# dryman/HashMergeJoin

Measured on AMD Instinct MI355X. Metric: probe-side tuples/s + achieved HBM GB/s, |R|=|S|=2^28 u64 keys, higher is better.
Workload: dtype u64

## Files before the change

### hashmergejoin_amd/_lib.py

```python
import ctypes as C
import os

HMJ_MATERIALIZE = 0x01
HMJ_ORDERED = 0x02
HMJ_FIRST_WINS = 0x04
HMJ_CHECKSUM = 0x08
HMJ_SUM_PROBE = 0x10
HMJ_NULL_EQUAL = 0x20
HMJ_E_RCCL, HMJ_E_PEER, HMJ_E_TIMEOUT = -6, -7, -8
HMJ_PATH_SLAB, HMJ_PATH_EXACT, HMJ_PATH_UNIQ_WRITE, HMJ_PATH_SPLIT, HMJ_PATH_WINDOW = 0x1, 0x2, 0x4, 0x8, 0x10
HMJ_PATH_ORDER_DEFERRED, HMJ_PATH_ORDER_BY_KEY, HMJ_PATH_PREPARED, HMJ_PATH_CHUNKED_BUILD = 0x20, 0x40, 0x80, 0x100
HMJ_PATH_HOT_KEY_HINT = 0x200
HMJ_PATH_SLAB_PROBE = 0x400
HMJ_PATH_SORTED_WRITE = 0x800
HMJ_PATH_SORTED_FK = 0x1000
HMJ_PATH_DENSE_BUILD = 0x2000
HMJ_PATH_GLOBAL_TABLE = 0x100000
HMJ_PATH_ORDER_BY_RANK_SORT = 0x200000
HMJ_PATH_ORDERED_EXPANSION = 0x400000
HMJ_PATH_LDS_TABLE = 0x800000
HMJ_PATH_RANK_RUNS = 0x1000000
HMJ_PATH_RANK_LOOKUP_IN_PASS = 0x2000000
HMJ_PATH_SORT_MSD = 0x4000000
HMJ_PATH_KEY_RANGES = 0x8000000
# ... 284 lines not shown
def load_library():
    global _LIB
    if _LIB is not None:
        return _LIB
    path = lib_path()
    if not os.path.exists(path):
        raise HmjError(-100, "HIP extension not built: %s is missing (run `make` at the repo root)" % path)
    L = C.CDLL(path)
    u, i, vp, cp = C.c_uint64, C.c_int, C.c_void_p, C.c_char_p
    L.hmj_create.restype = i
    L.hmj_create.argtypes = [C.POINTER(vp), i]
    L.hmj_destroy.restype = None
    L.hmj_destroy.argtypes = [vp]
    L.hmj_set_stream.restype = i
    L.hmj_set_stream.argtypes = [vp, vp]
    L.hmj_reserve.restype = i
    L.hmj_reserve.argtypes = [vp, u, u, u, C.c_uint32]
    L.hmj_set_radix_bits.restype = i
    L.hmj_set_radix_bits.argtypes = [vp, i]
    L.hmj_autotune_radix_bits.restype = i
    L.hmj_autotune_radix_bits.argtypes = [vp, u, u, i, C.POINTER(C.c_int), C.POINTER(C.c_double)]
    L.hmj_set_key_prefix_bits.restype = i
    L.hmj_set_key_prefix_bits.argtypes = [vp, i]
    L.hmj_plan.restype = i
    L.hmj_plan.argtypes = [u, C.POINTER(i), C.POINTER(i), C.POINTER(i * 4)]
    L.hmj_set_profiling.restype = i
    L.hmj_set_profiling.argtypes = [vp, i]
    L.hmj_last_timing.restype = i
    L.hmj_last_timing.argtypes = [vp, C.POINTER(Timing)]
    L.hmj_last_plan.restype = i
    L.hmj_last_plan.argtypes = [vp, C.POINTER(PlanDesc)]
    L.hmj_forget_workloads.restype = i
    L.hmj_forget_workloads.argtypes = [vp]
    L.hmj_placement_info.restype = i
    L.hmj_placement_info.argtypes = [vp, C.POINTER(PlaceInfo), i]
    L.hmj_strerror.restype = cp
    L.hmj_strerror.argtypes = [i]
    L.hmj_last_error.restype = cp
    L.hmj_last_error.argtypes = [vp]
    L.hmj_version.restype = cp
    L.hmj_version.argtypes = []
    L.hmj_abi_version.restype = i
    L.hmj_abi_version.argtypes = []
    L.hmj_join_u64_device.restype = i
    L.hmj_join_u64_device.argtypes = [vp, vp, u, vp, u, C.c_uint32, C.POINTER(JoinResult)]
    L.hmj_join_kind_u64_device.restype = i
    L.hmj_join_kind_u64_device.argtypes = [vp, vp, u, vp, u, C.c_uint32, C.POINTER(JoinOpts), C.POINTER(JoinResult)]
    L.hmj_join_build_kind_u64_device.restype = i
    L.hmj_join_build_kind_u64_device.argtypes = [vp, vp, u, vp, u, C.c_uint32, C.POINTER(BuildJoinOpts), C.POINTER(JoinResult)]
    L.hmj_hash_str_device.restype = i
    L.hmj_hash_str_device.argtypes = [vp, vp, vp, u, C.c_uint32, vp]
    L.hmj_join_str_device.restype = i
    L.hmj_join_str_device.argtypes = [vp, C.POINTER(StrRel), C.POINTER(StrRel), C.c_uint32, C.POINTER(StrJoinOpts),
                                      C.POINTER(StrResult)]
    L.hmj_join_kind_str_device.restype = i
    L.hmj_join_kind_str_device.argtypes = [vp, C.POINTER(StrRel), C.POINTER(StrRel), C.c_uint32, C.POINTER(StrKindOpts),
                                           C.POINTER(StrResult)]
    L.hmj_join_cols_device.restype = i
    L.hmj_join_cols_device.argtypes = [vp, C.POINTER(ColsRel), C.POINTER(ColsRel), C.c_uint32, C.POINTER(ColsJoinOpts),
                                       C.POINTER(ColsResult)]
    L.hmj_join_kind_cols_device.restype = i
    L.hmj_join_kind_cols_device.argtypes = [vp, C.POINTER(ColsRel), C.POINTER(ColsRel), C.c_uint32, C.POINTER(ColsKindOpts),
                                            C.POINTER(ColsResult)]
    L.hmj_join_mixed_device.restype = i
    L.hmj_join_mixed_device.argtypes = [vp, C.POINTER(MixedRel), C.POINTER(MixedRel), C.c_uint32, C.POINTER(MixedOpts),
                                        C.POINTER(ColsResult)]
# ... 74 lines not shown
```

### hashmergejoin_amd/csrc/api.hip

```cpp
#include <hip/hip_runtime.h>
#include <sys/mman.h>

#include <algorithm>
#include <cstdio>
#include <cstdlib>
#include <chrono>
#include <cmath>
#include <cstring>
#include <mutex>
#include <string>
#include <thread>
#include <vector>

#include "hmj_ctx.h"

using hmj::u32;
using hmj::u64;
using namespace hmj_host;

namespace hmj_host {

constexpr int kMaxEvents = 1024;

int fail(hmj_ctx* c, int code, const char* what, hipError_t e) {
// ... 347 lines not shown
  for (int i = 0; i < 4; i++) pass_bits[i] = 0;
  for (int i = 0; i < np; i++) pass_bits[i] = B / np + (i < B % np ? 1 : 0);
  *total = B;
  *passes = np;
}

static inline bool slab_sizes_ok(const hmj_ctx* c, u64 nb, u64 np, bool small_side_ok = false) {
  const u64 big = nb > np ? nb : np, small = nb > np ? np : nb;
  const u64 floor_rows = small_side_ok ? (1u << 18) : (1u << 22);
  const u64 small_min = c->slab_min_rows < floor_rows ? c->slab_min_rows : floor_rows;
  return big >= c->slab_min_rows && small >= small_min;
}

int radix_pass(hmj_ctx* c, const void* src, void* dst, u32 n, int shift, int bits, int rel,
               u64* offsets_out, int pass_index) {
  u32 nblk, rpb;
  const int variant = c->scatter_variant;
  const int tile = hmj::radix_tile_rows(bits, variant);
  hmj::radix_pass_geometry(n, tile, &nblk, &rpb);
  RC_TRY(ensure_dev(c, c->hist, (size_t)(1u << bits) * nblk * sizeof(u32)));
  RC_TRY(ensure_dev(c, c->totals, (size_t)hmj::RP_MAXD * sizeof(u32)));
  int s = span_begin(c, K_HIST, rel);
  HIP_TRY(hmj::launch_radix_hist(src, n, tile, shift, bits, (u32*)c->hist.p, nblk, rpb, c->stream));
  span_end(c, s);
  s = span_begin(c, K_SCAN, rel);
  HIP_TRY(hmj::launch_radix_rowscan((u32*)c->hist.p, nblk, bits, (u32*)c->totals.p, c->stream));
  span_end(c, s);
  s = span_begin(c, K_SCATTER, rel, pass_index);
  HIP_TRY(hmj::launch_radix_scatter(src, dst, n, variant, shift, bits, (const u32*)c->hist.p,
                                    (const u32*)c->totals.p, nblk, rpb, offsets_out, c->stream));
  span_end(c, s);
  c->timing.bytes_hist += 16ull * n;
  c->timing.bytes_scatter += 32ull * n;
  return HMJ_OK;
}

int partition_relation(hmj_ctx* c, const void* in, u32 n, DevBuf buf[2], int top, int passes,
                       const int pass_bits[4], int rel, const void** result, bool try_in_place = false) {
  *result = in;
  if (passes == 0 || n == 0) return HMJ_OK;
  if (try_in_place) {
    int bits = 0;
    for (int i = 0; i < passes; i++) bits += pass_bits[i];
    RC_TRY(ensure_dev(c, c->offs64, 8 * sizeof(u64)));
    RC_TRY(ensure_host(c, c->h_accum, 8 * sizeof(u64)));
    u32* flag = (u32*)((u64*)c->offs64.p + 7);
    u32* hflag = (u32*)((u64*)c->h_accum.p + 7);
    HIP_TRY(hipMemsetAsync(flag, 0, 4, c->stream));
    const int sp = span_begin(c, K_HIST, rel);
    HIP_TRY(hmj::launch_check_partitioned(in, n, top, bits, flag, c->num_cus, c->stream));
    span_end(c, sp);
    HIP_TRY(hipMemcpyAsync(hflag, flag, 4, hipMemcpyDeviceToHost, c->stream));
    HIP_TRY(hipStreamSynchronize(c->stream));
    if (*hflag == 0) {
      c->timing.path |= HMJ_PATH_PRESORTED;
      return HMJ_OK;
    }
  }
  RC_TRY(ensure_dev(c, buf[0], (size_t)n * 16));
  if (passes > 1) RC_TRY(ensure_dev(c, buf[1], (size_t)n * 16));
  const void* src = in;
  int shift = top;
  for (int i = 0; i < passes; i++) {
    void* dst = buf[i & 1].p;
    RC_TRY(radix_pass(c, src, dst, n, shift, pass_bits[i], rel, nullptr, i));
    shift += pass_bits[i];
// ... 113 lines not shown
  a.r_off = (const u32*)c->r_off.p;
  a.S = Sp;
  a.s_off = (const u32*)c->s_off.p;
  a.P = P;
  a.Q = Q;
  a.accum = (u64*)c->accum.p;
  return a;
}
static hmj::ProbeArgs slab_probe_args(hmj_ctx* c, const hmj::SlabGeom* build_slabs, const void* Rp, const DevBuf& s_slab,
                                      const DevBuf& s_cnt, u32 s_cap, u32 P, u32 Q) {
  hmj::ProbeArgs a;
  std::memset(&a, 0, sizeof(a));
  if (build_slabs) {
    a.R = c->slab_br.p;
    a.r_cnt = (const u32*)c->cnt_br.p;
    a.r_cap = build_slabs->CB;
    a.r_cnt_n = c->cnt_br.cap / 4;
    a.r_rows = c->slab_br.cap / 16;
  } else {
    a.R = Rp;
    a.r_off = (const u32*)c->r_off.p;
  }
  a.S = s_slab.p;
  a.s_cnt = (const u32*)s_cnt.p;
  a.s_cap = s_cap;
  a.s_cnt_n = s_cnt.cap / 4;
  a.s_rows = s_slab.cap / 16;
  a.P = P;
  a.Q = Q;
  a.accum = (u64*)c->accum.p;
  return a;
}

static int slab_pass_a(hmj_ctx* c, const void* in, u32 n, int rel, int low, int bits, const hmj::SlabGeom& g, bool arriving) {
  u64* acc = (u64*)c->accum.p;
  const u64 a_rows = c->slab_a.cap / 16, a_cnt = c->cnt_a.cap / 4;
  const int sp = span_begin(c, K_SCATTER, rel, 0);
  if (arriving) {
    u32 w_done = 0;
    for (size_t i = 0; i < c->arrive_ev.size(); i++) {
      RC_TRY(wait_arrival(c, c->arrive_ev[i]));
      const bool last = i + 1 == c->arrive_ev.size();
      const u32 w_end = last ? g.WA : (u32)std::min<u64>(g.WA, c->arrive_rows[i] / g.rpw);
      if (w_end > w_done) {
        HIP_TRY(hmj::launch_slab_a(in, n, low, bits, g, c->slab_a.p, a_rows, (u32*)c->cnt_a.p, a_cnt, acc, c->stream, w_done, w_end));
        w_done = w_end;
      }
    }
  } else {
    HIP_TRY(hmj::launch_slab_a(in, n, low, bits, g, c->slab_a.p, a_rows, (u32*)c->cnt_a.p, a_cnt, acc, c->stream));
  }
  span_end(c, sp);
  c->timing.bytes_scatter += 32ull * n;
  return HMJ_OK;
}
static int slab_passes(hmj_ctx* c, const void* in, u32 n, int rel, int low, int ba, int bb, const hmj::SlabGeom& g, DevBuf& sb,
                       DevBuf& cb, bool arriving) {
  RC_TRY(slab_pass_a(c, in, n, rel, low, ba, g, arriving));
  const int sp = span_begin(c, K_SCATTER, rel, 1);
  HIP_TRY(hmj::launch_slab_b(c->slab_a.p, (const u32*)c->cnt_a.p, ba, low + ba, bb, g, sb.p, sb.cap / 16, (u32*)cb.p, cb.cap / 4,
                             (u64*)c->accum.p, c->stream));
  span_end(c, sp);
  c->timing.bytes_scatter += 32ull * n;
  return HMJ_OK;
}

static int clear_matched(hmj_ctx* c, size_t slots, u32** matched) {
  const size_t bytes = (slots / 32 + 1) * 4;
  RC_TRY(ensure_dev(c, c->matched, bytes));
  *matched = (u32*)c->matched.p;
  HIP_TRY(hipMemsetAsync(c->matched.p, 0, bytes, c->stream));
  return HMJ_OK;
}

int order_rows(hmj_ctx* c, const u32* vstart, const u32* in_base32, const u64* in_base64, u32 P, u32 Q, int low,
               u64 n, bool by_key_only, bool many_per_key, const u64** rk, const u64** rr, const u64** rs, int* retry_code) {
  const size_t bytes = (size_t)n * 8;
  RC_TRY(ensure_dev(c, c->ord_key, bytes));
  RC_TRY(ensure_dev(c, c->ord_rval, bytes));
  RC_TRY(ensure_dev(c, c->ord_sval, bytes));
  const bool can_sort = n <= 0xFFFFFFFFull;
  if (by_key_only && !can_sort) {
    *retry_code = kRetryNoWinOrdered;
    return HMJ_OK;
  }
  int sp = span_begin(c, K_ORDER, -1);
  HIP_TRY(hmj::launch_order((const u64*)c->part_out_off.p, vstart, in_base32, in_base64, P, Q, low,
                            (const u64*)c->out_key.p, (const u64*)c->out_rval.p, (const u64*)c->out_sval.p,
                            (u64*)c->ord_key.p, (u64*)c->ord_rval.p, (u64*)c->ord_sval.p, (u64*)c->accum.p,
                            can_sort ? 65536u : 0u, many_per_key, c->num_cus * 4, c->stream));
  span_end(c, sp);
  u64* h = (u64*)c->h_accum.p;
  HIP_TRY(hipMemcpyAsync(&h[hmj::ACC_ERR], (u64*)c->accum.p + hmj::ACC_ERR, 8, hipMemcpyDeviceToHost, c->stream));
  HIP_TRY(hipStreamSynchronize(c->stream));
  if (h[hmj::ACC_ERR] & hmj::ERR_ORDER_FAIL)
    return fail(c, HMJ_E_UNSUPPORTED, "HMJ_ORDERED: one partition's result exceeds 2^31-1 rows and the whole result 2^32-1 rows");
// ... 520 lines not shown

static int run_slab_join(hmj_ctx* c, const JoinCall& j, const JoinPlan& p) {
  const bool materialize = j.materialize(), first = j.first(), extra = j.extra();
  const u32 nb = j.nb, np = j.np, np_plan = p.np_plan, P = p.P;
  const int* pass_bits = p.pass_bits;
  hmj::SlabGeom gr, gs;
  if (p.allow_slab && c->slab_mode && c->wm->slab_cooldown == 0 && !c->prepare_only && !(c->timing.path & HMJ_PATH_SLAB) &&
      !((!materialize || p.fast_write) && p.Q == 1 && p.probe_fits && p.passes == 2 && pass_bits[0] <= hmj::SLAB_MAX_BITS &&
        pass_bits[1] <= hmj::SLAB_MAX_BITS && p.dense_scale <= 2.5))
    c->plan.refused |= HMJ_REFUSED_SLAB_SHAPE;
  if (!(p.allow_slab && c->slab_mode && c->wm->slab_cooldown == 0 && (!materialize || p.fast_write) && p.Q == 1 &&
        p.probe_fits &&
        p.passes == 2 && pass_bits[0] <= hmj::SLAB_MAX_BITS && pass_bits[1] <= hmj::SLAB_MAX_BITS &&
        slab_sizes_ok(c, nb, np_plan, materialize || np_plan < nb) &&
        p.dense_scale <= 2.5 &&
        hmj::slab_geometry(nb, pass_bits[0], pass_bits[1], &gr, 0, 1.0, p.dense_scale) &&
        hmj::slab_geometry(np_plan, pass_bits[0], pass_bits[1], &gs, 0,
                           (nb && np_plan > nb) ? (double)np_plan / (double)nb : 1.0, p.dense_scale)))
    return kPlanNotTaken;
  const bool reuse = c->prep.valid && c->prep.slab && c->prep.ptr == j.R && c->prep.n == nb &&
                     c->prep.low == p.low && c->prep.B == p.B;
  c->prep.valid = false;
  c->timing.path |= HMJ_PATH_SLAB | (reuse ? HMJ_PATH_PREPARED : 0u);
  c->timing.n_probe_items = P;
  const int ba = pass_bits[0], bb = pass_bits[1];
  const u64 rows_a = gr.rows_a > gs.rows_a ? gr.rows_a : gs.rows_a;
  const u32 wa = gr.WA > gs.WA ? gr.WA : gs.WA;
  RC_TRY(ensure_dev(c, c->slab_a, rows_a * 16));
  RC_TRY(ensure_dev(c, c->cnt_a, ((size_t)wa << ba) * 4));
  RC_TRY(ensure_dev(c, c->slab_br, gr.rows_b * 16));
  RC_TRY(ensure_dev(c, c->slab_bs, gs.rows_b * 16));
  RC_TRY(ensure_dev(c, c->cnt_br, (size_t)P * gr.KB * 4));
  RC_TRY(ensure_dev(c, c->cnt_bs, (size_t)P * gs.KB * 4));
  if (!reuse) RC_TRY(slab_passes(c, j.R, nb, 0, p.low, ba, bb, gr, c->slab_br, c->cnt_br, false));
  if (!c->prepare_only) RC_TRY(slab_passes(c, j.S, np, 1, p.low, ba, bb, gs, c->slab_bs, c->cnt_bs, !c->arrive_ev.empty()));
  u64* hh;
  if (c->prepare_only) {
    RC_TRY(read_accum(c, &hh));
    if (hh[hmj::ACC_ERR] & hmj::ERR_SLAB) {
      c->wm->slab_cooldown = 8;
      return kRetryNoSlab;
    }
    c->prep.valid = true;
    c->prep.slab = true;
    c->prep.ptr = j.R;
    c->prep.n = nb;
    c->prep.low = p.low;
    c->prep.B = p.B;
    return HMJ_OK;
  }
  hmj::ProbeArgs sa = slab_probe_args(c, &gr, nullptr, c->slab_bs, c->cnt_bs, gs.CB, P, 1);
  if (p.fast_write)
    return unique_key_write(c, sa, true, nb, np, p.low, extra, p.verify_pfx ? p.prefix : 0, p.pfx_ref, j.ordered(), j.to_host,
                            p.fk_wide_plan, p.dense_scale, j.out);
#ifdef HMJ_DEV
  sa.debug = c->dev_ablate;
#endif
  int sp = span_begin(c, K_PROBE_COUNT, -1);
  if (first || extra) {
    sa.extra = (extra ? 1u : 0u) | (first ? 2u : 0u);
    HIP_TRY(hmj::launch_probe_count_ext(sa, nullptr, nullptr, true, c->num_cus, c->stream));
  } else {
    HIP_TRY(hmj::launch_probe_count_slab(sa, c->num_cus, c->stream));
  }
  span_end(c, sp);
  c->timing.bytes_probe_count = 16ull * ((u64)nb + np);
  RC_TRY(read_accum(c, &hh));
  if (hh[hmj::ACC_ERR] & hmj::ERR_SLAB) {
    c->wm->slab_cooldown = 8;
    return kRetryNoSlab;
  }
  result_sums(j.out, hh);
  return HMJ_OK;
}

static int partition_build_exact(hmj_ctx* c, const JoinCall& j, const JoinPlan& p, const void** Rp) {
  const bool reuse_exact = c->prep.valid && !c->prep.slab && c->prep.ptr == j.R && c->prep.n == j.nb &&
                           c->prep.low == p.low && c->prep.B == p.B;
  c->prep.valid = false;
  c->timing.path |= HMJ_PATH_EXACT | (reuse_exact ? HMJ_PATH_PREPARED : 0u);
  if (reuse_exact) {
    *Rp = c->prep.Rp;
  } else {
    RC_TRY(partition_relation(c, j.R, j.nb, c->rbuf, p.low, p.passes, p.pass_bits, 0, Rp, p.asc_r));
    const int s = span_begin(c, K_OFFSETS, -1);
    HIP_TRY(hmj::launch_part_offsets(*Rp, j.nb, p.low, p.B, (u32*)c->r_off.p, c->stream));
    span_end(c, s);
  }
  if (c->prepare_only) {
    HIP_TRY(hipStreamSynchronize(c->stream));
    c->prep.valid = true;
    c->prep.slab = false;
    c->prep.ptr = j.R;
    c->prep.Rp = *Rp;
    c->prep.n = j.nb;
    c->prep.low = p.low;
    c->prep.B = p.B;
  }
  return HMJ_OK;
}

static int run_probe_slab_join(hmj_ctx* c, const JoinCall& j, const JoinPlan& p, const void* Rp) {
  const bool materialize = j.materialize(), first = j.first(), extra = j.extra();
// ... 1089 lines not shown
      HIP_TRY(hipMemcpyAsync((u64*)c->cat_key.p + rows_done, sub.key, bytes, hipMemcpyDeviceToDevice, c->stream));
      HIP_TRY(hipMemcpyAsync((u64*)c->cat_rval.p + rows_done, sub.rval, bytes, hipMemcpyDeviceToDevice, c->stream));
      HIP_TRY(hipMemcpyAsync((u64*)c->cat_sval.p + rows_done, sub.sval, bytes, hipMemcpyDeviceToDevice, c->stream));
      rows_done += sub.n_matches;
    }
    tot.n_matches += sub.n_matches;
    tot.sum_r += sub.sum_r;
    tot.sum_s += sub.sum_s;
    tot.xor_fold ^= sub.xor_fold;
    tot.mix_sum += sub.mix_sum;
    tot.sum_probe_all += sub.sum_probe_all;
  }
  HIP_TRY(hipStreamSynchronize(c->stream));
  *out = tot;
  out->key = rows_done ? (const uint64_t*)c->cat_key.p : nullptr;
  out->rval = rows_done ? (const uint64_t*)c->cat_rval.p : nullptr;
  out->sval = rows_done ? (const uint64_t*)c->cat_sval.p : nullptr;
  c->timing = tsum;
  c->timing.path |= HMJ_PATH_KEY_RANGES;
  *done = true;
  return HMJ_OK;
}

int join_device(hmj_ctx* c, const void* R, uint64_t n_build, const void* S, uint64_t n_probe,
                uint32_t flags, hmj_result* out, bool to_host) {
  if ((flags & HMJ_MATERIALIZE) && !(flags & HMJ_ORDERED) && !c->prepare_only && !c->join_kind && c->promote_to_ordered && n_build > 0 &&
      n_probe <= 0xFFFFFFFFull && n_probe >= c->big_join_rows && (double)n_probe >= 2.5 * (double)n_build && c->force_bits < 0) {
    const double P18 = (double)(1u << (2 * hmj::SLAB_MAX_BITS));
    const double hi = fk_probe_rows_hi((double)n_probe / P18, (double)n_probe / (double)n_build, P18);
    if (hi > 5120.0 && hi <= 6144.0) flags |= HMJ_ORDERED;
  }
  memo_for(c, workload_signature(n_build, c->prepare_only ? c->probe_hint : n_probe, flags, c->join_kind ? 2 + (int)c->join_kind : c->memo_kind));
  std::memset(&c->plan, 0, sizeof(c->plan));
  int rc = HMJ_OK, kr_h = 0;
  bool kr_done = false;
  if (!c->join_kind && key_ranges_wanted(c, n_build, n_probe, flags, to_host, &kr_h)) {
    rc = join_by_key_ranges(c, R, n_build, S, n_probe, flags, out, kr_h, &kr_done);
  } else if (c->cat_key.p) {
    free_dev(c->cat_key);
    free_dev(c->cat_rval);
    free_dev(c->cat_sval);
  }
  if (rc == HMJ_OK && !kr_done) rc = join_device_planned(c, R, n_build, S, n_probe, flags, out, to_host);
  hmj_plan_desc& p = c->plan;
  p.struct_size = sizeof(p);
  p.path = c->timing.path;
  p.radix_bits = c->timing.radix_bits;
  p.radix_passes = c->timing.radix_passes;
  p.key_prefix_bits = c->timing.key_prefix_bits;
  p.key_window_low = c->timing.key_window_low;
  p.n_partitions = (c->timing.path & (HMJ_PATH_GLOBAL_TABLE | HMJ_PATH_LDS_TABLE)) ? 0u : (p.radix_bits < 32 ? 1u << p.radix_bits : 0u);
  p.probe_items = c->timing.n_probe_items;
  p.cooling = c->wm->cooling();
  p.workload = c->wm_sig;
  return rc;
}
static int join_device_planned(hmj_ctx* c, const void* R, uint64_t n_build, const void* S, uint64_t n_probe, uint32_t flags,
                               hmj_result* out, bool to_host) {
  const bool kinds = c->join_kind != 0;
  if (!kinds) {
    bool done = false;
    int rc = try_global_table(c, R, n_build, S, n_probe, flags, out, to_host, &done);
    if (rc != HMJ_OK || done) return rc;
    rc = try_small_build_ordered(c, R, n_build, S, n_probe, flags, out, to_host, &done);
    if (rc != HMJ_OK || done) return rc;
  }
// ... 6 lines not shown
  struct Unforce {
    hmj_ctx* c;
    bool* on;
    ~Unforce() {
      if (*on) c->force_bits = -1;
      c->expand_allow_rebits = true;
    }
  } unforce{c, &forced_here};
  for (int attempt = 0; attempt < 8; attempt++) {
    c->plan.attempts = (uint32_t)attempt + 1;
    int rc = join_device_impl(c, R, n_build, S, n_probe, flags, out, to_host, auto_prefix, slab, fast_write,
                              win_ordered, prefix_unsafe, slab_probe);
    c->plan.refused |= rc == kRetryNoSlab ? HMJ_REFUSED_SLAB_OVERFLOW : rc == kRetryNoPrefix ? HMJ_REFUSED_PREFIX_VIOLATED
                       : rc == kRetryNoFastWrite ? HMJ_REFUSED_FAST_WRITE_GAVE_UP : rc == kRetryNoSlabProbe ? HMJ_REFUSED_SLAB_PROBE_OVERFLOW
                       : rc == kRetryMoreBits ? HMJ_REFUSED_EXPANSION_GAVE_UP : 0u;
    if (c->trace)
      std::fprintf(stderr, "[hmj] join nb=%llu np=%llu flags=%#x attempt %d: rc=%d bits=%d passes=%d path=%#x prefix=%d low=%d items=%u%s\n",
                   (unsigned long long)n_build, (unsigned long long)n_probe, flags, attempt, rc, c->timing.radix_bits,
                   c->timing.radix_passes, c->timing.path, c->timing.key_prefix_bits, c->timing.key_window_low,
                   c->timing.n_probe_items,
                   rc == kRetryNoSlab ? " -> retry without the slab path (a slab overflowed)"
                   : rc == kRetryNoPrefix ? " -> retry: a row outside the sampled key prefix"
                   : rc == kRetryNoFastWrite ? " -> retry without the unique-key write mode"
                   : rc == kRetryNoWinOrdered ? " -> retry without the key window"
                   : rc == kRetryNoSlabProbe ? " -> retry without probe-side slabs (one overflowed)"
                   : rc == kRetryMoreBits ? " -> retry with one more radix bit (a partition did not fit the ordered expansion)" : "");
    if (rc == kRetryNoSlab || rc == kRetryNoPrefix || rc == kRetryNoFastWrite || rc == kRetryNoWinOrdered || rc == kRetryNoSlabProbe ||
        rc == kRetryMoreBits) {
      std::vector<Span> keep;
      for (const Span& sp : c->spans)
        if (sp.kind == K_TOTAL || sp.kind == K_H2D) keep.push_back(sp);
      c->spans.swap(keep);
      std::memset(&c->timing, 0, sizeof(c->timing));
      if (rc == kRetryNoSlab) slab = false;
      else if (rc == kRetryMoreBits) {
        c->force_bits = c->expand_rebits;
        c->expand_allow_rebits = false;
        forced_here = true;
      }
      else if (rc == kRetryNoSlabProbe) slab_probe = false;
      else if (rc == kRetryNoFastWrite) fast_write = false;
      else if (rc == kRetryNoWinOrdered) win_ordered = false;
      else if (!prefix_unsafe && win_ordered) {
        prefix_unsafe = true;
        c->wm->exact_prefix_joins = 32;
      }
      else auto_prefix = false;
      continue;
    }
    return rc;
  }
  return fail(c, HMJ_E_HIP, "join could not be planned");
}

int prepare_build(hmj_ctx* c, const void* R, uint64_t n_build, uint64_t n_probe_hint) {
  hmj_result dummy;
  c->prepare_only = true;
  c->probe_hint = n_probe_hint;
  c->prep.valid = false;
  const int rc = join_device(c, R, n_build, nullptr, 0, 0, &dummy, false);
  c->prepare_only = false;
  return rc;
}

int join_device_kind(hmj_ctx* c, const JoinKind& k, const void* R, uint64_t n_build, const void* S, uint64_t n_probe,
                     uint32_t flags, hmj_result* out, hmj_kind_counts* counts) {
// ... 17 lines not shown
    const u64 unmatched = k.kind == HMJ_JOIN_SEMI ? n_probe - out->n_matches : filled;
    counts->n_probe_matched = n_probe - unmatched;
    counts->n_probe_unmatched = unmatched;
  } else {
    const u64 b_unmatched = k.kind == HMJ_BUILD_SEMI ? n_build - swept : swept;
    counts->n_build_matched = n_build - b_unmatched;
    counts->n_build_unmatched = b_unmatched;
    if (k.kind == HMJ_FULL_OUTER) {
      counts->n_probe_matched = n_probe - filled;
      counts->n_probe_unmatched = filled;
    }
  }
  return HMJ_OK;
}

}

extern "C" {

int hmj_create(hmj_ctx** out, int device_id) {
  if (!out) return HMJ_E_ARG;
  *out = nullptr;
  int ndev = 0;
  if (hipGetDeviceCount(&ndev) != hipSuccess || ndev <= 0) {
    (void)hipGetLastError();
    return HMJ_E_NODEV;
  }
  if (device_id < 0 && hipGetDevice(&device_id) != hipSuccess) return HMJ_E_NODEV;
  if (device_id >= ndev) return HMJ_E_ARG;
  if (hipSetDevice(device_id) != hipSuccess) return HMJ_E_NODEV;
  hmj_ctx* c = new hmj_ctx();
  c->device = device_id;
  if (const char* e = getenv("HMJ_SLAB")) c->slab_mode = atoi(e);
  if (const char* e = getenv("HMJ_ONE_PASS_SLAB")) c->one_pass_slab = atoi(e) != 0;
  if (const char* e = getenv("HMJ_GTABLE")) c->gtable_mode = atoi(e) != 0;
  if (const char* e = getenv("HMJ_RANK_RUNS")) c->rank_runs_mode = atoi(e) != 0;
  if (const char* e = getenv("HMJ_RANK_RUNS_MAX_CUT")) c->rank_runs_max_cut = atoi(e) < 0 ? 0 : atoi(e) > 16 ? 16 : atoi(e);
  if (const char* e = getenv("HMJ_RANK_RUNS_MAX_GROUP")) c->rank_runs_max_group = atoi(e) < 0 ? 0 : atoi(e) > 4 ? 4 : atoi(e);
  if (const char* e = getenv("HMJ_PROMOTE_TO_ORDERED")) c->promote_to_ordered = atoi(e) != 0;
  if (const char* e = getenv("HMJ_KEY_RANGES")) c->key_ranges = atoi(e) != 0;
  if (const char* e = getenv("HMJ_KEY_RANGES_FORCE")) c->key_ranges_force = atoi(e) < 0 ? 0 : atoi(e) > 4 ? 4 : atoi(e);
  if (const char* e = getenv("HMJ_RANK_RUNS_WAVE")) c->rank_runs_wave = atoi(e) != 0;
  if (const char* e = getenv("HMJ_RANK_RUNS_MAX_LEVEL")) c->rank_runs_max_level = atoi(e) < 0 ? 0 : atoi(e) > 2 ? 2 : atoi(e);
  if (const char* e = getenv("HMJ_GTABLE_SORT")) c->gtable_sort_mode = atoi(e) != 0;
  if (const char* e = getenv("HMJ_EXPAND_FK_FANOUT")) c->expand_fk_fanout = atoi(e) > 0 ? (u32)atoi(e) : 0u;
  if (const char* e = getenv("HMJ_SORT_MSD")) c->sort_msd = atoi(e) != 0;
  if (const char* e = getenv("HMJ_SORT_MSD_MEAN")) c->sort_msd_mean = atof(e) >= 64.0 ? atof(e) : c->sort_msd_mean;
  if (const char* e = getenv("HMJ_SORT_MSD_MAX_BITS")) c->sort_msd_max_bits = atoi(e) < 2 ? 2 : atoi(e) > 18 ? 18 : atoi(e);
  if (const char* e = getenv("HMJ_SORT_MSD_MIN_LOG2")) {
    const int l = atoi(e);
    if (l >= 16 && l <= 32) c->sort_msd_min = 1ull << l;
  }
  if (const char* e = getenv("HMJ_SORT_SLAB_MIN_LOG2")) {
    const int l = atoi(e);
    if (l >= 12 && l <= 32) c->sort_slab_min = 1ull << l;
  }
  if (const char* e = getenv("HMJ_GTABLE_SORT_SLAB_MIN_LOG2")) {
    const int l = atoi(e);
    if (l >= 12 && l <= 32) c->gtable_sort_slab_min = 1ull << l;
  }
  if (const char* e = getenv("HMJ_GTABLE_SORT_FANOUT")) c->gtable_sort_fanout = atoi(e) > 0 ? (u32)atoi(e) : 1u;
  if (const char* e = getenv("HMJ_PLACE")) {
    c->place_tune = atoi(e) != 0;
    if (atoi(e) > 0) {
      c->place_tries = atoi(e);
      c->place_search_always = true;
// ... 208 lines not shown
  return HMJ_OK;
}

int hmj_set_profiling(hmj_ctx* c, int enabled) {
  if (!c) return HMJ_E_ARG;
  c->profiling = enabled != 0;
  return HMJ_OK;
}

int hmj_placement_info(hmj_ctx* c, hmj_place_info* out, int max_entries) {
  if (!c || !out || max_entries <= 0) return 0;
  int n = 0;
  for (const hmj_place_info& e : c->place_log)
    if (n < max_entries) out[n++] = e;
  return n;
}

int hmj_last_plan(hmj_ctx* c, hmj_plan_desc* out) {
  if (!c || !out || out->struct_size < 8) return HMJ_E_ARG;
  const uint32_t room = out->struct_size < sizeof(hmj_plan_desc) ? out->struct_size : (uint32_t)sizeof(hmj_plan_desc);
  hmj_plan_desc p = c->plan;
  p.struct_size = room;
  std::memcpy(out, &p, room);
  return HMJ_OK;
}

int hmj_forget_workloads(hmj_ctx* c) {
  if (!c) return HMJ_E_ARG;
  c->memos.clear();
  c->wm = &c->memo_init;
  c->wm_sig = 0;
  return HMJ_OK;
}

int hmj_last_timing(hmj_ctx* c, hmj_timing* out) {
  if (!c || !out) return HMJ_E_ARG;
  *out = c->timing;
  return HMJ_OK;
}

const char* hmj_strerror(int code) {
  switch (code) {
    case HMJ_OK: return "ok";
    case HMJ_E_ARG: return "invalid argument";
    case HMJ_E_NODEV: return "no usable HIP device";
    case HMJ_E_OOM: return "out of device or pinned host memory";
    case HMJ_E_HIP: return "HIP runtime error";
    case HMJ_E_UNSUPPORTED: return "unsupported flag combination for this input";
    case HMJ_E_RCCL: return "RCCL / transport error";
    case HMJ_E_PEER: return "another rank of the collective failed";
    case HMJ_E_TIMEOUT: return "the exchange step timed out (a peer never took part); the communicator was aborted";
    default: return "unknown error";
  }
}

const char* hmj_last_error(hmj_ctx* c) { return c ? c->last_error.c_str() : ""; }
const char* hmj_version(void) { return "hashmergejoin_amd 0.5 (gfx950)"; }
int hmj_abi_version(void) { return HMJ_ABI_VERSION; }

int hmj_reserve(hmj_ctx* c, uint64_t n_build, uint64_t n_probe, uint64_t max_matches,
                uint32_t flags) {
  if (!c) return HMJ_E_ARG;
  if (n_build > 0xFFFFFFFFull || n_probe > 0xFFFFFFFFull) return fail(c, HMJ_E_ARG, "too many rows");
  HIP_TRY(hipSetDevice(c->device));
  c->prep.valid = false;
  struct InReserve {
// ... 588 lines not shown
```

### hashmergejoin_amd/csrc/hmj_ctx.h

```cpp
#pragma once
#include <hip/hip_runtime.h>

#include <string>
#include <unordered_map>
#include <vector>

#include "../../include/hmj.h"
#include "hmj_dev.h"
#include "hmj_launch.h"

struct hmj_comm;

namespace hmj_host {

struct DevBuf {
  void* p = nullptr;
  size_t cap = 0;
};
struct HostBuf {
  void* p = nullptr;
  size_t cap = 0;
  bool pinned = true;
};

// ... 33 lines not shown
    for (DevBuf* b : {&rows, &sorted, &flags, &blk, &blk_off, &list, &runs, &acc, &start}) f(*b);
    each_result_buf(f);
  }
};

enum Kind {
  K_TOTAL = 0, K_H2D, K_D2H, K_HIST, K_SCAN, K_SCATTER, K_OFFSETS, K_PROBE_COUNT, K_OUT_SCAN,
  K_PROBE_WRITE, K_ORDER, K_NKINDS
};
struct Span {
  int kind, rel, e0, e1;
  int pass;
};

struct WorkloadMemo {
  int uniq_cooldown = 0;
  int sorted_cooldown = 0;
  bool sorted_chained = false;
  bool sorted_wide = true;
  bool sorted_fk = false;
  int sorted_fk_age = 0;
  int gtable_cooldown = 0;
  int gtable_write_cooldown = 0;
  int gtable_sort_cooldown = 0;
  int gtable_sort_slab_cooldown = 0;
  int rank_runs_cooldown = 0;
  int rank_lookup_cooldown = 0;
  int expand_cooldown = 0;
  int sort_slab_cooldown = 0;
  int sort_msd_cooldown = 0;
  int slab_cooldown = 0;
  int slab_probe_cooldown = 0;
  int one_pass_write_cooldown = 0;
  int exact_prefix_joins = 0;
  uint32_t cooling() const;
};

}

namespace hmj_host {
struct OrderedCostModel {
  double part_fixed_ms = 0.15;
  double part_ns = 0.030, part_ns_per_f = 0.00023;
  double part_bucket_ns = 0.043, part_bucket_ns_per_f = 0.0001;
  double part_epilogue_ns = 0.25;
  double comp_fixed_ms = 0.65;
  double comp_ns_chain = 0.060, comp_ns_exact = 0.072;
  double comp_ns_wide = 0.145;
  double comp_ns_beyond_l2 = 0.02;
  double runs_fixed_ms = 0.25, runs_ns = 0.0215, runs_ns_per_run = 7.5;
  double runs_ns_per_log2_build = 0.0023;
  double runs_wave_ns_per_run = 1.2, runs_wave_ns = 0.007;
  double runs_range_ns = 0.0;
};
}

struct hmj_ctx {
  using DevBuf = hmj_host::DevBuf;
  using HostBuf = hmj_host::HostBuf;
  using Span = hmj_host::Span;
  using WorkloadMemo = hmj_host::WorkloadMemo;
  using u32 = hmj::u32;
  using u64 = hmj::u64;
  int device = 0, num_cus = 256;
  hipStream_t own_stream = nullptr, stream = nullptr;
  DevBuf rbuf[2], sbuf[2], in_r, in_s, hist, totals, r_off, s_off, part_count, part_out_off, accum,
// ... 55 lines not shown
  uint64_t gtable_max_rows = 1ull << 17;
  u32 gtable_min_fanout = 0;
  uint64_t gtable_min_probe = 1;
  int gtable_wg_per_cu = 8;
  u32 gtable_slots_per_row = 16;
  int gtable_max_log_cap = 18;
  bool ltable_mode = true;
  bool gtable_sort_mode = true;
  u32 gtable_sort_fanout = 128;
  bool rank_runs_mode = true;
  int rank_runs_max_cut = 10;
  int rank_runs_max_group = 3;
  int rank_runs_max_level = 2;
  uint64_t big_join_rows = 1ull << 29;
  bool promote_to_ordered = true;
  bool key_ranges = true;
  int key_ranges_force = 0;
  bool rank_runs_wave = true;
  bool build_sort_msd = true;
  bool gtable_sort_slab = true;
  u64 gtable_sort_slab_min = 1ull << 25;
  bool expand_mode = true;
  u32 fk_payload_buckets = 24;
  u32 expand_fk_fanout = 0;
  bool expand_allow_rebits = true;
  int expand_rebits = 0;
  bool sort_msd = true;
  double sort_msd_mean = 1200.0;
  int sort_msd_max_bits = 18;
  u64 sort_msd_min = 1ull << 22;
  bool sort_slab = true;
  u64 sort_slab_min = 1ull << 25;
  int slab_mode = 1;
  bool staged_upload = false;
  bool host_pipeline = true;
  hipStream_t copy_stream = nullptr;
  std::vector<hipEvent_t> copy_ev;
  bool split_mode = true;
  bool window_mode = true;
  u32 slab_min_rows = 1u << 21;
  u32 slab_probe_kb = 0;
  bool one_pass_slab = true;
  int scatter_variant = 1;
  bool profiling = false;
  bool trace = false;
#ifdef HMJ_DEV
  u32 dev_ablate = 0;
#endif
  std::vector<hipEvent_t> events;
  std::vector<Span> spans;
  int ev_used = 0;
  hmj_timing timing;
  std::string last_error;
  hmj_comm* comm = nullptr;
  std::vector<u64> arrive_rows;
  std::vector<hipEvent_t> arrive_ev;
  bool sample_build_only = false;
  int (*arrive_wait)(hmj_ctx*, hipEvent_t) = nullptr;
};


namespace hmj_host {
int fail(hmj_ctx* c, int code, const char* what, hipError_t e = hipSuccess);
#define HIP_TRY(expr)                                                        \
  do {                                                                       \
    hipError_t _e = (expr);                                                  \
// ... 38 lines not shown
```

### hashmergejoin_amd/csrc/hmj_dev.h

```cpp
#pragma once
#include <hip/hip_runtime.h>
#include <stdint.h>

namespace hmj {

typedef unsigned long long u64;
typedef unsigned int u32;
typedef unsigned short u16;

struct __attribute__((aligned(16))) Tup {
  u64 key;
  u64 val;
};

constexpr int kWave = 64;
#ifndef HMJ_SCAN_DPP
#define HMJ_SCAN_DPP 1
#endif

#ifndef HMJ_STREAM_POLICY
#define HMJ_STREAM_POLICY 2
#endif
typedef u64 u64x2_t __attribute__((ext_vector_type(2)));
__device__ __forceinline__ void store_stream(Tup* p, const Tup& v) {
#if HMJ_STREAM_POLICY >= 1
  u64x2_t x = {v.key, v.val};
  __builtin_nontemporal_store(x, reinterpret_cast<u64x2_t*>(p));
#else
  *p = v;
#endif
}
__device__ __forceinline__ Tup load_stream(const Tup* p) {
#if HMJ_STREAM_POLICY >= 2
  const u64x2_t x = __builtin_nontemporal_load(reinterpret_cast<const u64x2_t*>(p));
  Tup t;
  t.key = x.x;
  t.val = x.y;
  return t;
#else
  return *p;
#endif
}

constexpr u64 GT_EMPTY = ~0ull;
constexpr int GT_MAXWALK = 64;
__device__ __forceinline__ u32 gt_hash(u64 key, int shift) {
  u64 h = key * 0x9E3779B97F4A7C15ull;
  h ^= h >> 32;
  h *= 0xD6E8FEB86659FD93ull;
  return (u32)(h >> shift);
}

#ifndef HMJ_RANK_PASS_CHUNK_ROWS
#define HMJ_RANK_PASS_CHUNK_ROWS 64
#endif
constexpr int RANK_PASS_CHUNK_ROWS = HMJ_RANK_PASS_CHUNK_ROWS;
__device__ __forceinline__ u64 rank_run_bucket(u64 off, int pre, u64 mult) { return ((off >> pre) * mult) >> 32; }

template <int ROWS, typename Table, typename OnSlot>
__device__ __forceinline__ void gt_walk(Table tab, u32 mask, u32 (&slot)[ROWS], bool (&live)[ROWS], OnSlot on_slot) {
  bool any_live = false;
#pragma unroll
  for (int r = 0; r < ROWS; r++) any_live |= live[r];
  while (any_live) {
    Tup e[ROWS];
#pragma unroll
    for (int r = 0; r < ROWS; r++)
      if (live[r]) e[r] = tab[slot[r]];
    any_live = false;
#pragma unroll
    for (int r = 0; r < ROWS; r++) {
      if (live[r]) {
        if (e[r].key == GT_EMPTY || on_slot(r, e[r])) {
          live[r] = false;
        } else {
          slot[r] = (slot[r] + 1) & mask;
          any_live = true;
        }
      }
    }
  }
}

constexpr int RP_THREADS = 512;
constexpr int RP_WAVES = RP_THREADS / kWave;
constexpr int RP_ITEMS = 8;
constexpr int RP_TILE = RP_THREADS * RP_ITEMS;
constexpr int RP_MAX_BITS = 9;
constexpr int RP_MAXD = 1 << RP_MAX_BITS;
constexpr int RP_MAX_BLOCKS = 2048;

constexpr int PB_THREADS = 1024;
constexpr int PB_CAP = 5120;
constexpr int PB_LOG_NB = 12;
constexpr int PB_TARGET_AVG = 4096;
constexpr int PB_PLAN_SLACK = 256;

constexpr int SLAB_KB = 4;
constexpr int SLAB_MAX_BITS = 9;

enum { ACC_N = 0, ACC_SUM_R, ACC_SUM_S, ACC_XOR, ACC_MIX, ACC_SUM_P, ACC_ERR, ACC_PAD };
constexpr u64 ERR_SLAB = 2;
constexpr u64 ERR_ORDER_DEFER = 16;
constexpr u64 ERR_ORDER_FAIL = 32;
constexpr u64 ERR_SORTED = 64;
constexpr u64 ERR_FASTPATH = 8;
constexpr u64 ERR_GTABLE = 128;
constexpr u64 ERR_PREFIX = 4;

__device__ __forceinline__ u64 mix64(u64 x) {
  x ^= x >> 30;
  x *= 0xBF58476D1CE4E5B9ull;
  x ^= x >> 27;
  x *= 0x94D049BB133111EBull;
  x ^= x >> 31;
  return x;
}

__device__ __forceinline__ u64 tmix(u64 key, u64 rval, u64 sval) {
  u64 t = mix64(key);
  t = mix64(t ^ rval);
  t = mix64(t + sval);
  return t;
}

__device__ __forceinline__ int lane_id() {
  return __builtin_amdgcn_mbcnt_hi(~0u, __builtin_amdgcn_mbcnt_lo(~0u, 0u));
}

__device__ __forceinline__ u32 popc_below(u64 m) {
  return __builtin_amdgcn_mbcnt_hi((u32)(m >> 32), __builtin_amdgcn_mbcnt_lo((u32)m, 0u));
}

__device__ __forceinline__ u32 wave_incl_scan_u32(u32 v, int ) {
#if HMJ_SCAN_DPP
  v += (u32)__builtin_amdgcn_update_dpp(0, (int)v, 0x111, 0xF, 0xF, false);
  v += (u32)__builtin_amdgcn_update_dpp(0, (int)v, 0x112, 0xF, 0xF, false);
  v += (u32)__builtin_amdgcn_update_dpp(0, (int)v, 0x114, 0xF, 0xF, false);
  v += (u32)__builtin_amdgcn_update_dpp(0, (int)v, 0x118, 0xF, 0xF, false);
  v += (u32)__builtin_amdgcn_update_dpp(0, (int)v, 0x142, 0xA, 0xF, false);
  v += (u32)__builtin_amdgcn_update_dpp(0, (int)v, 0x143, 0xC, 0xF, false);
// ... 72 lines not shown
```

### hashmergejoin_amd/csrc/hmj_launch.h

```cpp
#pragma once
#include <hip/hip_runtime.h>
#include <stddef.h>
#include <stdint.h>

#include <atomic>

namespace hmj {
typedef unsigned long long u64;
typedef unsigned int u32;

struct SmemAttrOnce {
  std::atomic<unsigned long long> devices{0};
};
inline hipError_t ensure_max_smem(SmemAttrOnce& once, const void* kernel, size_t bytes) {
  int dev = 0;
  hipError_t e = hipGetDevice(&dev);
  if (e != hipSuccess) return e;
  const unsigned long long bit = 1ull << (dev & 63);
  if (dev < 64 && (once.devices.load(std::memory_order_acquire) & bit)) return hipSuccess;
  e = hipFuncSetAttribute(kernel, hipFuncAttributeMaxDynamicSharedMemorySize, (int)bytes);
  if (e != hipSuccess) return e;
  if (dev < 64) once.devices.fetch_or(bit, std::memory_order_release);
  return hipSuccess;
}

constexpr int kMaxRanks = 16;
struct OwnerFn {
  u32 mode;
  u32 G;
  u64 spl[kMaxRanks - 1];
};
int radix_tile_rows(int bits, int variant);
void radix_pass_geometry(u32 n, int tile, u32* nblk, u32* rows_per_block);
size_t radix_scatter_smem_bytes();
hipError_t launch_radix_hist(const void* in, u32 n, int tile, int shift, int bits, u32* hist,
                             u32 nblk, u32 rows_per_block, hipStream_t st, const OwnerFn* own = nullptr);
hipError_t launch_owner_scatter(const void* in, void* out, u32 n, int bits, const OwnerFn& own,
                                const u32* hist_scanned, const u32* totals, u32 nblk, u32 rows_per_block,
                                u64* offsets_out, hipStream_t st);
hipError_t launch_radix_rowscan(u32* hist, u32 nblk, int bits, u32* totals, hipStream_t st);
hipError_t launch_radix_scatter(const void* in, void* out, u32 n, int variant, int shift, int bits,
                                const u32* hist_scanned, const u32* totals, u32 nblk,
                                u32 rows_per_block, u64* offsets_out, hipStream_t st);
struct SlabGeom {
  u32 WA, rpw, CA, CB, KB;
  u64 rows_a, rows_b;
};
bool slab_geometry(u32 n, int bits_a, int bits_b, SlabGeom* g, u32 kb = 0, double fan = 1.0, double density = 1.0);
bool slab_geometry_one_pass(u32 n, int bits, double keys_per_digit, u32 max_workers, SlabGeom* g, double density = 1.0);
u32 slab_capacity(double mean, double fan);
hipError_t launch_slab_a(const void* in, u32 n, int shift, int bits, const SlabGeom& g, void* slab_a, u64 slab_a_rows,
                         u32* cnt_a, u64 cnt_a_n, u64* accum, hipStream_t st, u32 w_begin = 0, u32 w_end = 0xFFFFFFFFu);
hipError_t launch_slab_b(const void* slab_a, const u32* cnt_a, int bits_a, int shift, int bits,
                         const SlabGeom& g, void* slab_b, u64 slab_b_rows, u32* cnt_b, u64 cnt_b_n, u64* accum, hipStream_t st);
hipError_t launch_key_sample(const void* R, u32 nb, const void* S, u32 np, u64* out, hipStream_t st);
hipError_t launch_key_exact(const void* R, u32 nb, const void* S, u32 np, u64 ref, u64* out, int num_cus, hipStream_t st,
                            bool ref_is_first_key = false);
hipError_t launch_check_partitioned(const void* a, u32 n, int low, int bits, u32* flag, int num_cus, hipStream_t st);
hipError_t launch_part_offsets(const void* a, u32 n, int low, int bits, u32* off, hipStream_t st);

struct ProbeArgs {
  const void* R;
  const u32* r_off;
  const void* S;
  const u32* s_off;
  u32 P;
  u32 Q;
  u64* part_count;
  const u64* part_out_off;
  u64* out_key;
  u64* out_rval;
  u64* out_sval;
  u64 out_cap;
  u64* accum;
  const u32* item_list;
  const u32* n_item_list;
  const u32* r_cnt;
  const u32* s_cnt;
  u32 r_cap, s_cap;
  u32 s_wa, s_ppi;
  u64 r_cnt_n, s_cnt_n;
  u64 r_rows, s_rows;
  const u64* item_base;
  const u32* r_end;
  const u32* s_end;
  u32 extra;
  u32 pfx_shift;
  u64 pfx_val;
  u32* matched;
  u32 debug;
};
hipError_t launch_probe(const ProbeArgs& a, int mode, bool first_wins, bool extra, int grid,
                        hipStream_t st);
int probe_default_grid(int num_cus);
hipError_t launch_probe_kind(const ProbeArgs& a, int mode, int kind, bool first_wins, u64 fill, int grid, hipStream_t st);
hipError_t launch_probe_build_kind(const ProbeArgs& a, int mode, int kind, u64 fill, u32* bmark, int grid, hipStream_t st);
hipError_t launch_build_sweep(const ProbeArgs& a, const u32* r_off, u32 P, const u32* vstart, u64* sweep_n, int mode,
                              bool set, u64 fill, int num_cus, hipStream_t st);
hipError_t launch_probe_count_ext(const ProbeArgs& a, u32* irregular, u32* n_irregular, bool slab,
                                  int num_cus, hipStream_t st);
hipError_t launch_probe_count_slab(const ProbeArgs& a, int num_cus, hipStream_t st);
hipError_t launch_probe_write_sorted(const ProbeArgs& a, bool slab, bool fk, int shape, u64* lookback, bool chained, int key_low,
                                     int num_cus, hipStream_t st);
hipError_t launch_probe_write_uniq(const ProbeArgs& a, bool slab, int num_cus, hipStream_t st);
hipError_t launch_slab_np(const u32* cnt, u32 P, u64* out, hipStream_t st);
hipError_t launch_probe_count_fast(const ProbeArgs& a, u32* irregular, u32* n_irregular, bool big,
                                   bool per_partition_counts, int num_cus, hipStream_t st);
hipError_t launch_scan_u64(const u64* in, u64* out_excl, u32 n, hipStream_t st);
hipError_t launch_probe_expand_ordered(const ProbeArgs& a, int key_low, int num_cus, hipStream_t st);
hipError_t launch_order(const u64* part_out_off, const u32* vstart, const u32* in_base32, const u64* in_base64, u32 P, u32 Q,
                        int low, const u64* akey, const u64* arval, const u64* asval, u64* bkey, u64* brval,
                        u64* bsval, u64* accum, u32 defer_rows, bool many_per_key, int grid, hipStream_t st);
hipError_t launch_compact(const u64* part_out_off, const u32* in_base32, const u64* in_base64, u32 P, const u64* akey,
                          const u64* arval, const u64* asval, u64* bkey, u64* brval, u64* bsval, int grid, hipStream_t st);
hipError_t launch_rekey(void* pairs, u64 n, const u64* col, hipStream_t st);

hipError_t launch_gtable_build(const void* R, u32 nb, void* tab, int log_cap, u64* accum, bool first, int num_cus,
                               hipStream_t st);
hipError_t launch_gtable_probe(const void* S, u32 np, const void* tab, int log_cap, const void* R, u64* accum, bool first,
                               bool extra, int num_cus, int wg_per_cu, hipStream_t st);
hipError_t launch_gtable_write(const void* S, u32 np, const void* tab, int log_cap, const void* R, u64* accum, u64* out_key,
                               u64* out_rval, u64* out_sval, bool first, bool extra, int num_cus, int wg_per_cu, hipStream_t st);

hipError_t launch_ltable_probe(const void* R, u32 nb, const void* S, u32 np, u64* accum, bool first, bool extra, int num_cus, hipStream_t st);
int ltable_max_rows();
hipError_t launch_sval_range(const void* S, u32 np, u64* out2 , int num_cus, hipStream_t st,
                             u32 every = 1 );
hipError_t launch_gtable_emit(const void* S, u32 np, const void* tab, int log_cap, u64 svmin, int range_bits, u64* accum,
                              void* pairs, bool extra, bool wide, int num_cus, int wg_per_cu, hipStream_t st);
hipError_t launch_gtable_swap(const void* in, void* out, u64 n, int num_cus, hipStream_t st);
hipError_t launch_gtable_emit_ranks(const void* S, u32 np, const void* tab, int log_cap, u64* accum, void* pairs, bool extra, int num_cus,
                                    int wg_per_cu, hipStream_t st);
int rank_sort_max_run(int level = 0);
hipError_t launch_sort_runs_write(const void* slabs, const u32* cnt, u32 cap, u32 P, const u64* out_off, void* out, u64* accum, int level,
// ... 36 lines not shown
```

### hashmergejoin_amd/csrc/probe.hip

```cpp
#include "hmj_dev.h"
#include "hmj_launch.h"
#include <type_traits>

namespace hmj {

constexpr u32 PB_NB = 1u << PB_LOG_NB;
constexpr u32 NIL = 0xFFFFu;
static_assert(PB_CAP < 0xFFFF, "chain links are 16-bit");

struct ProbeSmem {
  u64 key[PB_CAP];
  u64 val[PB_CAP];
  u32 head[PB_NB];
  u32 aux[PB_CAP];
  u16 next[PB_CAP];
  u32 scratch[PB_THREADS / kWave + 1];
  u64 pcount;
  u64 red[8];
  u64 obase;
  u32 wtot[PB_THREADS / kWave];
  u32 nslot;
};
constexpr u32 PB_BATCH = 2 * PB_THREADS;
static_assert(PB_BATCH <= PB_CAP, "a batch must fit an empty table");
// ... 836 lines not shown
constexpr int FP_ROWS = 5;
#ifdef HMJ_DEV
#define HMJ_ABLATE(bit) ((a.debug & (bit)) != 0u)
#else
#define HMJ_ABLATE(bit) false
#endif
#ifndef BIG_LOG_NB
#define BIG_LOG_NB 13
#endif
#ifndef HMJ_PROBE_PIECES
#define HMJ_PROBE_PIECES 1
#endif

template <int THREADS, int LOG_NB>
struct FastSmem {
  static constexpr int CAP = THREADS * FP_ROWS;
  u64 key[CAP];
  u64 val[CAP];
  u32 head[1u << LOG_NB];
  u16 next[CAP];
  u64 red[8];
  u32 itemcnt[2];
  u64 wscan[THREADS / kWave + 1];
  u32 wdup[THREADS / kWave + 1];
};

template <int LOG_NB>
__device__ __forceinline__ u32 fast_hash(u64 k) {
  u32 x = (u32)k ^ ((u32)(k >> 32) * 0x85EBCA6Bu);
  x *= 0x9E3779B1u;
  return x >> (32 - LOG_NB);
}

template <int THREADS, int ROWS = FP_ROWS>
__device__ __forceinline__ void fp_load(Tup (&t)[ROWS], const Tup* __restrict__ base, u32 n,
                                        int tid) {
#pragma unroll
  for (int k = 0; k < ROWS; k++) {
    u32 i = k * THREADS + tid;
    t[k] = base[i < n ? i : n - 1];
  }
}

static_assert(SLAB_KB == 4, "fp_load_slab / fp_load_pieces / slab_np_kernel unroll exactly four pieces per partition");
template <int THREADS, int ROWS = FP_ROWS>
__device__ __forceinline__ void fp_load_slab(Tup (&t)[ROWS], const Tup* __restrict__ base, u32 cap,
                                             u32 p1, u32 p2, u32 p3, u32 n, int tid) {
#pragma unroll
  for (int k = 0; k < ROWS; k++) {
    u32 i = k * THREADS + tid;
    i = i < n ? i : n - 1;
    const u32 j = (i >= p1) + (i >= p2) + (i >= p3);
    const u32 pre = j == 0 ? 0u : (j == 1 ? p1 : (j == 2 ? p2 : p3));
    t[k] = base[(u64)j * cap + (i - pre)];
  }
}

template <int THREADS>
__device__ __forceinline__ void fp_load_pieces(Tup (&t)[FP_ROWS], const Tup* __restrict__ base, u32 cap, u32 cnt_mine, int tid) {
  constexpr int QT = THREADS / 4;
  const u32 g = (u32)tid / QT, l = (u32)tid % QT;
  const Tup* __restrict__ piece = base + (u64)g * cap;
  const u32 last = cnt_mine ? cnt_mine - 1 : 0;
#pragma unroll
  for (int k = 0; k < FP_ROWS; k++) {
    const u32 r = l + (u32)k * QT;
    t[k] = piece[r < last ? r : last];
  }
}

template <int THREADS, int LOG_NB, bool PCOUNT, bool SLAB, int OUT>
__global__ __launch_bounds__(THREADS, 4) void probe_count_fast_kernel(
    ProbeArgs a, u32* __restrict__ irregular, u32* __restrict__ n_irregular) {
  typedef FastSmem<THREADS, LOG_NB> Smem;
  constexpr u32 CAP = Smem::CAP, NB = 1u << LOG_NB;
  constexpr bool PIECES = SLAB && OUT == 0 && !PCOUNT && HMJ_PROBE_PIECES;
  constexpr u32 QT = THREADS / 4, PIECE_CAP = FP_ROWS * QT;
  extern __shared__ __attribute__((aligned(16))) unsigned char smem_raw[];
  Smem& sm = *reinterpret_cast<Smem*>(smem_raw);
  const Tup* __restrict__ R = static_cast<const Tup*>(a.R);
  const Tup* __restrict__ S = static_cast<const Tup*>(a.S);
  const u32* __restrict__ r_off = a.r_off;
  const u32* __restrict__ s_off = a.s_off;
  const u32* __restrict__ r_end = (SLAB || a.r_end == nullptr) ? a.r_off + 1 : a.r_end;
  const u32* __restrict__ s_end = (SLAB || a.s_end == nullptr) ? a.s_off + 1 : a.s_end;
  const u32 P = a.P;
  const int tid = threadIdx.x;
  u64 acc_n = 0, acc_r = 0, acc_s = 0, acc_x = 0, acc_m = 0, acc_p = 0;
  bool pfx_bad = false, giveup = false;
  for (u32 i = tid; i < NB; i += THREADS) sm.head[i] = 0;
  if (tid < 2) sm.itemcnt[tid] = 0;
  u32 epoch = 0;
  u32 prev_p = 0xFFFFFFFFu, parity = 0;

  u32 p = blockIdx.x;
  u32 rb = 0, nb = 0, sb = 0, np = 0;
  bool regular = false;
  Tup br[FP_ROWS], pr[FP_ROWS], pq[FP_ROWS];
  u32 r1 = 0, r2 = 0, r3 = 0, s1 = 0, s2 = 0, s3 = 0, r1n = 0, r2n = 0, r3n = 0, s1n = 0, s2n = 0, s3n = 0;
  u32 rm = 0, sm_ = 0, rmn = 0, smn = 0;
  const u32 my_piece = (u32)tid / QT;
  bool slab_bad = false;
  if (p < P) {
    if (SLAB) {
      const u32* rc = a.r_cnt + (u64)p * SLAB_KB;
      const u32* sc = a.s_cnt + (u64)p * SLAB_KB;
      r1 = rc[0]; r2 = r1 + rc[1]; r3 = r2 + rc[2]; nb = r3 + rc[3];
      s1 = sc[0]; s2 = s1 + sc[1]; s3 = s2 + sc[2]; np = s3 + sc[3];
      if (nb > CAP || np > CAP) slab_bad = true;
      if (PIECES) {
        rm = my_piece == 0 ? rc[0] : my_piece == 1 ? rc[1] : my_piece == 2 ? rc[2] : rc[3];
        sm_ = my_piece == 0 ? sc[0] : my_piece == 1 ? sc[1] : my_piece == 2 ? sc[2] : sc[3];
        if (rc[0] > PIECE_CAP || rc[1] > PIECE_CAP || rc[2] > PIECE_CAP || rc[3] > PIECE_CAP || sc[0] > PIECE_CAP ||
            sc[1] > PIECE_CAP || sc[2] > PIECE_CAP || sc[3] > PIECE_CAP) {
          slab_bad = true;
          nb = CAP + 1;
        }
      }
    } else {
      rb = r_off[p]; nb = r_end[p] - rb;
      sb = s_off[p]; np = s_end[p] - sb;
    }
    regular = nb && np && nb <= CAP && np <= CAP;
    if (regular) {
      if (PIECES) {
        fp_load_pieces<THREADS>(br, R + (u64)p * SLAB_KB * a.r_cap, a.r_cap, rm, tid);
        fp_load_pieces<THREADS>(pr, S + (u64)p * SLAB_KB * a.s_cap, a.s_cap, sm_, tid);
      } else if (SLAB) {
        fp_load_slab<THREADS>(br, R + (u64)p * SLAB_KB * a.r_cap, a.r_cap, r1, r2, r3, nb, tid);
        if (OUT == 0) fp_load_slab<THREADS>(pr, S + (u64)p * SLAB_KB * a.s_cap, a.s_cap, s1, s2, s3, np, tid);
      } else {
        fp_load<THREADS>(br, R + rb, nb, tid);
        if (OUT == 0) fp_load<THREADS>(pr, S + sb, np, tid);
      }
    }
  }
  const Tup* __restrict__ dummy = reinterpret_cast<const Tup*>(a.accum);
  auto load_build = [&](Tup (&t)[FP_ROWS], bool ok, u32 pp, u32 rb_, u32 nb_, u32 q1, u32 q2, u32 q3, u32 mine) {
    if (PIECES)
      fp_load_pieces<THREADS>(t, ok ? R + (u64)pp * SLAB_KB * a.r_cap : dummy, ok ? a.r_cap : 0u, ok ? mine : 1u, tid);
    else if (SLAB)
      fp_load_slab<THREADS>(t, ok ? R + (u64)pp * SLAB_KB * a.r_cap : dummy, ok ? a.r_cap : 0u, ok ? q1 : 1u, ok ? q2 : 1u,
                            ok ? q3 : 1u, ok ? nb_ : 1u, tid);
    else
      fp_load<THREADS>(t, ok ? R + rb_ : dummy, ok ? nb_ : 1u, tid);
  };
  auto load_probe = [&](Tup (&t)[FP_ROWS], bool ok, u32 pp, u32 sb_, u32 np_, u32 q1, u32 q2, u32 q3, u32 mine) {
    if (PIECES)
      fp_load_pieces<THREADS>(t, ok ? S + (u64)pp * SLAB_KB * a.s_cap : dummy, ok ? a.s_cap : 0u, ok ? mine : 1u, tid);
    else if (SLAB)
      fp_load_slab<THREADS>(t, ok ? S + (u64)pp * SLAB_KB * a.s_cap : dummy, ok ? a.s_cap : 0u, ok ? q1 : 1u, ok ? q2 : 1u,
                            ok ? q3 : 1u, ok ? np_ : 1u, tid);
    else
      fp_load<THREADS>(t, ok ? S + sb_ : dummy, ok ? np_ : 1u, tid);
  };
  const int tid_outer = tid;
  while (p < P) {
    int tid = tid_outer;
    if constexpr (OUT != 0) asm volatile("" : "+v"(tid));
    u64 out_base = (u64)sb;
    if constexpr (OUT == 1 && SLAB) {
      const u64* ibp = a.item_base + p;
      asm volatile("s_load_dwordx2 %0, %1, 0x0\n\ts_waitcnt lgkmcnt(0)" : "=s"(out_base) : "s"(ibp) : "memory");
    }
    const u32 pn = __builtin_amdgcn_readfirstlane(p + gridDim.x);
    u32 rb2 = 0, nb2 = 0, sb2 = 0, np2 = 0;
    bool regular2 = false;
    if (pn < P) {
      if (SLAB) {
        const u32* rc = a.r_cnt + (u64)pn * SLAB_KB;
        const u32* sc = a.s_cnt + (u64)pn * SLAB_KB;
        r1n = rc[0]; r2n = r1n + rc[1]; r3n = r2n + rc[2]; nb2 = r3n + rc[3];
        s1n = sc[0]; s2n = s1n + sc[1]; s3n = s2n + sc[2]; np2 = s3n + sc[3];
        if (nb2 > CAP || np2 > CAP) slab_bad = true;
        if (PIECES) {
          rmn = my_piece == 0 ? rc[0] : my_piece == 1 ? rc[1] : my_piece == 2 ? rc[2] : rc[3];
          smn = my_piece == 0 ? sc[0] : my_piece == 1 ? sc[1] : my_piece == 2 ? sc[2] : sc[3];
          if (rc[0] > PIECE_CAP || rc[1] > PIECE_CAP || rc[2] > PIECE_CAP || rc[3] > PIECE_CAP || sc[0] > PIECE_CAP ||
              sc[1] > PIECE_CAP || sc[2] > PIECE_CAP || sc[3] > PIECE_CAP) {
            slab_bad = true;
            nb2 = CAP + 1;
          }
        }
      } else {
        rb2 = r_off[pn]; nb2 = r_end[pn] - rb2;
        sb2 = s_off[pn]; np2 = s_end[pn] - sb2;
      }
// ... 23 lines not shown
      const u32 tag = epoch << 16;
      if (!HMJ_ABLATE(1u)) {
        u32 old[FP_ROWS];
#pragma unroll
        for (int k = 0; k < FP_ROWS; k++) {
          const u32 i = k * THREADS + tid;
          old[k] = tag | NIL;
          if (PIECES ? ((u32)tid % QT + (u32)k * QT < rm) : (i < nb)) {
            if (a.pfx_shift && (br[k].key >> a.pfx_shift) != a.pfx_val) pfx_bad = true;
            sm.key[i] = br[k].key;
            sm.val[i] = br[k].val;
            old[k] = atomicExch(&sm.head[fast_hash<LOG_NB>(br[k].key)], tag | i);
          }
        }
#pragma unroll
        for (int k = 0; k < FP_ROWS; k++) {
          const u32 i = k * THREADS + tid;
          if (PIECES ? ((u32)tid % QT + (u32)k * QT < rm) : (i < nb)) sm.next[i] = ((old[k] >> 16) == epoch) ? (u16)old[k] : (u16)NIL;
        }
      } else {
#pragma unroll
        for (int k = 0; k < FP_ROWS; k++) acc_r += br[k].key;
      }
      load_build(br, regular2, pn, rb2, nb2, r1n, r2n, r3n, rmn);
      lds_barrier();
      const u64 n_before = acc_n;
      if (!HMJ_ABLATE(1u)) {
        u32 cur[FP_ROWS];
        u32 cnt[FP_ROWS], first[FP_ROWS];
#pragma unroll
        for (int k = 0; k < FP_ROWS; k++) {
          const u32 j = k * THREADS + tid;
          cur[k] = NIL;
          cnt[k] = 0;
          first[k] = OUT == 2 ? NIL : 0;
          if (PIECES ? ((u32)tid % QT + (u32)k * QT < sm_) : (j < np)) {
            if (a.pfx_shift && (pr[k].key >> a.pfx_shift) != a.pfx_val) pfx_bad = true;
            if (OUT >= 1 && (a.extra & 1u)) acc_p += pr[k].val;
            const u32 hv = sm.head[fast_hash<LOG_NB>(pr[k].key)];
            cur[k] = ((hv >> 16) == epoch) ? (hv & 0xFFFFu) : NIL;
          }
        }
        for (; !HMJ_ABLATE(2u);) {
          bool any = false;
#pragma unroll
          for (int k = 0; k < FP_ROWS; k++) any |= (cur[k] != NIL);
          if (!__any(any)) break;
#pragma unroll
          for (int k = 0; k < FP_ROWS; k++) {
            if (cur[k] != NIL) {
              const u32 i = cur[k];
              const u64 kk = sm.key[i], vv = sm.val[i];
              cur[k] = sm.next[i];
              if (kk == pr[k].key) {
                if (OUT == 2 && (a.extra & 2u)) {
                  first[k] = i < first[k] ? i : first[k];
                } else {
                  acc_n++;
                  acc_r += vv;
                  acc_s += pr[k].val;
                  if (OUT == 1) {
                    if (cnt[k] == 0) first[k] = i;
                    cnt[k]++;
                  }
                  if (OUT >= 1 && (a.extra & 1u)) {
                    const u64 m = tmix(kk, vv, pr[k].val);
                    acc_x ^= m;
                    acc_m += m;
                  }
                }
              }
            }
          }
        }
        if (OUT == 2 && (a.extra & 2u)) {
#pragma unroll
          for (int k = 0; k < FP_ROWS; k++) {
            if (first[k] != NIL) {
              const u64 vv = sm.val[first[k]];
              acc_n++;
              acc_r += vv;
              acc_s += pr[k].val;
              if (a.extra & 1u) {
                const u64 m = tmix(pr[k].key, vv, pr[k].val);
                acc_x ^= m;
                acc_m += m;
              }
            }
          }
        }
        if (OUT == 1) {
          u64 packed = 0;
          bool cx = false;
#pragma unroll
          for (int k = 0; k < FP_ROWS; k++) {
            cx |= cnt[k] > 1;
            packed |= (u64)(cnt[k] ? 1u : 0u) << (12 * k);
          }
          const int lane = tid & 63, wv = tid >> 6;
          const bool wave_dup = __any(cx);
          u64 incl = packed;
#pragma unroll
          for (int o = 1; o < kWave; o <<= 1) {
            u64 t = __shfl_up(incl, o, kWave);
            if (lane >= o) incl += t;
          }
          if (lane == 63) {
// ... 13 lines not shown
          const u64 ex = pre + incl - packed;
          if (dup) {
            giveup = true;
          } else {
            u64 o = out_base;
            u32 total = 0;
#pragma unroll
            for (int k = 0; k < FP_ROWS; k++) {
              if (cnt[k]) {
                const u64 d = o + ((ex >> (12 * k)) & 0xFFFu);
                a.out_key[d] = pr[k].key;
                a.out_rval[d] = sm.val[first[k]];
                a.out_sval[d] = pr[k].val;
              }
              const u32 tk = (u32)((tot >> (12 * k)) & 0xFFFu);
              o += tk;
              total += tk;
            }
            if (tid == 0) a.part_count[p] = total;
          }
        }
      } else {
#pragma unroll
        for (int k = 0; k < FP_ROWS; k++) acc_r += pr[k].key;
      }
      if (PCOUNT) {
        const u32 mine = (u32)(acc_n - n_before);
        const u32 ws = (u32)wave_sum_u64(mine);
        if ((tid & 63) == 0 && ws) atomicAdd(&sm.itemcnt[parity], ws);
        prev_p = p;
        parity ^= 1;
      }
    } else {
      if ((PCOUNT || OUT == 1) && tid == 0 && !(nb && np)) a.part_count[p] = 0;
      if (OUT == 1 && nb && np) giveup = true;
      if (OUT >= 1 && (a.extra & 1u) && !nb) {
        if (SLAB) {
          const Tup* base = S + (u64)p * SLAB_KB * a.s_cap;
          for (u32 j = tid; j < np; j += THREADS) {
            const u32 pc = (j >= s1) + (j >= s2) + (j >= s3);
            const u32 pre = pc == 0 ? 0 : pc == 1 ? s1 : pc == 2 ? s2 : s3;
            acc_p += base[(u64)pc * a.s_cap + (j - pre)].val;
          }
        } else {
          for (u32 j = tid; j < np; j += THREADS) acc_p += S[sb + j].val;
        }
      }
      if (OUT != 1 && !SLAB && tid == 0 && nb && np) irregular[atomicAdd(n_irregular, 1u)] = p;
      load_build(br, regular2, pn, rb2, nb2, r1n, r2n, r3n, rmn);
    }
    if (OUT == 0) {
#pragma unroll
      for (int k = 0; k < FP_ROWS; k++) pr[k] = pq[k];
    }
    p = pn; rb = rb2; nb = nb2; sb = sb2; np = np2; regular = regular2;
    r1 = r1n; r2 = r2n; r3 = r3n; s1 = s1n; s2 = s2n; s3 = s3n;
    rm = rmn; sm_ = smn;
  }
  if (SLAB && slab_bad && tid == 0) atomicOr(&a.accum[ACC_ERR], ERR_SLAB);
  if (OUT == 1 && __any(giveup) && (tid & 63) == 0) atomicOr(&a.accum[ACC_ERR], ERR_FASTPATH);
  if (__any(pfx_bad) && (tid & 63) == 0) atomicOr(&a.accum[ACC_ERR], ERR_PREFIX);
  lds_barrier();
  if (PCOUNT && prev_p != 0xFFFFFFFFu && tid == 0) a.part_count[prev_p] = sm.itemcnt[parity ^ 1];
  if (tid < 8) sm.red[tid] = 0;
  lds_barrier();
  const u64 v[6] = {acc_n, acc_r, acc_s, acc_x, acc_m, acc_p};
  block_accumulate(sm.red, a.accum, v, 1u << ACC_XOR);
}

constexpr int SW_LOGB = 12, SW_NB = 1 << SW_LOGB, SW_MAXBUCKET = 32;
constexpr u64 LB_AGG = 1ull << 62, LB_PFX = 2ull << 62, LB_MASK = (1ull << 62) - 1;
constexpr u32 LB_SPIN_LIMIT = 1u << 22;

template <int THREADS>
struct SortedSmem {
  static constexpr int CAP = THREADS * FP_ROWS, CAPB = CAP, LOGB = SW_LOGB;
  u64 key[CAP];
  u64 val[CAP];
  u64 sval[CAP];
  u32 cnt[SW_NB];
  u16 bstart[SW_NB + 2];
  u16 perm[CAP];
  u32 mbits[2][CAP / 32];
  u32 scratch[THREADS / kWave + 1];
  u32 tick[2];
  u32 flag;
  u64 obase;
  u64 red[8];
};

constexpr int SWF_LOGB = 11, SWF_CAPB = 4608, SWF_MAXDUP = 1024;
constexpr int SWF_HALF_THREADS = 512, SWF_HALF_ROWS = 6, SWF_HALF_CAPB = 2048, SWF_HALF_LOGB = 10;
// ... 1096 lines not shown
      vr_beg[v] = rb + b;
      vr_end[v] = rb + e;
    }
    if (ns == 1) {
      vs_beg[v] = sb;
      vs_end[v] = sb + np;
    } else {
      const u32 step = (np + ns - 1) / ns;
      const u32 b = qs * step, e = (b + step < np) ? b + step : np;
      vs_beg[v] = sb + (b < np ? b : np);
      vs_end[v] = sb + e;
    }
  }
}
hipError_t launch_split_parts(const u32* r_off, const u32* s_off, u32 P, u32 thr_rows, u32 slice_rows, u32 build_thr,
                              u32 build_slice, u32 cap_v, u32* vstart, u32* vr_beg, u32* vr_end, u32* vs_beg,
                              u32* vs_end, u32* nv_out, hipStream_t st) {
  hipLaunchKernelGGL(split_count_kernel, dim3(1), dim3(1024), 0, st, r_off, s_off, P, thr_rows, slice_rows, build_thr,
                     build_slice, cap_v, vstart, nv_out);
  hipLaunchKernelGGL(split_fill_kernel, dim3((cap_v + 255) / 256), dim3(256), 0, st, r_off, s_off, P, thr_rows,
                     slice_rows, build_thr, build_slice, cap_v, vstart, vr_beg, vr_end, vs_beg, vs_end);
  return hipGetLastError();
}

template <int MODE, bool FIRST, bool EXTRA>
static hipError_t launch_probe_t(const ProbeArgs& a, int grid, hipStream_t st) {
  static SmemAttrOnce attr_once;
  if (hipError_t e = ensure_max_smem(attr_once, reinterpret_cast<const void*>(probe_kernel<MODE, FIRST, EXTRA>), (size_t)sizeof(ProbeSmem)); e != hipSuccess) return e;
  hipLaunchKernelGGL((probe_kernel<MODE, FIRST, EXTRA>), dim3(grid), dim3(PB_THREADS),
                     sizeof(ProbeSmem), st, a);
  return hipGetLastError();
}

template <int THREADS, int LOG_NB, bool PCOUNT, bool SLAB = false, int OUT = 0>
static hipError_t launch_fast_t(const ProbeArgs& a, u32* irregular, u32* n_irregular, int grid,
                                hipStream_t st) {
  typedef FastSmem<THREADS, LOG_NB> Smem;
  static SmemAttrOnce attr_once;
  if (hipError_t e = ensure_max_smem(attr_once, reinterpret_cast<const void*>(probe_count_fast_kernel<THREADS, LOG_NB, PCOUNT, SLAB, OUT>), (size_t)sizeof(Smem)); e != hipSuccess) return e;
  if ((u32)grid > a.P) grid = (int)a.P;
  if (grid < 1) grid = 1;
  hipLaunchKernelGGL((probe_count_fast_kernel<THREADS, LOG_NB, PCOUNT, SLAB, OUT>), dim3(grid), dim3(THREADS),
                     sizeof(Smem), st, a, irregular, n_irregular);
  return hipGetLastError();
}

hipError_t launch_probe_count_fast(const ProbeArgs& a, u32* irregular, u32* n_irregular, bool big,
                                   bool per_partition_counts, int num_cus, hipStream_t st) {
  if (per_partition_counts) {
    if (big) return launch_fast_t<1024, BIG_LOG_NB, true>(a, irregular, n_irregular, num_cus * 4, st);
    return launch_fast_t<512, 11, true>(a, irregular, n_irregular, num_cus * 3 * 4, st);
  }
  if (big) return launch_fast_t<1024, BIG_LOG_NB, false>(a, irregular, n_irregular, num_cus * 4, st);
  return launch_fast_t<512, 11, false>(a, irregular, n_irregular, num_cus * 3 * 4, st);
}

static bool slab_operands_ok(const ProbeArgs& a) {
  const u64 pieces = (u64)a.P * SLAB_KB;
  return a.r_cnt && a.s_cnt && a.r_cnt_n >= pieces && a.s_cnt_n >= pieces && a.r_rows >= pieces * a.r_cap &&
         a.s_rows >= pieces * a.s_cap;
}

hipError_t launch_probe_write_uniq(const ProbeArgs& a, bool slab, int num_cus, hipStream_t st) {
  if (slab && !slab_operands_ok(a)) return hipErrorInvalidValue;
  if (slab) return launch_fast_t<1024, BIG_LOG_NB, false, true, 1>(a, nullptr, nullptr, num_cus * 4, st);
  return launch_fast_t<1024, BIG_LOG_NB, false, false, 1>(a, nullptr, nullptr, num_cus * 4, st);
}

template <bool SLAB, bool FK, bool EXTRA, bool PB = false>
static hipError_t launch_sorted_t(const ProbeArgs& a, u64* lookback, bool chained, int key_low, int grid, hipStream_t st) {
  typedef typename std::conditional<FK, SortedFkSmem<1024>, SortedSmem<1024>>::type Smem;
  static_assert(sizeof(Smem) <= 160 * 1024, "one workgroup's LDS");
  if constexpr (FK && !PB) {
    if (a.extra & 4u) return launch_sorted_t<SLAB, FK, EXTRA, true>(a, lookback, chained, key_low, grid, st);
  }
  static SmemAttrOnce attr_once;
  const void* fn = reinterpret_cast<const void*>(probe_write_sorted_kernel<1024, SLAB, FK, EXTRA, FP_ROWS, SWF_CAPB, SWF_LOGB, PB>);
  if (hipError_t e = ensure_max_smem(attr_once, fn, sizeof(Smem)); e != hipSuccess) return e;
  hipLaunchKernelGGL((probe_write_sorted_kernel<1024, SLAB, FK, EXTRA, FP_ROWS, SWF_CAPB, SWF_LOGB, PB>), dim3(grid), dim3(1024), sizeof(Smem), st, a,
                     lookback, key_low, chained);
  return hipGetLastError();
}
template <int THREADS, int ROWS, int CAPB_, int LOGB_, bool SLAB, bool EXTRA, bool PB = false>
static hipError_t launch_sorted_shape_t(const ProbeArgs& a, u64* lookback, bool chained, int key_low, int grid, hipStream_t st) {
  typedef SortedFkSmem<THREADS, ROWS, CAPB_, LOGB_> Smem;
  if constexpr (!PB) {
    if (a.extra & 4u) return launch_sorted_shape_t<THREADS, ROWS, CAPB_, LOGB_, SLAB, EXTRA, true>(a, lookback, chained, key_low, grid, st);
  }
  static SmemAttrOnce attr_once;
  const void* fn = reinterpret_cast<const void*>(probe_write_sorted_kernel<THREADS, SLAB, true, EXTRA, ROWS, CAPB_, LOGB_, PB>);
  if (hipError_t e = ensure_max_smem(attr_once, fn, sizeof(Smem)); e != hipSuccess) return e;
  hipLaunchKernelGGL((probe_write_sorted_kernel<THREADS, SLAB, true, EXTRA, ROWS, CAPB_, LOGB_, PB>), dim3(grid), dim3(THREADS),
                     sizeof(Smem), st, a, lookback, key_low, chained);
// ... 17 lines not shown
  if (slab && !slab_operands_ok(a)) return hipErrorInvalidValue;
  int grid = (fk && shape == 1) ? 2 * num_cus : num_cus;
  if ((u32)grid > a.P) grid = (int)a.P;
  if (grid < 1) grid = 1;
  if (fk && shape == 1)
    return launch_sorted_shape<SWF_HALF_THREADS, SWF_HALF_ROWS, SWF_HALF_CAPB, SWF_HALF_LOGB>(a, slab, lookback, chained, key_low, grid, st);
  if (fk && shape == 2)
    return launch_sorted_shape<1024, SWF_WIDE_ROWS, SWF_WIDE_CAPB, SWF_LOGB>(a, slab, lookback, chained, key_low, grid, st);
  if (slab) return fk ? launch_sorted_x<true, true>(a, lookback, chained, key_low, grid, st)
                      : launch_sorted_x<true, false>(a, lookback, chained, key_low, grid, st);
  return fk ? launch_sorted_x<false, true>(a, lookback, chained, key_low, grid, st)
            : launch_sorted_x<false, false>(a, lookback, chained, key_low, grid, st);
}

__global__ void slab_np_kernel(const u32* __restrict__ cnt, u32 P, u64* __restrict__ out) {
  u32 p = blockIdx.x * blockDim.x + threadIdx.x;
  if (p < P) {
    const u32* q = cnt + (u64)p * SLAB_KB;
    out[p] = (u64)q[0] + q[1] + q[2] + q[3];
  }
}
hipError_t launch_slab_np(const u32* cnt, u32 P, u64* out, hipStream_t st) {
  hipLaunchKernelGGL(slab_np_kernel, dim3((P + 255) / 256), dim3(256), 0, st, cnt, P, out);
  return hipGetLastError();
}

hipError_t launch_probe_count_ext(const ProbeArgs& a, u32* irregular, u32* n_irregular, bool slab,
                                  int num_cus, hipStream_t st) {
  if (slab && !slab_operands_ok(a)) return hipErrorInvalidValue;
  if (slab) return launch_fast_t<1024, BIG_LOG_NB, false, true, 2>(a, nullptr, nullptr, num_cus * 4, st);
  return launch_fast_t<1024, BIG_LOG_NB, false, false, 2>(a, irregular, n_irregular, num_cus * 4, st);
}

hipError_t launch_probe_count_slab(const ProbeArgs& a, int num_cus, hipStream_t st) {
  if (!slab_operands_ok(a)) return hipErrorInvalidValue;
  return launch_fast_t<1024, BIG_LOG_NB, false, true>(a, nullptr, nullptr, num_cus * 4, st);
}

hipError_t launch_probe(const ProbeArgs& a, int mode, bool first_wins, bool extra, int grid,
                        hipStream_t st) {
  if (!a.item_list && (u64)grid > (u64)a.P * a.Q) grid = (int)((u64)a.P * a.Q);
  if (grid < 1) grid = 1;
  if (a.s_ppi) {
    if (!a.s_cnt || (mode != 0 && mode != 3) || (mode == 3 && (!a.out_key || !a.out_rval || !a.out_sval || a.out_cap == 0)) || (first_wins && !a.matched) || a.s_wa == 0 || (u64)a.P * a.s_wa * a.s_cap > 0xFFFFFFFFull || (u64)a.Q * a.s_ppi < a.s_wa || (u64)(a.Q - 1) * a.s_ppi >= a.s_wa ||
        a.s_cnt_n < (u64)a.P * a.s_wa || a.s_rows < (u64)a.P * a.s_wa * a.s_cap)
      return hipErrorInvalidValue;
  } else if (a.s_cnt && (a.s_cnt_n < (u64)a.P * a.Q || a.s_rows < (u64)a.P * a.Q * a.s_cap || (u64)a.P * a.Q * a.s_cap > 0xFFFFFFFFull))
    return hipErrorInvalidValue;
#define HMJ_DISPATCH(M)                                                          \
  if (first_wins)                                                                \
    return extra ? launch_probe_t<M, true, true>(a, grid, st)                    \
                 : launch_probe_t<M, true, false>(a, grid, st);                  \
  else                                                                           \
    return extra ? launch_probe_t<M, false, true>(a, grid, st)                   \
                 : launch_probe_t<M, false, false>(a, grid, st);
  if (mode == 3 && !a.s_ppi) return hipErrorInvalidValue;
  if (mode == 0) {
    HMJ_DISPATCH(0)
  } else if (mode == 3) {
    HMJ_DISPATCH(3)
  } else if (mode == 1) {
    HMJ_DISPATCH(1)
  } else {
    if (first_wins) return launch_probe_t<2, true, false>(a, grid, st);
    return launch_probe_t<2, false, false>(a, grid, st);
  }
#undef HMJ_DISPATCH
}
// ... 427 lines not shown
```

### hashmergejoin_amd/csrc/radix.hip

```cpp
#include <cstdlib>
#include <cstring>

#include <type_traits>

#include "hmj_dev.h"
#include "hmj_launch.h"

namespace hmj {

template <int OWN>
__device__ __forceinline__ u32 owner_digit(u64 key, int shift, u32 mask, const OwnerFn& f) {
  if (OWN == 1) return (u32)__umul64hi(mix64(key), (u64)f.G);
  if (OWN == 2) {
    u32 d = 0;
#pragma unroll
    for (int i = 0; i < kMaxRanks - 1; i++) d += ((u32)i + 1 < f.G && key >= f.spl[i]) ? 1u : 0u;
    return d;
  }
  return (u32)(key >> shift) & mask;
}

template <int OWN>
__global__ __launch_bounds__(RP_THREADS) void radix_hist_kernel(const Tup* __restrict__ in, u32 n,
                                                                int shift, u32 mask,
// ... 218 lines not shown
#define HMJ_WC_NOBAR5 1
#endif
#ifdef HMJ_STAMPS
__device__ unsigned long long g_wc_stamps[32];
struct WcStamps {
  u32 acc[14];
  u64 last;
  int base;
  __device__ __forceinline__ void begin() {
    asm volatile("s_waitcnt vmcnt(0)" ::: "memory");
    last = __builtin_amdgcn_s_memtime();
  }
  __device__ __forceinline__ void mark(int i) {
    const u64 now = __builtin_amdgcn_s_memtime();
    acc[i] += (u32)(now - last);
    last = now;
  }
  __device__ __forceinline__ void flush() {
    if ((threadIdx.x & 63) == 0)
      for (int i = 0; i < 14; i++) atomicAdd(&g_wc_stamps[base + i], (unsigned long long)acc[i]);
  }
};
#define WC_STAMP_ARG , WcStamps& stamps
#define WC_STAMP_PASS , stamps
#define WC_MARK(i) stamps.mark(i)
#define WC_VMWAIT() asm volatile("s_waitcnt vmcnt(0)" ::: "memory")
#else
#define WC_STAMP_ARG
#define WC_STAMP_PASS
#define WC_MARK(i)
#define WC_VMWAIT()
#endif

template <int THREADS, int MAXD>
struct WcSmem {
  static constexpr int TILE = THREADS * WC_ITEMS;
  static constexpr int WAVES = THREADS / kWave;
  static constexpr int ZROWS = WAVES * MAXD * 8 / 16;
  static constexpr int MAXLINES = TILE / WC_LINE + 2 * MAXD;
  static_assert(ZROWS <= TILE && ZROWS % THREADS == 0, "lane masks must alias whole row slabs");
  static_assert(MAXD <= THREADS && MAXD * WC_LINE == TILE, "one digit per thread; carry == tile slots");
  union {
    Tup stage[TILE];
    u64 lanemask[WAVES][MAXD];
  };
  Tup carry[MAXD][WC_LINE];
  u16 wcnt[WAVES][MAXD];
  u32 tile_off[MAXD];
  u32 cflush[MAXD];
  static constexpr bool HAS_CF_TILE = MAXD <= 256;
  u32 cf_tile[HAS_CF_TILE ? MAXD : 1];
  u32 plan[MAXD];
  u32 pend[MAXD];
  u32 line_off[MAXD];
  u16 line_tab[MAXLINES];
  u32 total_lines;
  u32 scratch[WAVES + 1];
};

struct NoLimit {
  __device__ __forceinline__ u32 operator()(u32) const { return 0xFFFFFFFFu; }
};
template <int THREADS, int MAXD, bool HI, bool ALLVALID, bool LIMIT, typename Prefetch, typename Limit>
__device__ __forceinline__ void wc_tile(WcSmem<THREADS, MAXD>& sm, Tup (&t)[WC_ITEMS], u32 tile_n,
                                        Tup* __restrict__ out, int shift, u32 mask, u32 D,
                                        Prefetch&& prefetch, const Limit& limit, bool* ovf WC_STAMP_ARG) {
  typedef WcSmem<THREADS, MAXD> Smem;
  constexpr int WAVES = Smem::WAVES;
  const int tid = threadIdx.x, lane = tid & 63, w = tid >> 6;
  u16* wc = &sm.wcnt[w][0];
  u64* lm = &sm.lanemask[w][0];
  const u64 lanebit = 1ull << lane;
  const u32 wbase = (u32)w * (WC_ITEMS * 64) + lane;

  u32 dr[WC_ITEMS];
#ifdef HMJ_STAMPS
  stamps.last = __builtin_amdgcn_s_memtime();
  WC_VMWAIT();
  WC_MARK(0);
  stamps.acc[11]++;
#endif
#pragma unroll
  for (int r = 0; r < WC_ITEMS; r++) {
    u32 d = 0, rank = 0;
    if (ALLVALID || wbase + r * 64 < tile_n) {
      d = digit_of<HI>(t[r].key, shift, mask);
      __hip_atomic_fetch_or(&lm[d], lanebit, __ATOMIC_RELAXED, __HIP_MEMORY_SCOPE_WORKGROUP);
      const u64 m = __hip_atomic_load(&lm[d], __ATOMIC_RELAXED, __HIP_MEMORY_SCOPE_WORKGROUP);
      const u32 old = __hip_atomic_load(&wc[d], __ATOMIC_RELAXED, __HIP_MEMORY_SCOPE_WORKGROUP);
      const u32 below = popc_below(m);
      if (below == 0) {
        __hip_atomic_store(&lm[d], 0ull, __ATOMIC_RELAXED, __HIP_MEMORY_SCOPE_WORKGROUP);
        __hip_atomic_store(&wc[d], (u16)(old + (u32)__popcll(m)), __ATOMIC_RELAXED,
                           __HIP_MEMORY_SCOPE_WORKGROUP);
      }
      rank = old + below;
    }
    dr[r] = (d << 16) | rank;
  }
  WC_MARK(1);
  lds_barrier();
  WC_MARK(2);

#if HMJ_WC_PLAN1
  if (w == 0) {
    constexpr int DPL = MAXD / kWave;
    u32 cnt[DPL], nl[DPL], pd[DPL], cf[DPL], fl[DPL];
#pragma unroll
    for (int j = 0; j < DPL; j++) {
      const u32 d = (u32)j * kWave + lane;
      cnt[j] = nl[j] = pd[j] = cf[j] = fl[j] = 0;
      if (d < D) {
        u32 c[WAVES];
#pragma unroll
        for (int k = 0; k < WAVES; k++) c[k] = sm.wcnt[k][d];
        u32 run = 0;
#pragma unroll
        for (int k = 0; k < WAVES; k++) {
          sm.wcnt[k][d] = (u16)run;
          run += c[k];
        }
        cnt[j] = run;
        pd[j] = sm.pend[d];
        cf[j] = sm.cflush[d];
        u32 avail = pd[j] + run;
        if (LIMIT && cf[j] + avail > limit(d)) {
          *ovf = true;
          avail = 0;
          pd[j] = 0;
        }
        const u32 tail = (cf[j] + avail) & (WC_LINE - 1);
        fl[j] = (tail >= avail) ? 0u : avail - tail;
        nl[j] = fl[j] ? (((cf[j] & (WC_LINE - 1)) + fl[j] + WC_LINE - 1) >> 3) : 0u;
        sm.pend[d] = avail - fl[j];
        sm.cflush[d] = cf[j] + fl[j];
      }
    }
    u32 running = 0;
#pragma unroll
    for (int j = 0; j < DPL; j++) {
      const u32 d = (u32)j * kWave + lane;
      const u32 v = (nl[j] << 16) | cnt[j];
      const u32 incl = wave_incl_scan_u32(v, lane);
      const u32 sc = running + incl - v;
      running += (u32)__builtin_amdgcn_readlane((int)incl, 63);
      if (d < D) {
        const u32 loff = sc >> 16;
        sm.tile_off[d] = sc & 0xFFFFu;
        if constexpr (Smem::HAS_CF_TILE) sm.cf_tile[d] = cf[j];
        sm.plan[d] = (fl[j] << 8) | pd[j];
        sm.line_off[d] = loff;
        for (u32 l = 0; l < nl[j]; l++) sm.line_tab[loff + l] = (u16)d;
      }
    }
    if (lane == 0) sm.total_lines = running >> 16;
  }
#else
  {
    u32 cnt = 0, nl = 0, pd = 0, cf = 0, fl = 0;
    if ((u32)tid < D) {
#pragma unroll
      for (int k = 0; k < WAVES; k++) {
        u32 c = sm.wcnt[k][tid];
        sm.wcnt[k][tid] = (u16)cnt;
        cnt += c;
      }
      pd = sm.pend[tid];
      cf = sm.cflush[tid];
      u32 avail = pd + cnt;
      if (LIMIT && cf + avail > limit((u32)tid)) {
        *ovf = true;
        avail = 0;
        pd = 0;
      }
      const u32 tail = (cf + avail) & (WC_LINE - 1);
      fl = (tail >= avail) ? 0u : avail - tail;
      nl = fl ? (((cf & (WC_LINE - 1)) + fl + WC_LINE - 1) >> 3) : 0u;
      sm.pend[tid] = avail - fl;
      sm.cflush[tid] = cf + fl;
    }
    u32 tot;
    const u32 sc = block_excl_scan_u32<THREADS, false>((nl << 16) | cnt, sm.scratch, &tot);
    if ((u32)tid < D) {
      const u32 loff = sc >> 16;
      sm.tile_off[tid] = sc & 0xFFFFu;
      if constexpr (Smem::HAS_CF_TILE) sm.cf_tile[tid] = cf;
      sm.plan[tid] = (fl << 8) | pd;
      sm.line_off[tid] = loff;
      for (u32 l = 0; l < nl; l++) sm.line_tab[loff + l] = (u16)tid;
    }
    if (tid == 0) sm.total_lines = tot >> 16;
  }
#endif
  WC_MARK(3);
  lds_barrier();
  WC_MARK(4);

#pragma unroll
  for (int r = 0; r < WC_ITEMS; r++) {
    if (ALLVALID || wbase + r * 64 < tile_n) {
      const u32 d = dr[r] >> 16;
      sm.stage[sm.tile_off[d] + sm.wcnt[w][d] + (dr[r] & 0xFFFFu)] = t[r];
    }
  }
  WC_MARK(5);
  prefetch();
  WC_MARK(12);
  lds_barrier();
  WC_MARK(6);

  {
    const u32 TL = sm.total_lines, k = (u32)tid & (WC_LINE - 1);
    for (u32 L = (u32)tid >> 3; L < TL; L += THREADS / WC_LINE) {
      const u32 d = sm.line_tab[L];
      const u32 pl = sm.plan[d], fl = pl >> 8, pd = pl & 0xFFu;
      u32 cfd;
      if constexpr (Smem::HAS_CF_TILE) cfd = sm.cf_tile[d];
      else cfd = sm.cflush[d] - fl;
      const u32 grow = (cfd & ~(u32)(WC_LINE - 1)) + (L - sm.line_off[d]) * WC_LINE + k;
      const u32 j = grow - cfd;
      if (j < fl) store_stream(&out[grow], (j < pd) ? sm.carry[d][j] : sm.stage[sm.tile_off[d] + j - pd]);
    }
  }
  u64 keep_k[WC_ITEMS], keep_v[WC_ITEMS];
  u32 has = 0;
#pragma unroll
  for (int q = 0; q < WC_ITEMS; q++) {
    const u32 s = q * THREADS + tid, d = s >> 3, k = s & (WC_LINE - 1);
    u32 idx = 0;
    if (d < D && k < sm.pend[d]) {
      const u32 pl = sm.plan[d], fl = pl >> 8, pd = pl & 0xFFu;
      if (fl != 0 || k >= pd) {
        idx = sm.tile_off[d] + (fl ? fl - pd + k : k - pd);
        has |= 1u << q;
      }
    }
    const Tup kv = sm.stage[idx];
    keep_k[q] = kv.key;
    keep_v[q] = kv.val;
  }
  WC_MARK(7);
  lds_barrier();
  WC_MARK(8);
#pragma unroll
  for (int q = 0; q < WC_ITEMS; q++) {
    const u32 s = q * THREADS + tid;
    if (has & (1u << q)) {
      Tup kv;
      kv.key = keep_k[q];
      kv.val = keep_v[q];
      sm.carry[s >> 3][s & (WC_LINE - 1)] = kv;
    }
  }
#if HMJ_WC_NOBAR5
  {
    constexpr int ZR = MAXD * 8 / 16;
    Tup z;
    z.key = 0;
    z.val = 0;
#pragma unroll
    for (int r = 0; r < ZR / kWave; r++) sm.stage[w * ZR + r * kWave + lane] = z;
    u32* wz = reinterpret_cast<u32*>(&sm.wcnt[w][0]);
#pragma unroll
    for (int r = 0; r < MAXD / 2 / kWave; r++) wz[r * kWave + lane] = 0;
  }
  WC_MARK(9);
  WC_MARK(10);
#else
#pragma unroll
  for (int r = 0; r < WC_ITEMS; r++) {
    if (r * THREADS < Smem::ZROWS) {
      Tup z;
      z.key = 0;
      z.val = 0;
      sm.stage[r * THREADS + tid] = z;
    }
  }
  for (int i = tid; i < WAVES * MAXD / 2; i += THREADS) reinterpret_cast<u32*>(&sm.wcnt[0][0])[i] = 0;
  WC_MARK(9);
  lds_barrier();
  WC_MARK(10);
#endif
}

template <int THREADS, int MAXD>
__device__ __forceinline__ void wc_flush_carry(WcSmem<THREADS, MAXD>& sm, Tup* __restrict__ out, u32 D) {
  const int tid = threadIdx.x;
  lds_barrier();
#pragma unroll
  for (int q = 0; q < WC_ITEMS; q++) {
    const u32 s = q * THREADS + tid, d = s >> 3, k = s & (WC_LINE - 1);
    if (d < D && k < sm.pend[d]) store_stream(&out[sm.cflush[d] + k], sm.carry[d][k]);
  }
}

template <int THREADS, int MAXD>
__device__ __forceinline__ void wc_clear(WcSmem<THREADS, MAXD>& sm) {
  constexpr int WAVES = WcSmem<THREADS, MAXD>::WAVES;
  const int tid = threadIdx.x;
  for (int i = tid; i < WAVES * MAXD / 2; i += THREADS) reinterpret_cast<u32*>(&sm.wcnt[0][0])[i] = 0;
  for (int i = tid; i < WAVES * MAXD; i += THREADS) (&sm.lanemask[0][0])[i] = 0;
}

template <int THREADS, int MAXD, bool HI, bool FULL>
__global__ __launch_bounds__(THREADS, (THREADS * (MAXD <= 256 ? 2 : 1)) / 256) void radix_scatter_wc_kernel(
    const Tup* __restrict__ in, Tup* __restrict__ out, u32 n, u32 n_full, int shift, int bits,
    u32 rows_per_block, u32 worker_base, const u32* __restrict__ hist_scanned,
    const u32* __restrict__ totals, u32 nblk, u64* __restrict__ offsets_out) {
  typedef WcSmem<THREADS, MAXD> Smem;
  constexpr int TILE = Smem::TILE;
  extern __shared__ __attribute__((aligned(16))) unsigned char smem_raw[];
  Smem& sm = *reinterpret_cast<Smem*>(smem_raw);
  const u32 D = 1u << bits, mask = D - 1;
  const int tid = threadIdx.x, lane = tid & 63, w = tid >> 6;
  const u32 worker = worker_base + blockIdx.x;

  {
    u32 t = ((u32)tid < D) ? totals[tid] : 0, tot;
    u32 base = block_excl_scan_u32<THREADS>(t, sm.scratch, &tot);
    if ((u32)tid < D) {
      sm.cflush[tid] = base + hist_scanned[(u64)tid * nblk + worker];
      sm.pend[tid] = 0;
      if (offsets_out && worker == 0) {
        offsets_out[tid] = base;
        if ((u32)tid == D - 1) offsets_out[D] = n;
      }
    }
    wc_clear(sm);
  }
  __syncthreads();

// ... 10 lines not shown
  const u32 wbase = (u32)w * (WC_ITEMS * 64) + lane;

  Tup t[WC_ITEMS];
#pragma unroll
  for (int r = 0; r < WC_ITEMS; r++)
    if (FULL || begin + wbase + r * 64 < end) t[r] = load_stream(&in[begin + wbase + r * 64]);

  bool ovf = false;
#ifdef HMJ_STAMPS
  WcStamps stamps = {};
#endif
  for (u64 tile = begin; tile < end; tile += TILE) {
    const u32 tile_n = FULL ? (u32)TILE : (u32)(end - tile);
    wc_tile<THREADS, MAXD, HI, FULL, false>(
        sm, t, tile_n, out, shift, mask, D,
        [&]() {
          if (FULL && tile + TILE < end) {
            const Tup* src = in + tile + TILE;
#pragma unroll
            for (int r = 0; r < WC_ITEMS; r++) t[r] = load_stream(&src[wbase + r * 64]);
          }
        },
        NoLimit(), &ovf WC_STAMP_PASS);
  }
  wc_flush_carry(sm, out, D);
#ifdef HMJ_STAMPS
  stamps.flush();
#endif
}

struct NoXform {
  static constexpr bool kStrided = false;
};
template <int THREADS, int MAXD, bool HI, typename Xform>
__device__ __forceinline__ void slab_a_body(const Tup* __restrict__ in, u32 n, int shift, int bits, u32 rows_per_worker,
                                            Tup* __restrict__ slab, u32 CA, u32 WA, u32* __restrict__ cnt_out,
                                            u64* __restrict__ accum, u32 worker_base, Xform& xf) {
  typedef WcSmem<THREADS, MAXD> Smem;
  constexpr int TILE = Smem::TILE;
  extern __shared__ __attribute__((aligned(16))) unsigned char smem_raw[];
  Smem& sm = *reinterpret_cast<Smem*>(smem_raw);
  const u32 D = 1u << bits, mask = D - 1;
  const int tid = threadIdx.x, lane = tid & 63, w = tid >> 6;
  const u32 worker = worker_base + blockIdx.x;
  const auto limit = [=](u32 d) { return (d * WA + worker) * CA + CA; };
  if ((u32)tid < D) {
    sm.cflush[tid] = ((u32)tid * WA + worker) * CA;
    sm.pend[tid] = 0;
  }
  wc_clear(sm);
  __syncthreads();
  const u64 begin = (u64)worker * rows_per_worker;
  u64 end = begin + rows_per_worker;
  if (end > n) end = n;
  const u32 wbase = (u32)w * (WC_ITEMS * 64) + lane;
  bool ovf = false;
#ifdef HMJ_STAMPS
  WcStamps stamps = {};
#endif
  if constexpr (Xform::kStrided) {
    constexpr u32 CH = RANK_PASS_CHUNK_ROWS, IPC = CH / 64, CPT = TILE / CH;
    static_assert(WC_ITEMS % IPC == 0 && IPC >= 1, "a wave's rows of a tile are whole chunks");
    const u64 n_chunks = ((u64)n + CH - 1) / CH, whole_chunks = n / CH;
    const u32 tail = n % CH;
    const u32 slot = (u32)(((u64)worker * xf.slot_mult) % WA);
    const u64 my_whole = whole_chunks > slot ? (whole_chunks - slot + WA - 1) / WA : 0;
    auto chunk_of = [&](u64 k, u32 c) { return (k * CPT + c) * WA + slot; };
    auto rows_of = [&](u64 k) {
      const u64 first = k * CPT;
      const u32 nv = my_whole > first ? (u32)((my_whole - first < CPT) ? my_whole - first : CPT) : 0u;
      return nv * CH + ((nv < CPT && tail && chunk_of(k, nv) == whole_chunks) ? tail : 0u);
// ... 42 lines not shown
          for (int r = 0; r < WC_ITEMS; r++) {
            const u32 q = wbase + r * 64;
            t[r] = load_stream(&src[q < tn ? q : tn - 1]);
          }
        }
      };
      if constexpr (!std::is_same<Xform, NoXform>::value) xf(t, tile_n, wbase);
      if (HMJ_WC_FULLTILE && tile_n == (u32)TILE)
        wc_tile<THREADS, MAXD, HI, true, true>(sm, t, tile_n, slab, shift, mask, D, prefetch, limit, &ovf WC_STAMP_PASS);
      else
        wc_tile<THREADS, MAXD, HI, false, true>(sm, t, tile_n, slab, shift, mask, D, prefetch, limit, &ovf WC_STAMP_PASS);
    }
    wc_flush_carry(sm, slab, D);
  }
  if ((u32)tid < D) cnt_out[(u32)tid * WA + worker] = sm.cflush[tid] + sm.pend[tid] - ((u32)tid * WA + worker) * CA;
  if (ovf) atomicOr(&accum[ACC_ERR], ERR_SLAB);
#ifdef HMJ_STAMPS
  stamps.flush();
#endif
}

#ifndef HMJ_B_ADDR
#define HMJ_B_ADDR 2
#endif
#ifndef HMJ_B_NT
#define HMJ_B_NT 0
#endif
#ifdef HMJ_DEV
__device__ u32 g_b_ablate;
static bool g_b_addr_alt = false;
#endif
constexpr int SLAB_MAXSEG = 512;

template <int THREADS, int MAXD, bool HI, int ADDR>
__global__ __launch_bounds__(THREADS, (THREADS * (MAXD <= 256 ? 2 : 1)) / 256) void radix_slab_b_kernel(
    const Tup* __restrict__ slab_a, const u32* __restrict__ cnt_a, u32 CA, u32 WA, int bits_a, int shift,
    int bits, Tup* __restrict__ slab_b, u32 CB, u32* __restrict__ cnt_b, u64* __restrict__ accum, u32 KB) {
  typedef WcSmem<THREADS, MAXD> Smem;
  constexpr int TILE = Smem::TILE;
  static_assert(SLAB_MAXSEG <= THREADS, "one A-slab count per thread in the prologue scan");
  extern __shared__ __attribute__((aligned(16))) unsigned char smem_raw[];
  Smem& sm = *reinterpret_cast<Smem*>(smem_raw);
  u32* pre = reinterpret_cast<u32*>(smem_raw + sizeof(Smem));
  const u32 D = 1u << bits, mask = D - 1;
  const int tid = threadIdx.x, lane = tid & 63, w = tid >> 6;
  const u32 dA = blockIdx.x / KB, k = blockIdx.x % KB;
  const auto limit = [=](u32 d) { return (((d << bits_a) | dA) * KB + k) * CB + CB; };
  const u32 w0 = (u32)((u64)k * WA / KB), w1 = (u32)((u64)(k + 1) * WA / KB), ns = w1 - w0;
  {
    const u32 c = ((u32)tid < ns) ? cnt_a[dA * WA + w0 + tid] : 0;
    u32 tot;
    const u32 ex = block_excl_scan_u32<THREADS>(c, sm.scratch, &tot);
    if ((u32)tid < ns) pre[tid] = ex;
    if (tid == 0) pre[ns] = tot;
    if ((u32)tid < D) {
      sm.cflush[tid] = ((((u32)tid << bits_a) | dA) * KB + k) * CB;
      sm.pend[tid] = 0;
    }
    wc_clear(sm);
  }
  __syncthreads();
  const u32 total = pre[ns];
#ifdef HMJ_DEV
  const u32 abl = g_b_ablate;
#else
  constexpr u32 abl = 0;
#endif
  const u32 wbase = (u32)w * (WC_ITEMS * 64) + lane;
  (void)wbase;
  const Tup* __restrict__ bucket = slab_a + (u64)(dA * WA + w0) * CA;
  bool ovf = false;
#ifdef HMJ_STAMPS
  WcStamps stamps = {};
  stamps.base = 16;
#endif
  if (total) {
    Tup t[WC_ITEMS];
    if constexpr (ADDR != 0) {
    u32 d_s0 = 0, d_b0 = 0, d_b1 = 0, d_b2 = 0, d_b3 = 0;
    const float slabs_per_row = (float)ns / (float)total;
    auto plan1 = [&](u32 tile_begin) {
      u32 q0 = tile_begin + (u32)w * (WC_ITEMS * 64) + (u32)(lane & 3) * 64;
      q0 = q0 < total ? q0 : total - 1;
      u32 g = (u32)((float)q0 * slabs_per_row);
      g = g < ns ? g : ns - 1;
      u32 lo = g >= 3 ? g - 3 : 0;
      u32 pw[8];
#pragma unroll
      for (int i = 0; i < 8; i++) pw[i] = pre[lo + i < ns ? lo + i : ns];
      u32 j = 0;
#pragma unroll
      for (int i = 1; i < 8; i++) j += pw[i] <= q0 ? 1u : 0u;
      const bool bracketed = pw[0] <= q0 && pw[7] > q0;
      lo += j;
      if (__any(!bracketed)) {
        u32 hi = ns;
        lo = 0;
#pragma unroll
        for (int it = 0; it < 9; it++) {
          const u32 mid = (lo + hi) >> 1;
          const bool le = pre[mid] <= q0, act = hi - lo > 1;
          lo = (act && le) ? mid : lo;
          hi = (act && !le) ? mid : hi;
        }
      }
      d_s0 = lo;
      d_b0 = pre[lo];
      d_b1 = pre[lo + 1 < ns ? lo + 1 : ns];
      d_b2 = pre[lo + 2 < ns ? lo + 2 : ns];
      d_b3 = pre[lo + 3 < ns ? lo + 3 : ns];
// ... 282 lines not shown
    atomicMax(&rng[1], (unsigned long long)mx);
  }
  if (eq_r) atomicAdd(&same[0], eq_r);
  if (eq_s) atomicAdd(&same[1], eq_s);
  if (up_r) atomicAdd(&order[0], up_r);
  if (dn_r) atomicAdd(&order[1], dn_r);
  if (up_s) atomicAdd(&order[2], up_s);
  if (dn_s) atomicAdd(&order[3], dn_s);
  __syncthreads();
  {
    const u64 lo = rng[0], span = rng[1] - rng[0];
#pragma unroll
    for (int k = 0; k < 2; k++)
      if (myvalid[k] && span) atomicAdd(&bins[(u32)((mykey[k] - lo) / ((span >> 6) + 1)) & 63u], 1u);
  }
  __syncthreads();
  if (tid == 0) {
    out[0] = acc;
    out[1] = ref;
    out[2] = (u64)same[0] | ((u64)order[0] << 16) | ((u64)order[1] << 32);
    out[3] = (u64)same[1] | ((u64)order[2] << 16) | ((u64)order[3] << 32);
    out[4] = rng[0];
    out[5] = rng[1];
    u32 nonempty = 0, big = 0;
    for (int i = 0; i < 64; i++) {
      nonempty += bins[i] ? 1u : 0u;
      big = bins[i] > big ? bins[i] : big;
    }
    out[6] = nonempty;
    out[7] = big;
  }
}

template <int THREADS, int MAXD, bool HI>
__global__ __launch_bounds__(THREADS, (THREADS * (MAXD <= 256 ? 2 : 1)) / 256) void radix_slab_a_kernel(
    const Tup* __restrict__ in, u32 n, int shift, int bits, u32 rows_per_worker, Tup* __restrict__ slab,
    u32 CA, u32 WA, u32* __restrict__ cnt_out, u64* __restrict__ accum, u32 worker_base) {
  NoXform xf;
  slab_a_body<THREADS, MAXD, HI, NoXform>(in, n, shift, bits, rows_per_worker, slab, CA, WA, cnt_out, accum, worker_base, xf);
}

template <bool CUT>
struct RankXform {
  static constexpr bool kStrided = CUT;
  u32 slot_mult;
  const Tup* __restrict__ tab;
  u32 mask;
  int hshift;
  int tb, pre;
  u64 svmin, svrange, mult;
  u64 acc_s;
  u64 n_rows;
  bool miss;
  __device__ __forceinline__ void operator()(Tup (&t)[WC_ITEMS], u32 tile_n, u32 wbase) {
    u32 slot[WC_ITEMS];
    bool live[WC_ITEMS], want[WC_ITEMS];
    u32 found = 0;
#pragma unroll
    for (int r = 0; r < WC_ITEMS; r++) {
      want[r] = wbase + (u32)r * 64 < tile_n;
      slot[r] = gt_hash(t[r].key, hshift);
      if (want[r]) acc_s += t[r].val;
      if (want[r]) n_rows++;
      live[r] = want[r] && t[r].key != GT_EMPTY;
    }
    u64 rank[WC_ITEMS] = {};
    gt_walk<WC_ITEMS>(tab, mask, slot, live, [&](int r, const Tup& e) {
      const bool eq = e.key == t[r].key;
      if (eq) {
        rank[r] = e.val;
        found |= 1u << r;
      }
// ... 10 lines not shown
        t[r].key = rank[r];
      }
    }
  }
};
template <int THREADS, int MAXD, bool CUT>
__global__ __launch_bounds__(THREADS, (THREADS * (MAXD <= 256 ? 2 : 1)) / 256) void radix_slab_a_rank_kernel(
    const Tup* __restrict__ in, u32 n, int shift, int bits, u32 rows_per_worker, Tup* __restrict__ slab, u32 CA, u32 WA,
    u32* __restrict__ cnt_out, u64* __restrict__ accum, const Tup* __restrict__ tab, int log_cap, bool extra, int tb, u64 svmin, u64 svrange,
    int pre, u64 mult, u32 slot_mult) {
  RankXform<CUT> xf{slot_mult, tab, (1u << log_cap) - 1, 64 - log_cap, tb, pre, svmin, svrange, mult, 0ull, 0ull, false};
  slab_a_body<THREADS, MAXD, false, RankXform<CUT>>(in, n, shift, bits, rows_per_worker, slab, CA, WA, cnt_out, accum, 0u, xf);
  __shared__ u64 wsum[THREADS / kWave], wrows[THREADS / kWave];
  const int lane = threadIdx.x & 63, wv = threadIdx.x >> 6;
  const u64 ws = wave_sum_u64(xf.acc_s), wr = wave_sum_u64(xf.n_rows);
  const bool any_miss = __any(xf.miss);
  if (lane == 0) {
    wsum[wv] = ws;
    wrows[wv] = wr;
  }
  if (any_miss && lane == 0) atomicOr(reinterpret_cast<unsigned long long*>(&accum[ACC_ERR]), (unsigned long long)ERR_FASTPATH);
  __syncthreads();
  if (threadIdx.x == 0) {
    u64 tot = 0, rows = 0;
    for (int w = 0; w < THREADS / kWave; w++) {
      tot += wsum[w];
      rows += wrows[w];
    }
    if (tot) atomicAdd(reinterpret_cast<unsigned long long*>(&accum[ACC_SUM_S]), (unsigned long long)tot);
    if (extra && tot) atomicAdd(reinterpret_cast<unsigned long long*>(&accum[ACC_SUM_P]), (unsigned long long)tot);
    if (rows) atomicAdd(reinterpret_cast<unsigned long long*>(&accum[ACC_N]), (unsigned long long)rows);
  }
}
template <int THREADS, int MAXD, bool HI>
static hipError_t launch_slab_a_t(const void* in, u32 n, int shift, int bits, u32 rpw, void* slab, u32 CA,
                                  u32 WA, u32* cnt, u64* accum, hipStream_t st, u32 w_begin, u32 w_end) {
  typedef WcSmem<THREADS, MAXD> Smem;
  const size_t smem = sizeof(Smem);
  static_assert(sizeof(Smem) <= 160 * 1024, "slab pass A: LDS");
  static SmemAttrOnce attr_once;
  if (hipError_t e = ensure_max_smem(attr_once, reinterpret_cast<const void*>(radix_slab_a_kernel<THREADS, MAXD, HI>), (size_t)smem); e != hipSuccess) return e;
  if (w_end > WA) w_end = WA;
  if (w_begin >= w_end) return hipSuccess;
  hipLaunchKernelGGL((radix_slab_a_kernel<THREADS, MAXD, HI>), dim3(w_end - w_begin), dim3(THREADS), smem, st,
                     static_cast<const Tup*>(in), n, shift, bits, rpw, static_cast<Tup*>(slab), CA, WA, cnt,
                     accum, w_begin);
  return hipGetLastError();
}

template <int THREADS, int MAXD, bool HI>
static hipError_t launch_slab_b_t(const void* slab_a, const u32* cnt_a, u32 CA, u32 WA, int bits_a, int shift,
                                  int bits, void* slab_b, u32 CB, u32* cnt_b, u64* accum, hipStream_t st, u32 KB) {
  typedef WcSmem<THREADS, MAXD> Smem;
  const size_t smem = sizeof(Smem) + (SLAB_MAXSEG + 1) * sizeof(u32);
  static_assert(sizeof(Smem) + (SLAB_MAXSEG + 1) * sizeof(u32) <= 160 * 1024, "slab pass B: LDS");
#ifdef HMJ_DEV
  if (g_b_addr_alt) {
    constexpr int ALT = HMJ_B_ADDR == 2 ? 1 : 2;
    static SmemAttrOnce attr_alt;
    if (hipError_t e = ensure_max_smem(attr_alt, reinterpret_cast<const void*>(radix_slab_b_kernel<THREADS, MAXD, HI, ALT>), (size_t)smem); e != hipSuccess) return e;
    hipLaunchKernelGGL((radix_slab_b_kernel<THREADS, MAXD, HI, ALT>), dim3((1u << bits_a) * KB), dim3(THREADS), smem, st,
                       static_cast<const Tup*>(slab_a), cnt_a, CA, WA, bits_a, shift, bits,
                       static_cast<Tup*>(slab_b), CB, cnt_b, accum, KB);
    return hipGetLastError();
  }
#endif
  static SmemAttrOnce attr_once;
  if (hipError_t e = ensure_max_smem(attr_once, reinterpret_cast<const void*>(radix_slab_b_kernel<THREADS, MAXD, HI, HMJ_B_ADDR>), (size_t)smem); e != hipSuccess) return e;
  hipLaunchKernelGGL((radix_slab_b_kernel<THREADS, MAXD, HI, HMJ_B_ADDR>), dim3((1u << bits_a) * KB), dim3(THREADS), smem, st,
                     static_cast<const Tup*>(slab_a), cnt_a, CA, WA, bits_a, shift, bits,
                     static_cast<Tup*>(slab_b), CB, cnt_b, accum, KB);
  return hipGetLastError();
}

static u32 slab_cap(double mean, double fan) {
  double c = mean + 8.0 * __builtin_sqrt(fan * mean) + 24.0;
  return ((u32)c + 8) & ~7u;
}
u32 slab_capacity(double mean, double fan) { return slab_cap(mean, fan < 1.0 ? 1.0 : fan); }
bool slab_geometry(u32 n, int bits_a, int bits_b, SlabGeom* g, u32 kb, double fan, double density) {
  if (bits_a < 1 || bits_a > SLAB_MAX_BITS || bits_b < 1 || bits_b > SLAB_MAX_BITS) return false;
  const u32 tile = bits_a > 8 ? 4096 : 2048;
  u64 tiles = ((u64)n + tile - 1) / tile;
  u64 max_workers = 2048;
#ifdef HMJ_DEV
  if (const char* e = getenv("HMJ_SLAB_WORKERS")) max_workers = (u64)atoi(e) > 0 ? (u64)atoi(e) : max_workers;
#endif
  u64 tpw = (tiles + max_workers - 1) / max_workers;
  if (tpw == 0) tpw = 1;
  g->WA = (u32)((tiles + tpw - 1) / tpw);
  g->rpw = (u32)(tpw * tile);
  if (kb == 0) kb = SLAB_KB;
  g->KB = kb;
  if (g->WA < kb || (g->WA + kb - 1) / kb > (u32)SLAB_MAXSEG) return false;
  if (fan < 1.0) fan = 1.0;
  if (density < 1.0) density = 1.0;
  const double fan_a = 1.0 + 4.0 * (double)g->rpw * fan / (double)(n ? n : 1);
  g->CA = slab_cap(density * (double)g->rpw / (double)(1u << bits_a), fan_a < fan ? fan_a : fan);
  g->CB = slab_cap(density * (double)n / (double)(1u << bits_a) / (double)kb / (double)(1u << bits_b), fan);
  const u64 rows_a = (u64)(1u << bits_a) * g->WA * g->CA;
  const u64 rows_b = (u64)(1u << (bits_a + bits_b)) * kb * g->CB;
  g->rows_a = rows_a;
  g->rows_b = rows_b;
  return rows_a < 0xFFFFFFF0ull && rows_b < 0xFFFFFFF0ull;
}

bool slab_geometry_one_pass(u32 n, int bits, double keys_per_digit, u32 max_workers, SlabGeom* g, double density) {
  if (bits < 1 || bits > SLAB_MAX_BITS || max_workers == 0) return false;
  const u32 tile = bits > 8 ? 4096 : 2048;
  const u64 tiles = ((u64)n + tile - 1) / tile;
  u64 tpw = (tiles + max_workers - 1) / max_workers;
  if (tpw == 0) tpw = 1;
  g->WA = (u32)((tiles + tpw - 1) / tpw);
  g->rpw = (u32)(tpw * tile);
  g->KB = 0;
  g->CB = 0;
  g->rows_b = 0;
  if (density < 1.0) density = 1.0;
  const double mean = density * (double)g->rpw / (double)(1u << bits);
  if (keys_per_digit < 1.0) keys_per_digit = 1.0;
  g->CA = slab_cap(mean, 1.0 + mean / keys_per_digit);
  g->rows_a = (u64)(1u << bits) * g->WA * g->CA;
  return g->WA >= 1 && g->rows_a < 0xFFFFFFF0ull;
}

hipError_t launch_slab_a(const void* in, u32 n, int shift, int bits, const SlabGeom& g, void* slab_a, u64 slab_a_rows,
                         u32* cnt_a, u64 cnt_a_n, u64* accum, hipStream_t st, u32 w_begin, u32 w_end) {
  if (bits < 1 || bits > SLAB_MAX_BITS || g.WA == 0 || g.CA == 0 || (u64)g.WA * g.rpw < n) return hipErrorInvalidValue;
  if (slab_a_rows < ((u64)g.WA << bits) * g.CA || cnt_a_n < ((u64)g.WA << bits)) return hipErrorInvalidValue;
  if (((u64)g.WA << bits) * g.CA >= 0xFFFFFFF0ull) return hipErrorInvalidValue;
  const bool hi = shift >= 32;
#define HMJ_SLAB_A(T, M, H) launch_slab_a_t<T, M, H>(in, n, shift, bits, g.rpw, slab_a, g.CA, g.WA, cnt_a, accum, st, w_begin, w_end)
  if (bits > 8) return hi ? HMJ_SLAB_A(1024, 512, true) : HMJ_SLAB_A(1024, 512, false);
  return hi ? HMJ_SLAB_A(512, 256, true) : HMJ_SLAB_A(512, 256, false);
#undef HMJ_SLAB_A
}

hipError_t launch_slab_a_ranks(const void* in, u32 n, int shift, int bits, const SlabGeom& g, void* slab_a, u64 slab_a_rows, u32* cnt_a,
                               u64 cnt_a_n, u64* accum, const void* tab, int log_cap, bool extra, int tb, u64 svmin, u64 svrange, int pre,
                               u64 mult, hipStream_t st) {
  if (bits < 1 || bits > SLAB_MAX_BITS || g.WA == 0 || g.CA == 0 || (u64)g.WA * g.rpw < n || !tab || log_cap < 4 || log_cap > 30 || tb < 0 ||
      tb > 16 || pre < 0 || pre > 32 || shift < 0 || shift > 4 || (shift && tb))
    return hipErrorInvalidValue;
  if (slab_a_rows < ((u64)g.WA << bits) * g.CA || cnt_a_n < ((u64)g.WA << bits)) return hipErrorInvalidValue;
  if (((u64)g.WA << bits) * g.CA >= 0xFFFFFFF0ull) return hipErrorInvalidValue;
  u32 slot_mult = 1;
  if (tb > 0 && g.WA > 2) {
    auto gcd = [](u32 a, u32 b) {
      while (b) {
        const u32 t = a % b;
        a = b;
        b = t;
      }
      return a;
    };
    slot_mult = (u32)((double)g.WA * 0.6180339887498949);
    if (slot_mult < 1) slot_mult = 1;
    while (gcd(slot_mult, g.WA) != 1) slot_mult++;
  }
#define HMJ_SLAB_AR(T, M, C)                                                                                                          \
  {                                                                                                                                   \
    typedef WcSmem<T, M> Smem;                                                                                                        \
    static SmemAttrOnce once;                                                                                                         \
    if (hipError_t e = ensure_max_smem(once, reinterpret_cast<const void*>(radix_slab_a_rank_kernel<T, M, C>), sizeof(Smem)); e != hipSuccess) \
      return e;                                                                                                                       \
    hipLaunchKernelGGL((radix_slab_a_rank_kernel<T, M, C>), dim3(g.WA), dim3(T), sizeof(Smem), st, static_cast<const Tup*>(in), n, shift, bits, g.rpw, \
                       static_cast<Tup*>(slab_a), g.CA, g.WA, cnt_a, accum, static_cast<const Tup*>(tab), log_cap, extra, tb, svmin, svrange, pre, mult, \
                       slot_mult);                                                                                                    \
  }
  if (tb > 0) {
    if (bits > 8) HMJ_SLAB_AR(1024, 512, true) else HMJ_SLAB_AR(512, 256, true)
  } else {
    if (bits > 8) HMJ_SLAB_AR(1024, 512, false) else HMJ_SLAB_AR(512, 256, false)
  }
#undef HMJ_SLAB_AR
  return hipGetLastError();
}

hipError_t launch_slab_b(const void* slab_a, const u32* cnt_a, int bits_a, int shift, int bits,
                         const SlabGeom& g, void* slab_b, u64 slab_b_rows, u32* cnt_b, u64 cnt_b_n, u64* accum, hipStream_t st) {
  if (bits < 1 || bits > SLAB_MAX_BITS || bits_a < 1 || bits_a > SLAB_MAX_BITS || g.KB == 0 || g.WA < g.KB ||
      (g.WA + g.KB - 1) / g.KB > (u32)SLAB_MAXSEG)
    return hipErrorInvalidValue;
  const u64 pieces = ((u64)g.KB << (bits_a + bits));
  if (slab_b_rows < pieces * g.CB || cnt_b_n < pieces || pieces * g.CB >= 0xFFFFFFF0ull) return hipErrorInvalidValue;
  const bool hi = shift >= 32;
#define HMJ_SLAB_B(T, M, H) launch_slab_b_t<T, M, H>(slab_a, cnt_a, g.CA, g.WA, bits_a, shift, bits, slab_b, g.CB, cnt_b, accum, st, g.KB)
  if (bits > 8) return hi ? HMJ_SLAB_B(1024, 512, true) : HMJ_SLAB_B(1024, 512, false);
  return hi ? HMJ_SLAB_B(512, 256, true) : HMJ_SLAB_B(512, 256, false);
#undef HMJ_SLAB_B
}

__global__ __launch_bounds__(256) void key_exact_kernel(const Tup* __restrict__ R, u32 nb, const Tup* __restrict__ S, u32 np,
                                                        u64 ref, bool ref_is_first_key, u64* __restrict__ out) {
  if (ref_is_first_key) ref = nb ? R[0].key : (np ? S[0].key : 0);
  u64 x = 0, mn = ~0ull, mx = 0;
  const u64 stride = (u64)gridDim.x * blockDim.x;
  for (u64 i = (u64)blockIdx.x * blockDim.x + threadIdx.x; i < nb; i += stride) {
    const u64 k = R[i].key;
    x |= k ^ ref;
    mn = k < mn ? k : mn;
    mx = k > mx ? k : mx;
  }
  for (u64 i = (u64)blockIdx.x * blockDim.x + threadIdx.x; i < np; i += stride) x |= S[i].key ^ ref;
#pragma unroll
  for (int o = kWave / 2; o > 0; o >>= 1) {
    x |= __shfl_xor(x, o, kWave);
    const u64 a2 = __shfl_xor(mn, o, kWave), b2 = __shfl_xor(mx, o, kWave);
    mn = a2 < mn ? a2 : mn;
    mx = b2 > mx ? b2 : mx;
  }
  __shared__ u64 wx[4], wmn[4], wmx[4];
  if ((threadIdx.x & 63) == 0) {
    wx[threadIdx.x >> 6] = x;
    wmn[threadIdx.x >> 6] = mn;
    wmx[threadIdx.x >> 6] = mx;
  }
  __syncthreads();
  if (threadIdx.x == 0) {
    for (int w = 1; w < 4; w++) {
      x |= wx[w];
      mn = wmn[w] < mn ? wmn[w] : mn;
// ... 228 lines not shown
```

### hashmergejoin_amd/join.py

```python
import ctypes as C

import numpy as np

from . import _lib
from ._lib import (HMJ_CHECKSUM, HMJ_FIRST_WINS, HMJ_MATERIALIZE, HMJ_ORDERED, HMJ_SUM_PROBE,
                   HmjError, JoinResult, Timing)

SEED_B = 0x243F6A8885A308D3


def plan(n_build):
    L = _lib.load_library()
    tb, npass, pb = C.c_int(0), C.c_int(0), (C.c_int * 4)()
    rc = L.hmj_plan(n_build, C.byref(tb), C.byref(npass), C.byref(pb))
    if rc:
        raise HmjError(rc, "hmj_plan")
    return tb.value, [pb[i] for i in range(npass.value)]


def _dev_ptr(t):
    if t is None:
        return None, 0
    if not t.is_cuda:
        raise ValueError("expected a device tensor")
# ... 35 lines not shown
        if rc:
            raise HmjError(rc, "%s (%s)" % (self.L.hmj_strerror(rc).decode(), self.L.hmj_last_error(self.h).decode()))

    def _sync_stream(self):
        if self.use_torch_stream:
            s = self._torch.cuda.current_stream(self.device).cuda_stream
            self._check(self.L.hmj_set_stream(self.h, C.c_void_p(s)))

    def reserve(self, n_build, n_probe, max_matches=0, flags=0):
        self._check(self.L.hmj_reserve(self.h, n_build, n_probe, max_matches, flags))

    def set_radix_bits(self, bits):
        self._check(self.L.hmj_set_radix_bits(self.h, -1 if bits is None else bits))

    def set_key_prefix_bits(self, bits):
        self._check(self.L.hmj_set_key_prefix_bits(self.h, bits))

    def set_profiling(self, on=True):
        self._check(self.L.hmj_set_profiling(self.h, int(bool(on))))

    def last_timing(self):
        t = Timing()
        self._check(self.L.hmj_last_timing(self.h, C.byref(t)))
        return t.as_dict()

    def last_plan(self):
        p = _lib.PlanDesc()
        p.struct_size = C.sizeof(_lib.PlanDesc)
        self._check(self.L.hmj_last_plan(self.h, C.byref(p)))
        return p.as_dict()

    def forget_workloads(self):
        self._check(self.L.hmj_forget_workloads(self.h))

    def placement_info(self):
        arr = (_lib.PlaceInfo * 16)()
        n = self.L.hmj_placement_info(self.h, arr, 16)
        out = []
        for i in range(n):
            e, k = arr[i], int(arr[i].candidates)
            out.append({"name": e.name.decode(), "bytes": int(e.bytes), "fill_TBps": round(float(e.fill_TBps), 3),
                        "candidates": k, "ms_search": round(float(e.ms_search), 2), "searched": bool(e.searched),
                        "aborted": bool(e.aborted), "budget_ms": round(float(e.budget_ms), 1),
                        "cand_ms_alloc": [round(float(x), 2) for x in e.cand_ms_alloc[:k]],
                        "cand_ms_fill": [round(float(x), 2) for x in e.cand_ms_fill[:k]],
                        "cand_TBps": [round(float(x), 3) for x in e.cand_TBps[:k]]})
        return out

    def join_device(self, build, probe, flags=0):
        self._sync_stream()
        bp, nb = _dev_ptr(build)
        pp, np_ = _dev_ptr(probe)
        res = JoinResult()
        self._check(self.L.hmj_join_u64_device(self.h, C.c_void_p(bp), nb, C.c_void_p(pp), np_, flags, C.byref(res)))
        return res

    def join_kind_device(self, build, probe, kind, flags=0, outer_fill=0):
        self._sync_stream()
        bp, nb = _dev_ptr(build)
        pp, np_ = _dev_ptr(probe)
        res = JoinResult()
        opts = _lib.JoinOpts()
        opts.struct_size = C.sizeof(_lib.JoinOpts)
        opts.kind = int(kind)
        opts.outer_fill = int(outer_fill) & 0xFFFFFFFFFFFFFFFF
        self._check(self.L.hmj_join_kind_u64_device(self.h, C.c_void_p(bp), nb, C.c_void_p(pp), np_, flags, C.byref(opts),
# ... 968 lines not shown
```

### include/hmj.h

```cpp
#ifndef HMJ_H
#define HMJ_H

#include <stddef.h>
#include <stdint.h>

#ifdef __cplusplus
extern "C" {
#endif

typedef struct hmj_ctx hmj_ctx;

#define HMJ_OK 0
#define HMJ_E_ARG (-1)
#define HMJ_E_NODEV (-2)
#define HMJ_E_OOM (-3)
#define HMJ_E_HIP (-4)
#define HMJ_E_UNSUPPORTED (-5)

#define HMJ_E_RCCL (-6)
#define HMJ_E_PEER (-7)
#define HMJ_E_TIMEOUT (-8)

#define HMJ_MATERIALIZE 0x01u
#define HMJ_ORDERED 0x02u
// ... 111 lines not shown
#define HMJ_COOL_RANK_RUNS 0x1000u
#define HMJ_COOL_SORT_MSD 0x2000u

int hmj_create(hmj_ctx** out, int device_id);
void hmj_destroy(hmj_ctx* ctx);
#define HMJ_STREAM_OWN ((void*)(intptr_t)-1)
int hmj_set_stream(hmj_ctx* ctx, void* hip_stream);
int hmj_reserve(hmj_ctx* ctx, uint64_t n_build, uint64_t n_probe, uint64_t max_matches,
                uint32_t flags);
int hmj_set_radix_bits(hmj_ctx* ctx, int total_bits);
int hmj_autotune_radix_bits(hmj_ctx* ctx, uint64_t n_build, uint64_t n_probe, int apply, int* best_bits,
                            double ms[3]);
int hmj_set_key_prefix_bits(hmj_ctx* ctx, int bits);
int hmj_plan(uint64_t n_build, int* total_bits, int* n_passes, int pass_bits[4]);
#define HMJ_ABI_VERSION 5
int hmj_abi_version(void);
#define HMJ_PLACE_MAX_CAND 4
typedef struct {
  char name[16];
  uint64_t bytes;
  float fill_TBps;
  int candidates;
  float ms_search;
  int searched;
  int aborted;
  float budget_ms;
  float cand_ms_alloc[HMJ_PLACE_MAX_CAND];
  float cand_ms_fill[HMJ_PLACE_MAX_CAND];
  float cand_TBps[HMJ_PLACE_MAX_CAND];
} hmj_place_info;
int hmj_placement_info(hmj_ctx* ctx, hmj_place_info* out, int max_entries);
int hmj_last_plan(hmj_ctx* ctx, hmj_plan_desc* out);
int hmj_forget_workloads(hmj_ctx* ctx);
int hmj_set_profiling(hmj_ctx* ctx, int enabled);
int hmj_last_timing(hmj_ctx* ctx, hmj_timing* out);
const char* hmj_strerror(int code);
const char* hmj_last_error(hmj_ctx* ctx);
const char* hmj_version(void);

int hmj_join_u64_device(hmj_ctx* ctx, const void* build_aos_dev, uint64_t n_build,
                        const void* probe_aos_dev, uint64_t n_probe, uint32_t flags,
                        hmj_result* out);
#define HMJ_JOIN_INNER 0u
#define HMJ_JOIN_SEMI 1u
#define HMJ_JOIN_ANTI 2u
#define HMJ_JOIN_PROBE_OUTER 3u
typedef struct {
  uint32_t struct_size;
  uint32_t kind;
  uint64_t outer_fill;
  uint64_t n_probe_matched;
  uint64_t n_probe_unmatched;
} hmj_join_opts;
int hmj_join_kind_u64_device(hmj_ctx* ctx, const void* build_aos_dev, uint64_t n_build,
                             const void* probe_aos_dev, uint64_t n_probe, uint32_t flags,
                             hmj_join_opts* opts, hmj_result* out);
#define HMJ_BUILD_SEMI 1u
#define HMJ_BUILD_ANTI 2u
#define HMJ_BUILD_OUTER 3u
#define HMJ_FULL_OUTER 4u
typedef struct {
  uint32_t struct_size;
  uint32_t kind;
  uint64_t build_fill;
  uint64_t probe_fill;
  uint64_t n_build_matched;
// ... 319 lines not shown
```

Before: 34.43 billion.

## Partition probe side as key-only rows for count-only slab joins

For plain count joins (no flags, no materialization), the probe relation is scattered through both slab passes as 8-byte key-only rows instead of 16-byte key/value tuples. The probe count kernel then reads these narrower rows through templated loaders, roughly halving probe-side slab write and read traffic. The path switches on only after a prior non-bare run of the same workload size has validated the slab geometry. If the kernel raises a new error flag, it falls back to the full-width path and applies a cooldown. The cost is more template variants, a stricter slab geometry and extra host-side bookkeeping, plus a possible repeat pass on fallback.

After: 32.85 billion. 0.954x the previous value.

```diff
diff --git a/hashmergejoin_amd/_lib.py b/hashmergejoin_amd/_lib.py
--- a/hashmergejoin_amd/_lib.py
+++ b/hashmergejoin_amd/_lib.py
@@ -340,6 +340,8 @@
     L.hmj_last_plan.argtypes = [vp, C.POINTER(PlanDesc)]
     L.hmj_forget_workloads.restype = i
     L.hmj_forget_workloads.argtypes = [vp]
+    L.hmj_last_probe_row_bytes.restype = C.c_uint32
+    L.hmj_last_probe_row_bytes.argtypes = [vp]
     L.hmj_placement_info.restype = i
     L.hmj_placement_info.argtypes = [vp, C.POINTER(PlaceInfo), i]
     L.hmj_strerror.restype = cp
diff --git a/hashmergejoin_amd/csrc/api.hip b/hashmergejoin_amd/csrc/api.hip
--- a/hashmergejoin_amd/csrc/api.hip
+++ b/hashmergejoin_amd/csrc/api.hip
@@ -403,6 +403,7 @@
   span_end(c, s);
   c->timing.bytes_hist += 16ull * n;
   c->timing.bytes_scatter += 32ull * n;
+  if (rel == 1) c->probe_row_bytes = 16;
   return HMJ_OK;
 }
 
@@ -582,7 +583,8 @@
   return a;
 }
 
-static int slab_pass_a(hmj_ctx* c, const void* in, u32 n, int rel, int low, int bits, const hmj::SlabGeom& g, bool arriving) {
+static int slab_pass_a(hmj_ctx* c, const void* in, u32 n, int rel, int low, int bits, const hmj::SlabGeom& g, bool arriving,
+                       u32 row_bytes = 16) {
   u64* acc = (u64*)c->accum.p;
   const u64 a_rows = c->slab_a.cap / 16, a_cnt = c->cnt_a.cap / 4;
   const int sp = span_begin(c, K_SCATTER, rel, 0);
@@ -593,25 +595,26 @@
       const bool last = i + 1 == c->arrive_ev.size();
       const u32 w_end = last ? g.WA : (u32)std::min<u64>(g.WA, c->arrive_rows[i] / g.rpw);
       if (w_end > w_done) {
-        HIP_TRY(hmj::launch_slab_a(in, n, low, bits, g, c->slab_a.p, a_rows, (u32*)c->cnt_a.p, a_cnt, acc, c->stream, w_done, w_end));
+        HIP_TRY(hmj::launch_slab_a(in, n, low, bits, g, c->slab_a.p, a_rows, (u32*)c->cnt_a.p, a_cnt, acc, c->stream, w_done, w_end, row_bytes));
         w_done = w_end;
       }
     }
   } else {
-    HIP_TRY(hmj::launch_slab_a(in, n, low, bits, g, c->slab_a.p, a_rows, (u32*)c->cnt_a.p, a_cnt, acc, c->stream));
+    HIP_TRY(hmj::launch_slab_a(in, n, low, bits, g, c->slab_a.p, a_rows, (u32*)c->cnt_a.p, a_cnt, acc, c->stream, 0, 0xFFFFFFFFu, row_bytes));
   }
   span_end(c, sp);
-  c->timing.bytes_scatter += 32ull * n;
+  c->timing.bytes_scatter += (16ull + row_bytes) * n;
+  if (rel == 1) c->probe_row_bytes = row_bytes;
   return HMJ_OK;
 }
 static int slab_passes(hmj_ctx* c, const void* in, u32 n, int rel, int low, int ba, int bb, const hmj::SlabGeom& g, DevBuf& sb,
-                       DevBuf& cb, bool arriving) {
-  RC_TRY(slab_pass_a(c, in, n, rel, low, ba, g, arriving));
+                       DevBuf& cb, bool arriving, u32 row_bytes = 16) {
+  RC_TRY(slab_pass_a(c, in, n, rel, low, ba, g, arriving, row_bytes));
   const int sp = span_begin(c, K_SCATTER, rel, 1);
   HIP_TRY(hmj::launch_slab_b(c->slab_a.p, (const u32*)c->cnt_a.p, ba, low + ba, bb, g, sb.p, sb.cap / 16, (u32*)cb.p, cb.cap / 4,
-                             (u64*)c->accum.p, c->stream));
+                             (u64*)c->accum.p, c->stream, row_bytes));
   span_end(c, sp);
-  c->timing.bytes_scatter += 32ull * n;
+  c->timing.bytes_scatter += 2ull * row_bytes * n;
   return HMJ_OK;
 }
 
@@ -1198,8 +1201,16 @@
   RC_TRY(ensure_dev(c, c->slab_bs, gs.rows_b * 16));
   RC_TRY(ensure_dev(c, c->cnt_br, (size_t)P * gr.KB * 4));
   RC_TRY(ensure_dev(c, c->cnt_bs, (size_t)P * gs.KB * 4));
+  const bool bare_ok = c->bare_probe && j.flags == 0 && !c->prepare_only && c->arrive_ev.empty() && !c->comm && !c->join_kind &&
+                       ba <= 8 && bb <= 8 && nb && np;
+  if (bare_ok && c->wm->bare_cooldown > 0) c->wm->bare_cooldown--;
+  hmj::SlabGeom gs8;
+  const bool bare = bare_ok && c->wm->bare_cooldown == 0 && c->wm->bare_nb == nb && c->wm->bare_np == np &&
+                    hmj::slab_geometry(np_plan, ba, bb, &gs8, 0, (nb && np_plan > nb) ? (double)np_plan / (double)nb : 1.0, p.dense_scale, 8) &&
+                    gs8.WA == gs.WA && gs8.rows_a * 8 <= c->slab_a.cap && gs8.rows_b * 8 <= c->slab_bs.cap;
   if (!reuse) RC_TRY(slab_passes(c, j.R, nb, 0, p.low, ba, bb, gr, c->slab_br, c->cnt_br, false));
-  if (!c->prepare_only) RC_TRY(slab_passes(c, j.S, np, 1, p.low, ba, bb, gs, c->slab_bs, c->cnt_bs, !c->arrive_ev.empty()));
+  if (!c->prepare_only)
+    RC_TRY(slab_passes(c, j.S, np, 1, p.low, ba, bb, bare ? gs8 : gs, c->slab_bs, c->cnt_bs, !c->arrive_ev.empty(), bare ? 8u : 16u));
   u64* hh;
   if (c->prepare_only) {
     RC_TRY(read_accum(c, &hh));
@@ -1215,7 +1226,7 @@
     c->prep.B = p.B;
     return HMJ_OK;
   }
-  hmj::ProbeArgs sa = slab_probe_args(c, &gr, nullptr, c->slab_bs, c->cnt_bs, gs.CB, P, 1);
+  hmj::ProbeArgs sa = slab_probe_args(c, &gr, nullptr, c->slab_bs, c->cnt_bs, bare ? gs8.CB : gs.CB, P, 1);
   if (p.fast_write)
     return unique_key_write(c, sa, true, nb, np, p.low, extra, p.verify_pfx ? p.prefix : 0, p.pfx_ref, j.ordered(), j.to_host,
                             p.fk_wide_plan, p.dense_scale, j.out);
@@ -1227,14 +1238,33 @@
     sa.extra = (extra ? 1u : 0u) | (first ? 2u : 0u);
     HIP_TRY(hmj::launch_probe_count_ext(sa, nullptr, nullptr, true, c->num_cus, c->stream));
   } else {
-    HIP_TRY(hmj::launch_probe_count_slab(sa, c->num_cus, c->stream));
+    HIP_TRY(hmj::launch_probe_count_slab(sa, c->num_cus, c->stream, bare));
   }
   span_end(c, sp);
-  c->timing.bytes_probe_count = 16ull * ((u64)nb + np);
+  c->timing.bytes_probe_count = 16ull * nb + (bare ? 8ull : 16ull) * np;
   RC_TRY(read_accum(c, &hh));
   if (hh[hmj::ACC_ERR] & hmj::ERR_SLAB) {
     c->wm->slab_cooldown = 8;
     return kRetryNoSlab;
+  }
+  if (bare && (hh[hmj::ACC_ERR] & hmj::ERR_BARE)) {
+    c->wm->bare_nb = c->wm->bare_np = 0;
+    c->wm->bare_cooldown = 64;
+    HIP_TRY(hipMemsetAsync(c->accum.p, 0, 8 * sizeof(u64), c->stream));
+    RC_TRY(slab_passes(c, j.S, np, 1, p.low, ba, bb, gs, c->slab_bs, c->cnt_bs, false));
+    sa.s_cap = gs.CB;
+    sp = span_begin(c, K_PROBE_COUNT, -1);
+    HIP_TRY(hmj::launch_probe_count_slab(sa, c->num_cus, c->stream));
+    span_end(c, sp);
+    c->timing.bytes_probe_count += 16ull * ((u64)nb + np);
+    RC_TRY(read_accum(c, &hh));
+    if (hh[hmj::ACC_ERR] & hmj::ERR_SLAB) {
+      c->wm->slab_cooldown = 8;
+      return kRetryNoSlab;
+    }
+  } else if (!bare && bare_ok && c->wm->bare_cooldown == 0 && hh[hmj::ACC_N] == (u64)np) {
+    c->wm->bare_nb = nb;
+    c->wm->bare_np = np;
   }
   result_sums(j.out, hh);
   return HMJ_OK;
@@ -2390,6 +2420,7 @@
   }
   memo_for(c, workload_signature(n_build, c->prepare_only ? c->probe_hint : n_probe, flags, c->join_kind ? 2 + (int)c->join_kind : c->memo_kind));
   std::memset(&c->plan, 0, sizeof(c->plan));
+  c->probe_row_bytes = 0;
   int rc = HMJ_OK, kr_h = 0;
   bool kr_done = false;
   if (!c->join_kind && key_ranges_wanted(c, n_build, n_probe, flags, to_host, &kr_h)) {
@@ -2462,6 +2493,7 @@
         if (sp.kind == K_TOTAL || sp.kind == K_H2D) keep.push_back(sp);
       c->spans.swap(keep);
       std::memset(&c->timing, 0, sizeof(c->timing));
+      c->probe_row_bytes = 0;
       if (rc == kRetryNoSlab) slab = false;
       else if (rc == kRetryMoreBits) {
         c->force_bits = c->expand_rebits;
@@ -2545,6 +2577,7 @@
   hmj_ctx* c = new hmj_ctx();
   c->device = device_id;
   if (const char* e = getenv("HMJ_SLAB")) c->slab_mode = atoi(e);
+  if (const char* e = getenv("HMJ_BARE_PROBE")) c->bare_probe = atoi(e) != 0;
   if (const char* e = getenv("HMJ_ONE_PASS_SLAB")) c->one_pass_slab = atoi(e) != 0;
   if (const char* e = getenv("HMJ_GTABLE")) c->gtable_mode = atoi(e) != 0;
   if (const char* e = getenv("HMJ_RANK_RUNS")) c->rank_runs_mode = atoi(e) != 0;
@@ -2819,6 +2852,8 @@
   c->wm_sig = 0;
   return HMJ_OK;
 }
+
+uint32_t hmj_last_probe_row_bytes(hmj_ctx* c) { return c ? c->probe_row_bytes : 0u; }
 
 int hmj_last_timing(hmj_ctx* c, hmj_timing* out) {
   if (!c || !out) return HMJ_E_ARG;
diff --git a/hashmergejoin_amd/csrc/hmj_ctx.h b/hashmergejoin_amd/csrc/hmj_ctx.h
--- a/hashmergejoin_amd/csrc/hmj_ctx.h
+++ b/hashmergejoin_amd/csrc/hmj_ctx.h
@@ -89,6 +89,8 @@
   int slab_cooldown = 0;
   int slab_probe_cooldown = 0;
   int one_pass_write_cooldown = 0;
+  hmj::u32 bare_nb = 0, bare_np = 0;
+  int bare_cooldown = 0;
   int exact_prefix_joins = 0;
   uint32_t cooling() const;
 };
@@ -210,6 +212,8 @@
   bool sort_slab = true;
   u64 sort_slab_min = 1ull << 25;
   int slab_mode = 1;
+  bool bare_probe = true;
+  uint32_t probe_row_bytes = 0;
   bool staged_upload = false;
   bool host_pipeline = true;
   hipStream_t copy_stream = nullptr;
diff --git a/hashmergejoin_amd/csrc/hmj_dev.h b/hashmergejoin_amd/csrc/hmj_dev.h
--- a/hashmergejoin_amd/csrc/hmj_dev.h
+++ b/hashmergejoin_amd/csrc/hmj_dev.h
@@ -41,6 +41,39 @@
   return *p;
 #endif
 }
+
+struct __attribute__((aligned(8))) KeyRow {
+  u64 key;
+  static constexpr u64 val = 0;
+};
+__device__ __forceinline__ void store_stream(KeyRow* p, const KeyRow& v) {
+#if HMJ_STREAM_POLICY >= 1
+  __builtin_nontemporal_store(v.key, reinterpret_cast<u64*>(p));
+#else
+  *p = v;
+#endif
+}
+__device__ __forceinline__ KeyRow load_stream(const KeyRow* p) {
+#if HMJ_STREAM_POLICY >= 2
+  KeyRow t;
+  t.key = __builtin_nontemporal_load(reinterpret_cast<const u64*>(p));
+  return t;
+#else
+  return *p;
+#endif
+}
+template <typename Row>
+__device__ __forceinline__ Row row_as(const Tup& t);
+template <>
+__device__ __forceinline__ Tup row_as<Tup>(const Tup& t) { return t; }
+template <>
+__device__ __forceinline__ KeyRow row_as<KeyRow>(const Tup& t) {
+  KeyRow k;
+  k.key = t.key;
+  return k;
+}
+template <typename Row>
+__device__ __forceinline__ Row row_as(const KeyRow& t) { return t; }
 
 constexpr u64 GT_EMPTY = ~0ull;
 constexpr int GT_MAXWALK = 64;
@@ -107,6 +140,7 @@
 constexpr u64 ERR_FASTPATH = 8;
 constexpr u64 ERR_GTABLE = 128;
 constexpr u64 ERR_PREFIX = 4;
+constexpr u64 ERR_BARE = 256;
 
 __device__ __forceinline__ u64 mix64(u64 x) {
   x ^= x >> 30;
diff --git a/hashmergejoin_amd/csrc/hmj_launch.h b/hashmergejoin_amd/csrc/hmj_launch.h
--- a/hashmergejoin_amd/csrc/hmj_launch.h
+++ b/hashmergejoin_amd/csrc/hmj_launch.h
@@ -46,13 +46,15 @@
   u32 WA, rpw, CA, CB, KB;
   u64 rows_a, rows_b;
 };
-bool slab_geometry(u32 n, int bits_a, int bits_b, SlabGeom* g, u32 kb = 0, double fan = 1.0, double density = 1.0);
+bool slab_geometry(u32 n, int bits_a, int bits_b, SlabGeom* g, u32 kb = 0, double fan = 1.0, double density = 1.0, u32 row_bytes = 16);
 bool slab_geometry_one_pass(u32 n, int bits, double keys_per_digit, u32 max_workers, SlabGeom* g, double density = 1.0);
 u32 slab_capacity(double mean, double fan);
 hipError_t launch_slab_a(const void* in, u32 n, int shift, int bits, const SlabGeom& g, void* slab_a, u64 slab_a_rows,
-                         u32* cnt_a, u64 cnt_a_n, u64* accum, hipStream_t st, u32 w_begin = 0, u32 w_end = 0xFFFFFFFFu);
+                         u32* cnt_a, u64 cnt_a_n, u64* accum, hipStream_t st, u32 w_begin = 0, u32 w_end = 0xFFFFFFFFu,
+                         u32 row_bytes = 16);
 hipError_t launch_slab_b(const void* slab_a, const u32* cnt_a, int bits_a, int shift, int bits,
-                         const SlabGeom& g, void* slab_b, u64 slab_b_rows, u32* cnt_b, u64 cnt_b_n, u64* accum, hipStream_t st);
+                         const SlabGeom& g, void* slab_b, u64 slab_b_rows, u32* cnt_b, u64 cnt_b_n, u64* accum, hipStream_t st,
+                         u32 row_bytes = 16);
 hipError_t launch_key_sample(const void* R, u32 nb, const void* S, u32 np, u64* out, hipStream_t st);
 hipError_t launch_key_exact(const void* R, u32 nb, const void* S, u32 np, u64 ref, u64* out, int num_cus, hipStream_t st,
                             bool ref_is_first_key = false);
@@ -99,7 +101,7 @@
                               bool set, u64 fill, int num_cus, hipStream_t st);
 hipError_t launch_probe_count_ext(const ProbeArgs& a, u32* irregular, u32* n_irregular, bool slab,
                                   int num_cus, hipStream_t st);
-hipError_t launch_probe_count_slab(const ProbeArgs& a, int num_cus, hipStream_t st);
+hipError_t launch_probe_count_slab(const ProbeArgs& a, int num_cus, hipStream_t st, bool bare = false);
 hipError_t launch_probe_write_sorted(const ProbeArgs& a, bool slab, bool fk, int shape, u64* lookback, bool chained, int key_low,
                                      int num_cus, hipStream_t st);
 hipError_t launch_probe_write_uniq(const ProbeArgs& a, bool slab, int num_cus, hipStream_t st);
diff --git a/hashmergejoin_amd/csrc/probe.hip b/hashmergejoin_amd/csrc/probe.hip
--- a/hashmergejoin_amd/csrc/probe.hip
+++ b/hashmergejoin_amd/csrc/probe.hip
@@ -892,8 +892,8 @@
   return x >> (32 - LOG_NB);
 }
 
-template <int THREADS, int ROWS = FP_ROWS>
-__device__ __forceinline__ void fp_load(Tup (&t)[ROWS], const Tup* __restrict__ base, u32 n,
+template <int THREADS, int ROWS = FP_ROWS, typename Row = Tup>
+__device__ __forceinline__ void fp_load(Row (&t)[ROWS], const Row* __restrict__ base, u32 n,
                                         int tid) {
 #pragma unroll
   for (int k = 0; k < ROWS; k++) {
@@ -903,8 +903,8 @@
 }
 
 static_assert(SLAB_KB == 4, "fp_load_slab / fp_load_pieces / slab_np_kernel unroll exactly four pieces per partition");
-template <int THREADS, int ROWS = FP_ROWS>
-__device__ __forceinline__ void fp_load_slab(Tup (&t)[ROWS], const Tup* __restrict__ base, u32 cap,
+template <int THREADS, int ROWS = FP_ROWS, typename Row = Tup>
+__device__ __forceinline__ void fp_load_slab(Row (&t)[ROWS], const Row* __restrict__ base, u32 cap,
                                              u32 p1, u32 p2, u32 p3, u32 n, int tid) {
 #pragma unroll
   for (int k = 0; k < ROWS; k++) {
@@ -916,11 +916,11 @@
   }
 }
 
-template <int THREADS>
-__device__ __forceinline__ void fp_load_pieces(Tup (&t)[FP_ROWS], const Tup* __restrict__ base, u32 cap, u32 cnt_mine, int tid) {
+template <int THREADS, typename Row>
+__device__ __forceinline__ void fp_load_pieces(Row (&t)[FP_ROWS], const Row* __restrict__ base, u32 cap, u32 cnt_mine, int tid) {
   constexpr int QT = THREADS / 4;
   const u32 g = (u32)tid / QT, l = (u32)tid % QT;
-  const Tup* __restrict__ piece = base + (u64)g * cap;
+  const Row* __restrict__ piece = base + (u64)g * cap;
   const u32 last = cnt_mine ? cnt_mine - 1 : 0;
 #pragma unroll
   for (int k = 0; k < FP_ROWS; k++) {
@@ -929,17 +929,19 @@
   }
 }
 
-template <int THREADS, int LOG_NB, bool PCOUNT, bool SLAB, int OUT>
+template <int THREADS, int LOG_NB, bool PCOUNT, bool SLAB, int OUT, bool BARE = false>
 __global__ __launch_bounds__(THREADS, 4) void probe_count_fast_kernel(
     ProbeArgs a, u32* __restrict__ irregular, u32* __restrict__ n_irregular) {
   typedef FastSmem<THREADS, LOG_NB> Smem;
   constexpr u32 CAP = Smem::CAP, NB = 1u << LOG_NB;
   constexpr bool PIECES = SLAB && OUT == 0 && !PCOUNT && HMJ_PROBE_PIECES;
+  static_assert(!BARE || PIECES, "bare probe rows: the piece walk of the plain count join only");
+  typedef typename std::conditional<BARE, KeyRow, Tup>::type PRow;
   constexpr u32 QT = THREADS / 4, PIECE_CAP = FP_ROWS * QT;
   extern __shared__ __attribute__((aligned(16))) unsigned char smem_raw[];
   Smem& sm = *reinterpret_cast<Smem*>(smem_raw);
   const Tup* __restrict__ R = static_cast<const Tup*>(a.R);
-  const Tup* __restrict__ S = static_cast<const Tup*>(a.S);
+  const PRow* __restrict__ S = static_cast<const PRow*>(a.S);
   const u32* __restrict__ r_off = a.r_off;
   const u32* __restrict__ s_off = a.s_off;
   const u32* __restrict__ r_end = (SLAB || a.r_end == nullptr) ? a.r_off + 1 : a.r_end;
@@ -948,6 +950,7 @@
   const int tid = threadIdx.x;
   u64 acc_n = 0, acc_r = 0, acc_s = 0, acc_x = 0, acc_m = 0, acc_p = 0;
   bool pfx_bad = false, giveup = false;
+  bool bare_bad = false;
   for (u32 i = tid; i < NB; i += THREADS) sm.head[i] = 0;
   if (tid < 2) sm.itemcnt[tid] = 0;
   u32 epoch = 0;
@@ -956,7 +959,8 @@
   u32 p = blockIdx.x;
   u32 rb = 0, nb = 0, sb = 0, np = 0;
   bool regular = false;
-  Tup br[FP_ROWS], pr[FP_ROWS], pq[FP_ROWS];
+  Tup br[FP_ROWS];
+  PRow pr[FP_ROWS], pq[FP_ROWS];
   u32 r1 = 0, r2 = 0, r3 = 0, s1 = 0, s2 = 0, s3 = 0, r1n = 0, r2n = 0, r3n = 0, s1n = 0, s2n = 0, s3n = 0;
   u32 rm = 0, sm_ = 0, rmn = 0, smn = 0;
   const u32 my_piece = (u32)tid / QT;
@@ -983,7 +987,7 @@
     }
     regular = nb && np && nb <= CAP && np <= CAP;
     if (regular) {
-      if (PIECES) {
+      if constexpr (PIECES) {
         fp_load_pieces<THREADS>(br, R + (u64)p * SLAB_KB * a.r_cap, a.r_cap, rm, tid);
         fp_load_pieces<THREADS>(pr, S + (u64)p * SLAB_KB * a.s_cap, a.s_cap, sm_, tid);
       } else if (SLAB) {
@@ -1005,14 +1009,15 @@
     else
       fp_load<THREADS>(t, ok ? R + rb_ : dummy, ok ? nb_ : 1u, tid);
   };
-  auto load_probe = [&](Tup (&t)[FP_ROWS], bool ok, u32 pp, u32 sb_, u32 np_, u32 q1, u32 q2, u32 q3, u32 mine) {
-    if (PIECES)
-      fp_load_pieces<THREADS>(t, ok ? S + (u64)pp * SLAB_KB * a.s_cap : dummy, ok ? a.s_cap : 0u, ok ? mine : 1u, tid);
+  const PRow* __restrict__ dummy_s = reinterpret_cast<const PRow*>(a.accum);
+  auto load_probe = [&](PRow (&t)[FP_ROWS], bool ok, u32 pp, u32 sb_, u32 np_, u32 q1, u32 q2, u32 q3, u32 mine) {
+    if constexpr (PIECES)
+      fp_load_pieces<THREADS>(t, ok ? S + (u64)pp * SLAB_KB * a.s_cap : dummy_s, ok ? a.s_cap : 0u, ok ? mine : 1u, tid);
     else if (SLAB)
-      fp_load_slab<THREADS>(t, ok ? S + (u64)pp * SLAB_KB * a.s_cap : dummy, ok ? a.s_cap : 0u, ok ? q1 : 1u, ok ? q2 : 1u,
+      fp_load_slab<THREADS>(t, ok ? S + (u64)pp * SLAB_KB * a.s_cap : dummy_s, ok ? a.s_cap : 0u, ok ? q1 : 1u, ok ? q2 : 1u,
                             ok ? q3 : 1u, ok ? np_ : 1u, tid);
     else
-      fp_load<THREADS>(t, ok ? S + sb_ : dummy, ok ? np_ : 1u, tid);
+      fp_load<THREADS>(t, ok ? S + sb_ : dummy_s, ok ? np_ : 1u, tid);
   };
   const int tid_outer = tid;
   while (p < P) {
@@ -1102,9 +1107,10 @@
         for (int k = 0; k < FP_ROWS; k++) {
           const u32 j = k * THREADS + tid;
           cur[k] = NIL;
-          cnt[k] = 0;
+          cnt[k] = BARE ? 1 : 0;
           first[k] = OUT == 2 ? NIL : 0;
           if (PIECES ? ((u32)tid % QT + (u32)k * QT < sm_) : (j < np)) {
+            if (BARE) cnt[k] = 0;
             if (a.pfx_shift && (pr[k].key >> a.pfx_shift) != a.pfx_val) pfx_bad = true;
             if (OUT >= 1 && (a.extra & 1u)) acc_p += pr[k].val;
             const u32 hv = sm.head[fast_hash<LOG_NB>(pr[k].key)];
@@ -1129,6 +1135,7 @@
                   acc_n++;
                   acc_r += vv;
                   acc_s += pr[k].val;
+                  if (BARE) cnt[k]++;
                   if (OUT == 1) {
                     if (cnt[k] == 0) first[k] = i;
                     cnt[k]++;
@@ -1143,6 +1150,10 @@
             }
           }
         }
+        if (BARE) {
+#pragma unroll
+          for (int k = 0; k < FP_ROWS; k++) bare_bad |= cnt[k] != 1;
+        }
         if (OUT == 2 && (a.extra & 2u)) {
 #pragma unroll
           for (int k = 0; k < FP_ROWS; k++) {
@@ -1222,11 +1233,12 @@
         parity ^= 1;
       }
     } else {
+      if (BARE && np && !nb) bare_bad = true;
       if ((PCOUNT || OUT == 1) && tid == 0 && !(nb && np)) a.part_count[p] = 0;
       if (OUT == 1 && nb && np) giveup = true;
       if (OUT >= 1 && (a.extra & 1u) && !nb) {
         if (SLAB) {
-          const Tup* base = S + (u64)p * SLAB_KB * a.s_cap;
+          const PRow* base = S + (u64)p * SLAB_KB * a.s_cap;
           for (u32 j = tid; j < np; j += THREADS) {
             const u32 pc = (j >= s1) + (j >= s2) + (j >= s3);
             const u32 pre = pc == 0 ? 0 : pc == 1 ? s1 : pc == 2 ? s2 : s3;
@@ -1248,6 +1260,7 @@
     rm = rmn; sm_ = smn;
   }
   if (SLAB && slab_bad && tid == 0) atomicOr(&a.accum[ACC_ERR], ERR_SLAB);
+  if (BARE && __any(bare_bad) && (tid & 63) == 0) atomicOr(&a.accum[ACC_ERR], ERR_BARE);
   if (OUT == 1 && __any(giveup) && (tid & 63) == 0) atomicOr(&a.accum[ACC_ERR], ERR_FASTPATH);
   if (__any(pfx_bad) && (tid & 63) == 0) atomicOr(&a.accum[ACC_ERR], ERR_PREFIX);
   lds_barrier();
@@ -2410,15 +2423,15 @@
   return hipGetLastError();
 }
 
-template <int THREADS, int LOG_NB, bool PCOUNT, bool SLAB = false, int OUT = 0>
+template <int THREADS, int LOG_NB, bool PCOUNT, bool SLAB = false, int OUT = 0, bool BARE = false>
 static hipError_t launch_fast_t(const ProbeArgs& a, u32* irregular, u32* n_irregular, int grid,
                                 hipStream_t st) {
   typedef FastSmem<THREADS, LOG_NB> Smem;
   static SmemAttrOnce attr_once;
-  if (hipError_t e = ensure_max_smem(attr_once, reinterpret_cast<const void*>(probe_count_fast_kernel<THREADS, LOG_NB, PCOUNT, SLAB, OUT>), (size_t)sizeof(Smem)); e != hipSuccess) return e;
+  if (hipError_t e = ensure_max_smem(attr_once, reinterpret_cast<const void*>(probe_count_fast_kernel<THREADS, LOG_NB, PCOUNT, SLAB, OUT, BARE>), (size_t)sizeof(Smem)); e != hipSuccess) return e;
   if ((u32)grid > a.P) grid = (int)a.P;
   if (grid < 1) grid = 1;
-  hipLaunchKernelGGL((probe_count_fast_kernel<THREADS, LOG_NB, PCOUNT, SLAB, OUT>), dim3(grid), dim3(THREADS),
+  hipLaunchKernelGGL((probe_count_fast_kernel<THREADS, LOG_NB, PCOUNT, SLAB, OUT, BARE>), dim3(grid), dim3(THREADS),
                      sizeof(Smem), st, a, irregular, n_irregular);
   return hipGetLastError();
 }
@@ -2433,10 +2446,10 @@
   return launch_fast_t<512, 11, false>(a, irregular, n_irregular, num_cus * 3 * 4, st);
 }
 
-static bool slab_operands_ok(const ProbeArgs& a) {
+static bool slab_operands_ok(const ProbeArgs& a, u32 s_row_bytes = 16) {
   const u64 pieces = (u64)a.P * SLAB_KB;
   return a.r_cnt && a.s_cnt && a.r_cnt_n >= pieces && a.s_cnt_n >= pieces && a.r_rows >= pieces * a.r_cap &&
-         a.s_rows >= pieces * a.s_cap;
+         a.s_rows * 16 >= pieces * a.s_cap * s_row_bytes;
 }
 
 hipError_t launch_probe_write_uniq(const ProbeArgs& a, bool slab, int num_cus, hipStream_t st) {
@@ -2520,8 +2533,9 @@
   return launch_fast_t<1024, BIG_LOG_NB, false, false, 2>(a, irregular, n_irregular, num_cus * 4, st);
 }
 
-hipError_t launch_probe_count_slab(const ProbeArgs& a, int num_cus, hipStream_t st) {
-  if (!slab_operands_ok(a)) return hipErrorInvalidValue;
+hipError_t launch_probe_count_slab(const ProbeArgs& a, int num_cus, hipStream_t st, bool bare) {
+  if (!slab_operands_ok(a, bare ? 8 : 16)) return hipErrorInvalidValue;
+  if (bare) return launch_fast_t<1024, BIG_LOG_NB, false, true, 0, true>(a, nullptr, nullptr, num_cus * 4, st);
   return launch_fast_t<1024, BIG_LOG_NB, false, true>(a, nullptr, nullptr, num_cus * 4, st);
 }
 
diff --git a/hashmergejoin_amd/csrc/radix.hip b/hashmergejoin_amd/csrc/radix.hip
--- a/hashmergejoin_amd/csrc/radix.hip
+++ b/hashmergejoin_amd/csrc/radix.hip
@@ -274,19 +274,24 @@
 #define WC_VMWAIT()
 #endif
 
-template <int THREADS, int MAXD>
+template <int THREADS, int MAXD, typename Row = Tup>
 struct WcSmem {
   static constexpr int TILE = THREADS * WC_ITEMS;
   static constexpr int WAVES = THREADS / kWave;
-  static constexpr int ZROWS = WAVES * MAXD * 8 / 16;
-  static constexpr int MAXLINES = TILE / WC_LINE + 2 * MAXD;
+  static constexpr int LINE = 128 / (int)sizeof(Row);
+  static constexpr int LINE_SH = LINE == 16 ? 4 : 3;
+  static constexpr int ZROWS = WAVES * MAXD * 8 / (int)sizeof(Row);
+  static constexpr int MAXLINES = TILE / LINE + 2 * MAXD;
+  static constexpr int CITEMS = MAXD * LINE / THREADS;
+  static_assert(LINE == (1 << LINE_SH) && (LINE == WC_LINE || LINE == 2 * WC_LINE), "rows of 16 or 8 bytes");
   static_assert(ZROWS <= TILE && ZROWS % THREADS == 0, "lane masks must alias whole row slabs");
-  static_assert(MAXD <= THREADS && MAXD * WC_LINE == TILE, "one digit per thread; carry == tile slots");
+  static_assert(MAXD <= THREADS && MAXD * LINE == CITEMS * THREADS, "one digit per thread; whole carry slots per thread");
+  static_assert(TILE <= 65536 / 16, "ranks, tile offsets and line counts are packed into 16 bits");
   union {
-    Tup stage[TILE];
+    Row stage[TILE];
     u64 lanemask[WAVES][MAXD];
   };
-  Tup carry[MAXD][WC_LINE];
+  Row carry[MAXD][LINE];
   u16 wcnt[WAVES][MAXD];
   u32 tile_off[MAXD];
   u32 cflush[MAXD];
@@ -303,12 +308,13 @@
 struct NoLimit {
   __device__ __forceinline__ u32 operator()(u32) const { return 0xFFFFFFFFu; }
 };
-template <int THREADS, int MAXD, bool HI, bool ALLVALID, bool LIMIT, typename Prefetch, typename Limit>
-__device__ __forceinline__ void wc_tile(WcSmem<THREADS, MAXD>& sm, Tup (&t)[WC_ITEMS], u32 tile_n,
-                                        Tup* __restrict__ out, int shift, u32 mask, u32 D,
+template <int THREADS, int MAXD, bool HI, bool ALLVALID, bool LIMIT, typename Prefetch, typename Limit, typename Row, typename In>
+__device__ __forceinline__ void wc_tile(WcSmem<THREADS, MAXD, Row>& sm, In (&t)[WC_ITEMS], u32 tile_n,
+                                        Row* __restrict__ out, int shift, u32 mask, u32 D,
                                         Prefetch&& prefetch, const Limit& limit, bool* ovf WC_STAMP_ARG) {
-  typedef WcSmem<THREADS, MAXD> Smem;
+  typedef WcSmem<THREADS, MAXD, Row> Smem;
   constexpr int WAVES = Smem::WAVES;
+  constexpr int WC_LINE = Smem::LINE, LINE_SH = Smem::LINE_SH, CITEMS = Smem::CITEMS;
   const int tid = threadIdx.x, lane = tid & 63, w = tid >> 6;
   u16* wc = &sm.wcnt[w][0];
   u64* lm = &sm.lanemask[w][0];
@@ -373,7 +379,7 @@
         }
         const u32 tail = (cf[j] + avail) & (WC_LINE - 1);
         fl[j] = (tail >= avail) ? 0u : avail - tail;
-        nl[j] = fl[j] ? (((cf[j] & (WC_LINE - 1)) + fl[j] + WC_LINE - 1) >> 3) : 0u;
+        nl[j] = fl[j] ? (((cf[j] & (WC_LINE - 1)) + fl[j] + WC_LINE - 1) >> LINE_SH) : 0u;
         sm.pend[d] = avail - fl[j];
         sm.cflush[d] = cf[j] + fl[j];
       }
@@ -417,7 +423,7 @@
       }
       const u32 tail = (cf + avail) & (WC_LINE - 1);
       fl = (tail >= avail) ? 0u : avail - tail;
-      nl = fl ? (((cf & (WC_LINE - 1)) + fl + WC_LINE - 1) >> 3) : 0u;
+      nl = fl ? (((cf & (WC_LINE - 1)) + fl + WC_LINE - 1) >> LINE_SH) : 0u;
       sm.pend[tid] = avail - fl;
       sm.cflush[tid] = cf + fl;
     }
@@ -442,7 +448,7 @@
   for (int r = 0; r < WC_ITEMS; r++) {
     if (ALLVALID || wbase + r * 64 < tile_n) {
       const u32 d = dr[r] >> 16;
-      sm.stage[sm.tile_off[d] + sm.wcnt[w][d] + (dr[r] & 0xFFFFu)] = t[r];
+      sm.stage[sm.tile_off[d] + sm.wcnt[w][d] + (dr[r] & 0xFFFFu)] = row_as<Row>(t[r]);
     }
   }
   WC_MARK(5);
@@ -453,7 +459,7 @@
 
   {
     const u32 TL = sm.total_lines, k = (u32)tid & (WC_LINE - 1);
-    for (u32 L = (u32)tid >> 3; L < TL; L += THREADS / WC_LINE) {
+    for (u32 L = (u32)tid >> LINE_SH; L < TL; L += THREADS / WC_LINE) {
       const u32 d = sm.line_tab[L];
       const u32 pl = sm.plan[d], fl = pl >> 8, pd = pl & 0xFFu;
       u32 cfd;
@@ -464,11 +470,12 @@
       if (j < fl) store_stream(&out[grow], (j < pd) ? sm.carry[d][j] : sm.stage[sm.tile_off[d] + j - pd]);
     }
   }
-  u64 keep_k[WC_ITEMS], keep_v[WC_ITEMS];
+  constexpr bool HAS_VAL = std::is_same<Row, Tup>::value;
+  u64 keep_k[CITEMS], keep_v[HAS_VAL ? CITEMS : 1];
   u32 has = 0;
 #pragma unroll
-  for (int q = 0; q < WC_ITEMS; q++) {
-    const u32 s = q * THREADS + tid, d = s >> 3, k = s & (WC_LINE - 1);
+  for (int q = 0; q < CITEMS; q++) {
+    const u32 s = q * THREADS + tid, d = s >> LINE_SH, k = s & (WC_LINE - 1);
     u32 idx = 0;
     if (d < D && k < sm.pend[d]) {
       const u32 pl = sm.plan[d], fl = pl >> 8, pd = pl & 0xFFu;
@@ -477,29 +484,30 @@
         has |= 1u << q;
       }
     }
-    const Tup kv = sm.stage[idx];
+    const Row kv = sm.stage[idx];
     keep_k[q] = kv.key;
-    keep_v[q] = kv.val;
+    if constexpr (HAS_VAL) keep_v[q] = kv.val;
   }
   WC_MARK(7);
   lds_barrier();
   WC_MARK(8);
 #pragma unroll
-  for (int q = 0; q < WC_ITEMS; q++) {
+  for (int q = 0; q < CITEMS; q++) {
     const u32 s = q * THREADS + tid;
     if (has & (1u << q)) {
-      Tup kv;
+      Row kv;
       kv.key = keep_k[q];
-      kv.val = keep_v[q];
-      sm.carry[s >> 3][s & (WC_LINE - 1)] = kv;
+      if constexpr (HAS_VAL) kv.val = keep_v[q];
+      sm.carry[s >> LINE_SH][s & (WC_LINE - 1)] = kv;
     }
   }
 #if HMJ_WC_NOBAR5
   {
-    constexpr int ZR = MAXD * 8 / 16;
-    Tup z;
-    z.key = 0;
-    z.val = 0;
+    constexpr int ZR = MAXD * 8 / (int)sizeof(Row);
+    Tup z0;
+    z0.key = 0;
+    z0.val = 0;
+    const Row z = row_as<Row>(z0);
 #pragma unroll
     for (int r = 0; r < ZR / kWave; r++) sm.stage[w * ZR + r * kWave + lane] = z;
     u32* wz = reinterpret_cast<u32*>(&sm.wcnt[w][0]);
@@ -515,7 +523,7 @@
       Tup z;
       z.key = 0;
       z.val = 0;
-      sm.stage[r * THREADS + tid] = z;
+      sm.stage[r * THREADS + tid] = row_as<Row>(z);
     }
   }
   for (int i = tid; i < WAVES * MAXD / 2; i += THREADS) reinterpret_cast<u32*>(&sm.wcnt[0][0])[i] = 0;
@@ -525,20 +533,21 @@
 #endif
 }
 
-template <int THREADS, int MAXD>
-__device__ __forceinline__ void wc_flush_carry(WcSmem<THREADS, MAXD>& sm, Tup* __restrict__ out, u32 D) {
+template <int THREADS, int MAXD, typename Row>
+__device__ __forceinline__ void wc_flush_carry(WcSmem<THREADS, MAXD, Row>& sm, Row* __restrict__ out, u32 D) {
+  typedef WcSmem<THREADS, MAXD, Row> Smem;
   const int tid = threadIdx.x;
   lds_barrier();
 #pragma unroll
-  for (int q = 0; q < WC_ITEMS; q++) {
-    const u32 s = q * THREADS + tid, d = s >> 3, k = s & (WC_LINE - 1);
+  for (int q = 0; q < Smem::CITEMS; q++) {
+    const u32 s = q * THREADS + tid, d = s >> Smem::LINE_SH, k = s & (Smem::LINE - 1);
     if (d < D && k < sm.pend[d]) store_stream(&out[sm.cflush[d] + k], sm.carry[d][k]);
   }
 }
 
-template <int THREADS, int MAXD>
-__device__ __forceinline__ void wc_clear(WcSmem<THREADS, MAXD>& sm) {
-  constexpr int WAVES = WcSmem<THREADS, MAXD>::WAVES;
+template <int THREADS, int MAXD, typename Row>
+__device__ __forceinline__ void wc_clear(WcSmem<THREADS, MAXD, Row>& sm) {
+  constexpr int WAVES = WcSmem<THREADS, MAXD, Row>::WAVES;
   const int tid = threadIdx.x;
   for (int i = tid; i < WAVES * MAXD / 2; i += THREADS) reinterpret_cast<u32*>(&sm.wcnt[0][0])[i] = 0;
   for (int i = tid; i < WAVES * MAXD; i += THREADS) (&sm.lanemask[0][0])[i] = 0;
@@ -615,11 +624,20 @@
 struct NoXform {
   static constexpr bool kStrided = false;
 };
-template <int THREADS, int MAXD, bool HI, typename Xform>
+struct SumXform {
+  static constexpr bool kStrided = false;
+  u64 acc_s;
+  __device__ __forceinline__ void operator()(Tup (&t)[WC_ITEMS], u32 tile_n, u32 wbase) {
+#pragma unroll
+    for (int r = 0; r < WC_ITEMS; r++)
+      if (wbase + (u32)r * 64 < tile_n) acc_s += t[r].val;
+  }
+};
+template <int THREADS, int MAXD, bool HI, typename Xform, typename Row = Tup>
 __device__ __forceinline__ void slab_a_body(const Tup* __restrict__ in, u32 n, int shift, int bits, u32 rows_per_worker,
-                                            Tup* __restrict__ slab, u32 CA, u32 WA, u32* __restrict__ cnt_out,
+                                            Row* __restrict__ slab, u32 CA, u32 WA, u32* __restrict__ cnt_out,
                                             u64* __restrict__ accum, u32 worker_base, Xform& xf) {
-  typedef WcSmem<THREADS, MAXD> Smem;
+  typedef WcSmem<THREADS, MAXD, Row> Smem;
   constexpr int TILE = Smem::TILE;
   extern __shared__ __attribute__((aligned(16))) unsigned char smem_raw[];
   Smem& sm = *reinterpret_cast<Smem*>(smem_raw);
@@ -728,11 +746,11 @@
 #endif
 constexpr int SLAB_MAXSEG = 512;
 
-template <int THREADS, int MAXD, bool HI, int ADDR>
+template <int THREADS, int MAXD, bool HI, int ADDR, typename Row = Tup>
 __global__ __launch_bounds__(THREADS, (THREADS * (MAXD <= 256 ? 2 : 1)) / 256) void radix_slab_b_kernel(
-    const Tup* __restrict__ slab_a, const u32* __restrict__ cnt_a, u32 CA, u32 WA, int bits_a, int shift,
-    int bits, Tup* __restrict__ slab_b, u32 CB, u32* __restrict__ cnt_b, u64* __restrict__ accum, u32 KB) {
-  typedef WcSmem<THREADS, MAXD> Smem;
+    const Row* __restrict__ slab_a, const u32* __restrict__ cnt_a, u32 CA, u32 WA, int bits_a, int shift,
+    int bits, Row* __restrict__ slab_b, u32 CB, u32* __restrict__ cnt_b, u64* __restrict__ accum, u32 KB) {
+  typedef WcSmem<THREADS, MAXD, Row> Smem;
   constexpr int TILE = Smem::TILE;
   static_assert(SLAB_MAXSEG <= THREADS, "one A-slab count per thread in the prologue scan");
   extern __shared__ __attribute__((aligned(16))) unsigned char smem_raw[];
@@ -764,14 +782,14 @@
 #endif
   const u32 wbase = (u32)w * (WC_ITEMS * 64) + lane;
   (void)wbase;
-  const Tup* __restrict__ bucket = slab_a + (u64)(dA * WA + w0) * CA;
+  const Row* __restrict__ bucket = slab_a + (u64)(dA * WA + w0) * CA;
   bool ovf = false;
 #ifdef HMJ_STAMPS
   WcStamps stamps = {};
   stamps.base = 16;
 #endif
   if (total) {
-    Tup t[WC_ITEMS];
+    Row t[WC_ITEMS];
     if constexpr (ADDR != 0) {
     u32 d_s0 = 0, d_b0 = 0, d_b1 = 0, d_b2 = 0, d_b3 = 0;
     const float slabs_per_row = (float)ns / (float)total;
@@ -1120,12 +1138,26 @@
   }
 }
 
-template <int THREADS, int MAXD, bool HI>
+template <int THREADS, int MAXD, bool HI, typename Row = Tup>
 __global__ __launch_bounds__(THREADS, (THREADS * (MAXD <= 256 ? 2 : 1)) / 256) void radix_slab_a_kernel(
-    const Tup* __restrict__ in, u32 n, int shift, int bits, u32 rows_per_worker, Tup* __restrict__ slab,
+    const Tup* __restrict__ in, u32 n, int shift, int bits, u32 rows_per_worker, Row* __restrict__ slab,
     u32 CA, u32 WA, u32* __restrict__ cnt_out, u64* __restrict__ accum, u32 worker_base) {
-  NoXform xf;
-  slab_a_body<THREADS, MAXD, HI, NoXform>(in, n, shift, bits, rows_per_worker, slab, CA, WA, cnt_out, accum, worker_base, xf);
+  if constexpr (std::is_same<Row, Tup>::value) {
+    NoXform xf;
+    slab_a_body<THREADS, MAXD, HI, NoXform>(in, n, shift, bits, rows_per_worker, slab, CA, WA, cnt_out, accum, worker_base, xf);
+  } else {
+    SumXform xf{0ull};
+    slab_a_body<THREADS, MAXD, HI, SumXform, Row>(in, n, shift, bits, rows_per_worker, slab, CA, WA, cnt_out, accum, worker_base, xf);
+    __shared__ u64 wsum[THREADS / kWave];
+    const u64 ws = wave_sum_u64(xf.acc_s);
+    if ((threadIdx.x & 63) == 0) wsum[threadIdx.x >> 6] = ws;
+    __syncthreads();
+    if (threadIdx.x == 0) {
+      u64 tot = 0;
+      for (int w = 0; w < THREADS / kWave; w++) tot += wsum[w];
+      if (tot) atomicAdd(reinterpret_cast<unsigned long long*>(&accum[ACC_SUM_S]), (unsigned long long)tot);
+    }
+  }
 }
 
 template <bool CUT>
@@ -1202,28 +1234,35 @@
     if (rows) atomicAdd(reinterpret_cast<unsigned long long*>(&accum[ACC_N]), (unsigned long long)rows);
   }
 }
-template <int THREADS, int MAXD, bool HI>
+template <int THREADS, int MAXD, bool HI, typename Row = Tup>
 static hipError_t launch_slab_a_t(const void* in, u32 n, int shift, int bits, u32 rpw, void* slab, u32 CA,
                                   u32 WA, u32* cnt, u64* accum, hipStream_t st, u32 w_begin, u32 w_end) {
-  typedef WcSmem<THREADS, MAXD> Smem;
+  typedef WcSmem<THREADS, MAXD, Row> Smem;
   const size_t smem = sizeof(Smem);
   static_assert(sizeof(Smem) <= 160 * 1024, "slab pass A: LDS");
   static SmemAttrOnce attr_once;
-  if (hipError_t e = ensure_max_smem(attr_once, reinterpret_cast<const void*>(radix_slab_a_kernel<THREADS, MAXD, HI>), (size_t)smem); e != hipSuccess) return e;
+  if (hipError_t e = ensure_max_smem(attr_once, reinterpret_cast<const void*>(radix_slab_a_kernel<THREADS, MAXD, HI, Row>), (size_t)smem); e != hipSuccess) return e;
   if (w_end > WA) w_end = WA;
   if (w_begin >= w_end) return hipSuccess;
-  hipLaunchKernelGGL((radix_slab_a_kernel<THREADS, MAXD, HI>), dim3(w_end - w_begin), dim3(THREADS), smem, st,
-                     static_cast<const Tup*>(in), n, shift, bits, rpw, static_cast<Tup*>(slab), CA, WA, cnt,
+  hipLaunchKernelGGL((radix_slab_a_kernel<THREADS, MAXD, HI, Row>), dim3(w_end - w_begin), dim3(THREADS), smem, st,
+                     static_cast<const Tup*>(in), n, shift, bits, rpw, static_cast<Row*>(slab), CA, WA, cnt,
                      accum, w_begin);
   return hipGetLastError();
 }
 
-template <int THREADS, int MAXD, bool HI>
+template <int THREADS, int MAXD, bool HI, typename Row = Tup>
 static hipError_t launch_slab_b_t(const void* slab_a, const u32* cnt_a, u32 CA, u32 WA, int bits_a, int shift,
                                   int bits, void* slab_b, u32 CB, u32* cnt_b, u64* accum, hipStream_t st, u32 KB) {
-  typedef WcSmem<THREADS, MAXD> Smem;
+  typedef WcSmem<THREADS, MAXD, Row> Smem;
   const size_t smem = sizeof(Smem) + (SLAB_MAXSEG + 1) * sizeof(u32);
   static_assert(sizeof(Smem) + (SLAB_MAXSEG + 1) * sizeof(u32) <= 160 * 1024, "slab pass B: LDS");
+  if constexpr (!std::is_same<Row, Tup>::value) {
+    static SmemAttrOnce attr_bare;
+    if (hipError_t e = ensure_max_smem(attr_bare, reinterpret_cast<const void*>(radix_slab_b_kernel<THREADS, MAXD, HI, 2, Row>), (size_t)smem); e != hipSuccess) return e;
+    hipLaunchKernelGGL((radix_slab_b_kernel<THREADS, MAXD, HI, 2, Row>), dim3((1u << bits_a) * KB), dim3(THREADS), smem, st,
+                       static_cast<const Row*>(slab_a), cnt_a, CA, WA, bits_a, shift, bits, static_cast<Row*>(slab_b), CB, cnt_b, accum, KB);
+    return hipGetLastError();
+  } else {
 #ifdef HMJ_DEV
   if (g_b_addr_alt) {
     constexpr int ALT = HMJ_B_ADDR == 2 ? 1 : 2;
@@ -1241,15 +1280,18 @@
                      static_cast<const Tup*>(slab_a), cnt_a, CA, WA, bits_a, shift, bits,
                      static_cast<Tup*>(slab_b), CB, cnt_b, accum, KB);
   return hipGetLastError();
-}
-
-static u32 slab_cap(double mean, double fan) {
+  }
+}
+
+static u32 slab_cap(double mean, double fan, u32 line = 8) {
   double c = mean + 8.0 * __builtin_sqrt(fan * mean) + 24.0;
-  return ((u32)c + 8) & ~7u;
+  return ((u32)c + line) & ~(line - 1);
 }
 u32 slab_capacity(double mean, double fan) { return slab_cap(mean, fan < 1.0 ? 1.0 : fan); }
-bool slab_geometry(u32 n, int bits_a, int bits_b, SlabGeom* g, u32 kb, double fan, double density) {
+bool slab_geometry(u32 n, int bits_a, int bits_b, SlabGeom* g, u32 kb, double fan, double density, u32 row_bytes) {
   if (bits_a < 1 || bits_a > SLAB_MAX_BITS || bits_b < 1 || bits_b > SLAB_MAX_BITS) return false;
+  if (row_bytes != 16 && !(row_bytes == 8 && bits_a <= 8 && bits_b <= 8)) return false;
+  const u32 line = 128 / row_bytes;
   const u32 tile = bits_a > 8 ? 4096 : 2048;
   u64 tiles = ((u64)n + tile - 1) / tile;
   u64 max_workers = 2048;
@@ -1266,8 +1308,8 @@
   if (fan < 1.0) fan = 1.0;
   if (density < 1.0) density = 1.0;
   const double fan_a = 1.0 + 4.0 * (double)g->rpw * fan / (double)(n ? n : 1);
-  g->CA = slab_cap(density * (double)g->rpw / (double)(1u << bits_a), fan_a < fan ? fan_a : fan);
-  g->CB = slab_cap(density * (double)n / (double)(1u << bits_a) / (double)kb / (double)(1u << bits_b), fan);
+  g->CA = slab_cap(density * (double)g->rpw / (double)(1u << bits_a), fan_a < fan ? fan_a : fan, line);
+  g->CB = slab_cap(density * (double)n / (double)(1u << bits_a) / (double)kb / (double)(1u << bits_b), fan, line);
   const u64 rows_a = (u64)(1u << bits_a) * g->WA * g->CA;
   const u64 rows_b = (u64)(1u << (bits_a + bits_b)) * kb * g->CB;
   g->rows_a = rows_a;
@@ -1295,14 +1337,16 @@
 }
 
 hipError_t launch_slab_a(const void* in, u32 n, int shift, int bits, const SlabGeom& g, void* slab_a, u64 slab_a_rows,
-                         u32* cnt_a, u64 cnt_a_n, u64* accum, hipStream_t st, u32 w_begin, u32 w_end) {
+                         u32* cnt_a, u64 cnt_a_n, u64* accum, hipStream_t st, u32 w_begin, u32 w_end, u32 row_bytes) {
   if (bits < 1 || bits > SLAB_MAX_BITS || g.WA == 0 || g.CA == 0 || (u64)g.WA * g.rpw < n) return hipErrorInvalidValue;
-  if (slab_a_rows < ((u64)g.WA << bits) * g.CA || cnt_a_n < ((u64)g.WA << bits)) return hipErrorInvalidValue;
+  if (row_bytes != 16 && !(row_bytes == 8 && bits <= 8 && g.CA % 16 == 0)) return hipErrorInvalidValue;
+  if (slab_a_rows * 16 < ((u64)g.WA << bits) * g.CA * row_bytes || cnt_a_n < ((u64)g.WA << bits)) return hipErrorInvalidValue;
   if (((u64)g.WA << bits) * g.CA >= 0xFFFFFFF0ull) return hipErrorInvalidValue;
   const bool hi = shift >= 32;
-#define HMJ_SLAB_A(T, M, H) launch_slab_a_t<T, M, H>(in, n, shift, bits, g.rpw, slab_a, g.CA, g.WA, cnt_a, accum, st, w_begin, w_end)
-  if (bits > 8) return hi ? HMJ_SLAB_A(1024, 512, true) : HMJ_SLAB_A(1024, 512, false);
-  return hi ? HMJ_SLAB_A(512, 256, true) : HMJ_SLAB_A(512, 256, false);
+#define HMJ_SLAB_A(T, M, H, R) launch_slab_a_t<T, M, H, R>(in, n, shift, bits, g.rpw, slab_a, g.CA, g.WA, cnt_a, accum, st, w_begin, w_end)
+  if (row_bytes == 8) return hi ? HMJ_SLAB_A(512, 256, true, KeyRow) : HMJ_SLAB_A(512, 256, false, KeyRow);
+  if (bits > 8) return hi ? HMJ_SLAB_A(1024, 512, true, Tup) : HMJ_SLAB_A(1024, 512, false, Tup);
+  return hi ? HMJ_SLAB_A(512, 256, true, Tup) : HMJ_SLAB_A(512, 256, false, Tup);
 #undef HMJ_SLAB_A
 }
 
@@ -1348,16 +1392,19 @@
 }
 
 hipError_t launch_slab_b(const void* slab_a, const u32* cnt_a, int bits_a, int shift, int bits,
-                         const SlabGeom& g, void* slab_b, u64 slab_b_rows, u32* cnt_b, u64 cnt_b_n, u64* accum, hipStream_t st) {
+                         const SlabGeom& g, void* slab_b, u64 slab_b_rows, u32* cnt_b, u64 cnt_b_n, u64* accum, hipStream_t st,
+                         u32 row_bytes) {
   if (bits < 1 || bits > SLAB_MAX_BITS || bits_a < 1 || bits_a > SLAB_MAX_BITS || g.KB == 0 || g.WA < g.KB ||
       (g.WA + g.KB - 1) / g.KB > (u32)SLAB_MAXSEG)
     return hipErrorInvalidValue;
   const u64 pieces = ((u64)g.KB << (bits_a + bits));
-  if (slab_b_rows < pieces * g.CB || cnt_b_n < pieces || pieces * g.CB >= 0xFFFFFFF0ull) return hipErrorInvalidValue;
+  if (row_bytes != 16 && !(row_bytes == 8 && bits <= 8 && bits_a <= 8 && g.CA % 16 == 0 && g.CB % 16 == 0)) return hipErrorInvalidValue;
+  if (slab_b_rows * 16 < pieces * g.CB * row_bytes || cnt_b_n < pieces || pieces * g.CB >= 0xFFFFFFF0ull) return hipErrorInvalidValue;
   const bool hi = shift >= 32;
-#define HMJ_SLAB_B(T, M, H) launch_slab_b_t<T, M, H>(slab_a, cnt_a, g.CA, g.WA, bits_a, shift, bits, slab_b, g.CB, cnt_b, accum, st, g.KB)
-  if (bits > 8) return hi ? HMJ_SLAB_B(1024, 512, true) : HMJ_SLAB_B(1024, 512, false);
-  return hi ? HMJ_SLAB_B(512, 256, true) : HMJ_SLAB_B(512, 256, false);
+#define HMJ_SLAB_B(T, M, H, R) launch_slab_b_t<T, M, H, R>(slab_a, cnt_a, g.CA, g.WA, bits_a, shift, bits, slab_b, g.CB, cnt_b, accum, st, g.KB)
+  if (row_bytes == 8) return hi ? HMJ_SLAB_B(512, 256, true, KeyRow) : HMJ_SLAB_B(512, 256, false, KeyRow);
+  if (bits > 8) return hi ? HMJ_SLAB_B(1024, 512, true, Tup) : HMJ_SLAB_B(1024, 512, false, Tup);
+  return hi ? HMJ_SLAB_B(512, 256, true, Tup) : HMJ_SLAB_B(512, 256, false, Tup);
 #undef HMJ_SLAB_B
 }
 
diff --git a/hashmergejoin_amd/join.py b/hashmergejoin_amd/join.py
--- a/hashmergejoin_amd/join.py
+++ b/hashmergejoin_amd/join.py
@@ -91,6 +91,9 @@
 
     def forget_workloads(self):
         self._check(self.L.hmj_forget_workloads(self.h))
+
+    def last_probe_row_bytes(self):
+        return int(self.L.hmj_last_probe_row_bytes(self.h))
 
     def placement_info(self):
         arr = (_lib.PlaceInfo * 16)()
diff --git a/include/hmj.h b/include/hmj.h
--- a/include/hmj.h
+++ b/include/hmj.h
@@ -167,6 +167,7 @@
 int hmj_placement_info(hmj_ctx* ctx, hmj_place_info* out, int max_entries);
 int hmj_last_plan(hmj_ctx* ctx, hmj_plan_desc* out);
 int hmj_forget_workloads(hmj_ctx* ctx);
+uint32_t hmj_last_probe_row_bytes(hmj_ctx* ctx);
 int hmj_set_profiling(hmj_ctx* ctx, int enabled);
 int hmj_last_timing(hmj_ctx* ctx, hmj_timing* out);
 const char* hmj_strerror(int code);
```
